# HyoJong-Moon/Distributed-Inference-System-based-Storm

Hardware: AMD Instinct MI355X
Metric: images/sec (whole node) + p50 latency, CIFAR-10 ResNet-20 at 1/2/4/8 GPUs (higher is better)
Workload: dtype bf16

## Files before the change

### csrc/bindings/host_bindings.cpp

```cpp
#include <pybind11/functional.h>
#include <pybind11/numpy.h>
#include <pybind11/pybind11.h>
#include <pybind11/stl.h>

#include <time.h>

#include <atomic>
#include <chrono>
#include <mutex>
#include <thread>

#include "../codec/json_codec.h"
#include "gale/llc_pair.h"
#include "../codec/text_pack.h"
#include "../kafka/broker.h"
#include "../kafka/client.h"
#include "../kafka/compress.h"
#include "../kafka/fetch_framing.h"
#include "../runtime/batch_plan.h"
#include "../runtime/ingest_plan.h"
#include "../runtime/pack_tap.h"
#include "../runtime/resize_plan.h"
#include "plan_dict.h"
#include "../kafka/protocol.h"
// ... 161 lines not shown
    const int64_t t0 = now_ns();
    const int64_t m = (int64_t)set_->batches.size();
    size_t pi = 0;
    int64_t sent = 0;
    while (!stop_) {
      const double due = (double)(now_ns() - t0) * 1e-9 * rate;
      while (!stop_) {
        const size_t k = (size_t)(((next_ % m) + m) % m);
        const int32_t nrec = set_->records[k];
        if ((double)(sent + nrec) > due) break;
        const int part = parts_[pi++ % parts_.size()];
        const int64_t base = b_->append_shared(topic_, part, set_->batches[k]);
        const int64_t t = now_ns();
        {
          std::lock_guard<std::mutex> lk(mu_);
          lp_.push_back(part);
          lbase_.push_back(base);
          ln_.push_back(nrec);
          lt_.push_back(t);
        }
        sent += nrec;
        appended_ += nrec;
        ++next_;
      }
      const int32_t nrec = set_->records[(size_t)(((next_ % m) + m) % m)];
      const double wait_s = ((double)(sent + nrec) - (double)(now_ns() - t0) * 1e-9 * rate) / rate;
      std::this_thread::sleep_for(std::chrono::nanoseconds(
          std::max<int64_t>(20000, (int64_t)(wait_s * 1e9))));
    }
  }
  std::shared_ptr<Broker> b_;
  std::string topic_;
  std::vector<int> parts_;
  std::shared_ptr<BatchSet> set_;
  std::thread t_;
  std::atomic<bool> stop_{true};
  std::atomic<int64_t> next_{0}, appended_{0};
  std::mutex mu_;
  std::vector<int32_t> lp_, ln_;
  std::vector<int64_t> lbase_, lt_;
};

std::shared_ptr<BatchSet> synthetic_batches(const float* x, int64_t n, int H, int W, int C,
                                            int ipr, int rpb, int threads,
                                            const std::string& key_prefix) {
  if (ipr <= 0 || rpb <= 0 || n <= 0) throw std::invalid_argument("synthetic_batches: bad sizes");
  auto bs = std::make_shared<BatchSet>();
  bs->images_per_record = ipr;
  const int64_t nrec = (n + ipr - 1) / ipr;
  const int64_t nb = (nrec + rpb - 1) / rpb;
  bs->batches.resize((size_t)nb);
  bs->records.resize((size_t)nb);
  const size_t img = (size_t)H * W * C;
  std::atomic<int64_t> next{0};
  auto work = [&] {
    std::vector<std::string> vals, keys;
    std::vector<RecordIn> ins;
    for (int64_t b; (b = next++) < nb;) {
      const int64_t r0 = b * rpb, r1 = std::min<int64_t>(nrec, r0 + rpb);
      vals.assign((size_t)(r1 - r0), std::string());
      keys.assign((size_t)(r1 - r0), std::string());
      ins.assign((size_t)(r1 - r0), RecordIn());
      for (int64_t r = r0; r < r1; ++r) {
        const int64_t i0 = r * ipr, cnt = std::min<int64_t>(ipr, n - i0);
        codec::encode_instances(x + (size_t)i0 * img, (int)cnt, H, W, C, vals[(size_t)(r - r0)]);
        RecordIn& ri = ins[(size_t)(r - r0)];
        ri.value = vals[(size_t)(r - r0)];
        if (!key_prefix.empty()) {
          keys[(size_t)(r - r0)] = key_prefix + std::to_string(r);
          ri.key = keys[(size_t)(r - r0)];
          ri.key_null = false;
        }
      }
      Writer w;
      encode_batch(w, ins.data(), ins.size(), 0, 0);
      bs->records[(size_t)b] = (int32_t)(r1 - r0);
      bs->batches[(size_t)b] = std::make_shared<const std::string>(std::move(w.buf));
    }
  };
  std::vector<std::thread> ts;
  for (int t = 1; t < std::max(1, threads); ++t) ts.emplace_back(work);
  work();
  for (auto& t : ts) t.join();
  for (auto& b : bs->batches) bs->bytes += b->size();
  return bs;
}

std::vector<std::string> strs(const py::handle& o) { return o.cast<std::vector<std::string>>(); }

py::bytes py_encode(const std::string& name, py::dict d) {
  Writer w;
  if (name == "request_header") {
    RequestHeader h;
    h.api_key = d["api_key"].cast<int16_t>();
    h.api_version = d["api_version"].cast<int16_t>();
    h.correlation_id = d["correlation_id"].cast<int32_t>();
    h.client_id = d["client_id"].cast<std::string>();
    encode_request_header(w, h);
  } else if (name == "metadata_request") {
    MetadataRequest m;
    if (d["topics"].is_none()) m.all_topics = true;
    else m.topics = strs(d["topics"]);
    m.allow_auto_topic_creation = d["allow_auto_topic_creation"].cast<bool>();
    encode_metadata_request(w, m);
  } else if (name == "fetch_request") {
    FetchRequest m;
    m.max_wait_ms = d["max_wait_ms"].cast<int32_t>();
    m.min_bytes = d["min_bytes"].cast<int32_t>();
    m.max_bytes = d["max_bytes"].cast<int32_t>();
    FetchTopic t;
    t.name = d["topic"].cast<std::string>();
    for (auto p : d["partitions"].cast<py::list>()) {
      auto tp = p.cast<py::tuple>();
      t.partitions.push_back({tp[0].cast<int32_t>(), tp[1].cast<int64_t>(), tp[2].cast<int32_t>()});
    }
    m.topics.push_back(t);
    encode_fetch_request(w, m);
  } else if (name == "produce_request") {
    ProduceRequest m;
    m.acks = d["acks"].cast<int16_t>();
    m.timeout_ms = d["timeout_ms"].cast<int32_t>();
    ProduceTopic t;
    t.name = d["topic"].cast<std::string>();
    ProducePartition pp;
    pp.index = d["partition"].cast<int32_t>();
    pp.records = std::string(view(d["records"].cast<py::bytes>()));
    t.partitions.push_back(pp);
    m.topics.push_back(t);
    encode_produce_request(w, m);
  } else if (name == "list_offsets_request") {
    ListOffsetsRequest m;
    m.topics.push_back({d["topic"].cast<std::string>(),
                        {{d["partition"].cast<int32_t>(), d["timestamp"].cast<int64_t>()}}});
    encode_list_offsets_request(w, m);
  } else if (name == "offset_commit_request") {
    OffsetCommitRequest m;
    m.group_id = d["group_id"].cast<std::string>();
    CommitTopic t;
    t.name = d["topic"].cast<std::string>();
    CommitPartition cp;
    cp.index = d["partition"].cast<int32_t>();
    cp.offset = d["offset"].cast<int64_t>();
    t.partitions.push_back(cp);
    m.topics.push_back(t);
    encode_offset_commit_request(w, m);
  } else {
    throw std::invalid_argument("unknown message " + name);
  }
  return py::bytes(w.buf);
}

py::dict py_decode(const std::string& name, py::bytes b) {
  const std::string_view s = view(b);
  Reader r(s);
  py::dict d;
  if (name == "metadata_response") {
    const MetadataResponse m = decode_metadata_response(r);
    py::list brokers;
    for (auto& n : m.brokers) brokers.append(py::make_tuple(n.node_id, n.host, n.port));
    d["brokers"] = brokers;
    d["cluster_id"] = m.cluster_id;
    d["controller_id"] = m.controller_id;
    py::dict topics;
    for (auto& t : m.topics) {
      py::list parts;
      for (auto& p : t.partitions) parts.append(py::make_tuple(p.index, p.leader, p.error));
      topics[py::str(t.name)] = py::make_tuple(t.error, parts);
    }
    d["topics"] = topics;
  } else if (name == "produce_response") {
    const ProduceResponse m = decode_produce_response(r);
    py::list parts;
    for (auto& t : m.topics)
      for (auto& p : t.partitions)
        parts.append(py::make_tuple(t.name, p.index, p.error, p.base_offset));
    d["partitions"] = parts;
    d["throttle_ms"] = m.throttle_ms;
  } else if (name == "fetch_response") {
    const FetchResponse m = decode_fetch_response(r);
    py::list parts;
    for (auto& t : m.topics)
      for (auto& p : t.partitions) {
        std::vector<RecordRef> recs;
        if (p.records_len > 0)
          decode_records(reinterpret_cast<const uint8_t*>(s.data()), p.records_off,
                         (size_t)p.records_len, 0, true, recs);
        parts.append(py::make_tuple(t.name, p.index, p.error, p.high_watermark,
                                    records_to_py(reinterpret_cast<const uint8_t*>(s.data()), recs)));
      }
    d["partitions"] = parts;
  } else if (name == "api_versions_response") {
    const ApiVersionsResponse m = decode_api_versions_response(r);
    d["error"] = m.error;
    py::dict apis;
    for (auto& a : m.apis) apis[py::int_(a.key)] = py::make_tuple(a.min_version, a.max_version);
    d["apis"] = apis;
  } else {
    throw std::invalid_argument("unknown message " + name);
  }
  return d;
}

std::shared_ptr<py::object> hold(py::object o) {
  return std::shared_ptr<py::object>(new py::object(std::move(o)), [](py::object* p) {
    py::gil_scoped_acquire g;
    delete p;
  });
}

}

void bind_host(py::module_& m) {
  m.def("status_name", &codec::status_name);
  m.def("scan_instances", [](py::bytes b, int H, int W, int C) {
    const std::string_view s = view(b);
    const codec::Scan sc =
        codec::scan_instances(reinterpret_cast<const uint8_t*>(s.data()), s.size(), H, W, C);
    return py::make_tuple(sc.status, sc.arr_off, sc.arr_len, sc.images);
  });
  m.def("parse_instances_host", [](py::bytes b, int H, int W, int C, int max_images) {
    const std::string_view s = view(b);
    const codec::Scan sc =
        codec::scan_instances(reinterpret_cast<const uint8_t*>(s.data()), s.size(), H, W, C);
    const int n = sc.status == codec::OK ? sc.images : 0;
    py::array_t<float> out({(py::ssize_t)n, (py::ssize_t)H, (py::ssize_t)W, (py::ssize_t)C});
    int images = 0;
    int st = sc.status;
    if (st == codec::OK)
      st = codec::parse_instances_host(reinterpret_cast<const uint8_t*>(s.data()), s.size(), H, W,
                                       C, out.mutable_data(), max_images, &images);
    return py::make_tuple(st, out);
  }, py::arg("data"), py::arg("H"), py::arg("W"), py::arg("C"), py::arg("max_images") = -1);
  m.def("scan_instances_b64", [](py::bytes b, int H, int W, int C) {
    const std::string_view s = view(b);
    const codec::Scan sc =
        codec::scan_instances_b64(reinterpret_cast<const uint8_t*>(s.data()), s.size(), H, W, C);
    return py::make_tuple(sc.status, sc.arr_off, sc.arr_len, sc.images);
  });
  m.def("parse_instances_b64_host", [](py::bytes b, int H, int W, int C, int max_images) {
    const std::string_view s = view(b);
    const uint8_t* p = reinterpret_cast<const uint8_t*>(s.data());
    const codec::Scan sc = codec::scan_instances_b64(p, s.size(), H, W, C);
    const int n = sc.status == codec::OK ? sc.images : 0;
    py::array_t<float> out({(py::ssize_t)n, (py::ssize_t)H, (py::ssize_t)W, (py::ssize_t)C});
    int images = 0;
    int st = sc.status;
    if (st == codec::OK)
      st = codec::parse_instances_b64_host(p, s.size(), H, W, C, out.mutable_data(), max_images,
                                           &images);
    return py::make_tuple(st, out);
  }, py::arg("data"), py::arg("H"), py::arg("W"), py::arg("C"), py::arg("max_images") = -1);
  m.def("b64_image_offsets", [](py::bytes arr, int H, int W, int C) -> py::object {
    const std::string_view s = view(arr);
    std::vector<uint32_t> offs;
    if (!codec::b64_image_offsets(reinterpret_cast<const uint8_t*>(s.data()), s.size(), H, W, C,
                                  offs))
      return py::none();
    return py::cast(offs);
  });
  m.def("plan_b64_ingest",
        [](std::vector<std::pair<int64_t, int64_t>> batches,
           std::vector<std::tuple<int, int, int64_t, int64_t, int64_t>> recs,
           std::vector<uint32_t> offs, int H, int W, int C, size_t arena_bytes,
           size_t fetch_size, bool check_crcs) {
          std::vector<B64PlanRecord> rs(recs.size());
          for (size_t i = 0; i < recs.size(); ++i) {
            rs[i].status = std::get<0>(recs[i]);
            rs[i].images = std::get<1>(recs[i]);
            rs[i].value_off = std::get<2>(recs[i]);
            rs[i].value_len = std::get<3>(recs[i]);
            rs[i].arr_off = std::get<4>(recs[i]);
          }
          B64IngestPlan p;
          plan_b64_ingest(batches, kafka::kBatchAttrOffset, check_crcs, rs, offs, H, W, C,
                          arena_bytes, fetch_size, p);
          py::list windows, imgs;
          for (const CrcChunk& c : p.chunks) windows.append(py::make_tuple(c.end, c.len));
          for (const B64Image& d : p.imgs) imgs.append(py::make_tuple(d.off, d.slot, d.rec));
          py::dict out;
          out["windows"] = windows;
          out["batch_windows"] = py::cast(p.batch_chunks);
          out["images"] = imgs;
          out["slot0"] = py::cast(p.slot0);
          out["img0"] = py::cast(p.img0);
          out["chunks_per_image"] = p.chunks_per_image;
          out["lo"] = p.lo;
          out["hi"] = p.hi;
          out["o_chunks"] = p.o_chunks;
          out["o_imgs"] = p.o_imgs;
          out["plan_bytes"] = p.plan_bytes;
          out["o_crc"] = p.o_crc;
          out["o_bad"] = p.o_bad;
          out["result_bytes"] = p.result_bytes;
          return out;
        },
        py::arg("batches"), py::arg("recs"), py::arg("offs"), py::arg("H"), py::arg("W"),
        py::arg("C"), py::arg("arena_bytes"), py::arg("fetch_size"),
        py::arg("check_crcs") = true,
        "The host plan of a b64 fetch's device ingest (csrc/runtime/ingest_plan.h)");
  m.def("plan_json_ingest",
        [](std::vector<std::pair<int64_t, int64_t>> batches,
           std::vector<std::tuple<int, int64_t, int64_t, int64_t, int64_t>> recs, int H, int W,
           int C, size_t arena_bytes, size_t fetch_size, size_t dev_cap, int64_t tap_result,
           bool plan_separate, bool check_crcs) {
          std::vector<JsonPlanRecord> rs(recs.size());
          for (size_t i = 0; i < recs.size(); ++i) {
            rs[i].status = std::get<0>(recs[i]);
            rs[i].value_off = std::get<1>(recs[i]);
            rs[i].value_len = std::get<2>(recs[i]);
            rs[i].arr_off = std::get<3>(recs[i]);
            rs[i].arr_len = std::get<4>(recs[i]);
          }
          JsonIngestPlan p;
          plan_json_ingest(batches, kafka::kBatchAttrOffset, check_crcs, rs, H, W, C, arena_bytes,
                           fetch_size, dev_cap, tap_result, plan_separate, p);
          std::string plan(p.o_gsum, '\0');
          if (!p.empty()) fill_json_ingest(p, rs, reinterpret_cast<uint8_t*>(&plan[0]));
          py::list windows;
          for (const CrcChunk& c : p.chunks) windows.append(py::make_tuple(c.end, c.len));
          py::dict out;
          out["windows"] = windows;
          out["batch_windows"] = py::cast(p.batch_chunks);
          out["rec_of"] = py::cast(p.rec_of);
          out["pjs"] = py::cast(p.pjs);
          out["nc"] = p.nc();
          out["nr"] = p.nr();
          out["np"] = p.np();
          out["ntiles"] = p.ntiles;
          out["ngroups"] = p.ngroups;
          out["ptiles"] = p.ptiles;
          out["ng"] = p.ng;
          out["packed"] = p.packed;
          out["lo"] = p.lo;
          out["span"] = p.span;
          out["link"] = p.link;
          out["c_lo"] = p.c_lo;
          out["c_len"] = p.c_len;
          out["tab_off"] = p.tab_off;
          out["used"] = p.used;
          out["cnt_base"] = p.cnt_base;
          out["o_chunks"] = p.o_chunks;
          out["o_groups"] = p.o_groups;
          out["o_recs"] = p.o_recs;
          out["o_precs"] = p.o_precs;
          out["o_ptr"] = p.o_ptr;
          out["o_gsum"] = p.o_gsum;
          out["prefix"] = p.o_gsum;
          out["o_crc"] = p.o_crc;
          out["o_gbad"] = p.o_gbad;
          out["o_pbad"] = p.o_pbad;
          out["io_bytes"] = p.io_bytes;
          out["plan_off"] = p.plan_off;
          out["plan_in_chunk"] = p.plan_in_chunk;
          out["plan"] = py::bytes(plan);
          return out;
        },
        py::arg("batches"), py::arg("recs"), py::arg("H"), py::arg("W"), py::arg("C"),
        py::arg("arena_bytes"), py::arg("fetch_size"), py::arg("dev_cap"),
        py::arg("tap_result") = (int64_t)-1, py::arg("plan_separate") = false,
        py::arg("check_crcs") = true,
        "The host plan of a JSON fetch's device ingest, laid out and filled "
        "(csrc/runtime/ingest_plan.h)");
  m.def("plan_batch",
        [](std::vector<py::dict> recs, int max_batch, int tiles_cap, int64_t per,
           const std::string& form, bool ptr_input, bool b64, uint64_t d_bytes,
           uint64_t input_base) {
          std::vector<BatchPlanRecord> rs(recs.size());
          std::vector<uint32_t> offs;
          for (size_t i = 0; i < recs.size(); ++i) {
            const py::dict& d = recs[i];
            BatchPlanRecord& r = rs[i];
            auto get = [&d](const char* k, auto& v) {
              if (d.contains(k)) v = d[k].cast<std::decay_t<decltype(v)>>();
            };
            get("buf", r.buf);
            get("arr_off", r.arr_off);
            get("arr_len", r.arr_len);
            get("images", r.images);
            get("pinned", r.pinned);
            get("resident", r.resident);
            get("preparsed", r.preparsed);
            get("dev_text", r.dev_text);
            get("dev_counts", r.dev_counts);
            get("dev_image", r.dev_image);
            if (d.contains("b64_offs")) {
              const auto o = d["b64_offs"].cast<std::vector<uint32_t>>();
              r.b64_first = (int32_t)offs.size();
              r.b64_n = (int32_t)o.size();
              offs.insert(offs.end(), o.begin(), o.end());
            }
          }
          const StepForm f = form == "op-by-op"   ? StepForm::OpByOp
                             : form == "captured" ? StepForm::Captured
                             : form == "kernels"  ? StepForm::Kernels
                                                  : throw std::invalid_argument("plan_batch: form");
          BatchPlan p;
          plan_batch(rs, max_batch, per, f, ptr_input, b64, p);
          const MetaLayout L(max_batch, std::max(tiles_cap, p.ntiles));
          const MetaRange used = L.used(p);
          std::string meta(L.total, '\xee');
          fill_batch(p, rs, offs, L, d_bytes, input_base, reinterpret_cast<uint8_t*>(&meta[0]));
          py::list spans, staged;
          for (const BatchPlan::Span& x : p.spans)
            spans.append(py::make_tuple(x.buf, x.lo, x.len, x.dev));
          for (const BatchPlan::Staged& g : p.staged)
            staged.append(py::make_tuple(g.rec, g.host, g.len));
          py::dict out;
          out["spans"] = spans;
          out["staged"] = staged;
          out["parse_idx"] = py::cast(p.parse_idx);
          out["staged_bytes"] = p.staged_bytes;
          out["staged_dev"] = p.staged_dev;
          out["dev_total"] = p.dev_total;
          out["nrec"] = p.nrec;
          out["ntiles"] = p.ntiles;
          out["img"] = p.img;
          out["b64n"] = p.b64n;
          out["npre"] = p.npre;
          out["resident"] = p.resident;
          out["count_pass"] = p.count_pass;
          py::dict lay;
          lay["hdr"] = L.hdr;
          lay["recs"] = L.recs;
          lay["xs"] = L.xs;
          lay["tiles"] = L.tiles;
          lay["b64_table"] = L.b64_table;
          lay["b64_status"] = L.b64_status;
          lay["total"] = L.total;
          out["layout"] = lay;
          out["used"] = py::make_tuple(used.off, used.bytes);
          out["meta"] = py::bytes(meta);
          return out;
        },
        py::arg("recs"), py::arg("max_batch"), py::arg("tiles_cap"), py::arg("per"),
        py::arg("form"), py::arg("ptr_input") = false, py::arg("b64") = false,
        py::arg("d_bytes") = (uint64_t)0, py::arg("input_base") = (uint64_t)0,
        "The host plan of a GPU replica's batch, laid out and filled "
        "(csrc/runtime/batch_plan.h)");
  m.def("validate_plan",
        [](py::list ops, std::vector<long long> buf_bytes, int max_batch, int slots, int chunk_ops,
           int chunk_images) {
          const PlanSpec spec = plan_spec_from_py(ops, std::move(buf_bytes), max_batch, slots, {},
                                                  chunk_ops, chunk_images);
          validate_plan(spec);
          return plan_ops_to_py(spec);
        },
        py::arg("ops"), py::arg("buf_bytes"), py::arg("max_batch") = 256, py::arg("slots") = 2,
        py::arg("chunk_ops") = 0, py::arg("chunk_images") = 0,
        "What Executor(...) checks before its first HIP call (gale/forward_plan.h), without a "
        "GPU: ValueError for a plan it would refuse, else the ops with every key written out");
  m.attr("BATCH_ATTR_OFFSET") = (int)kafka::kBatchAttrOffset;
  m.def("split_instances_b64", [](py::bytes arr, int H, int W, int C) -> py::object {
    const std::string_view s = view(arr);
    std::vector<std::pair<uint32_t, uint32_t>> spans;
    if (!codec::split_instances_b64(reinterpret_cast<const uint8_t*>(s.data()), s.size(), H, W,
                                    C, spans))
      return py::none();
    return py::cast(spans);
  });
  m.def("scan_instances_b64_bytes", [](py::bytes b, int64_t nbytes) {
    const std::string_view s = view(b);
    const codec::Scan sc = codec::scan_instances_b64_bytes(
        reinterpret_cast<const uint8_t*>(s.data()), s.size(), nbytes);
    return py::make_tuple(sc.status, sc.arr_off, sc.arr_len, sc.images);
  });
  m.def("b64_image_offsets_bytes", [](py::bytes arr, int64_t nbytes) -> py::object {
    const std::string_view s = view(arr);
    std::vector<uint32_t> offs;
    if (!codec::b64_image_offsets_bytes(reinterpret_cast<const uint8_t*>(s.data()), s.size(),
                                        nbytes, offs))
      return py::none();
    return py::cast(offs);
  });
  m.def("split_instances_b64_bytes", [](py::bytes arr, int64_t nbytes) -> py::object {
    const std::string_view s = view(arr);
    std::vector<std::pair<uint32_t, uint32_t>> spans;
    if (!codec::split_instances_b64_bytes(reinterpret_cast<const uint8_t*>(s.data()), s.size(),
                                          nbytes, spans))
      return py::none();
    return py::cast(spans);
  });
  m.def("yuv_coeffs", [](const std::string& matrix, const std::string& range) {
    YuvCoeffs k;
    const int mi = matrix == "bt601" ? 0 : matrix == "bt709" ? 1 : -1;
    const int ri = range == "limited" ? 0 : range == "full" ? 1 : -1;
    if (!yuv_coeffs(mi, ri, &k)) throw std::invalid_argument("yuv_coeffs: matrix / range");
    return py::make_tuple(k.cy, k.crv, k.cgu, k.cgv, k.cbu, k.yo);
  });
  m.def("yuv420_to_rgb_host",
        [](py::bytes frame, int HS, int WS, const std::string& format,
           std::vector<int32_t> coeffs, std::optional<std::vector<float>> a,
           std::optional<std::vector<float>> b) {
          const std::string_view s = view(frame);
          if (coeffs.size() != 6 || (a && a->size() < 3) || (b && b->size() < 3) ||
              bool(a) != bool(b))
            throw std::invalid_argument("yuv420_to_rgb_host: coeffs (6), a / b (>= 3 each)");
          const int fmt = format == "i420" ? YUV_I420 : format == "nv12" ? YUV_NV12 : YUV_NONE;
          if (fmt == YUV_NONE || HS <= 0 || WS <= 0 || (HS & 1) || (WS & 1) ||
              (int64_t)s.size() != yuv420_bytes(HS, WS))
            throw std::invalid_argument("yuv420_to_rgb_host: format / size / byte count");
          YuvCoeffs k;
          k.cy = coeffs[0], k.crv = coeffs[1], k.cgu = coeffs[2], k.cgv = coeffs[3];
          k.cbu = coeffs[4], k.yo = coeffs[5];
          py::array_t<uint8_t> rgb({(py::ssize_t)HS, (py::ssize_t)WS, (py::ssize_t)3});
          py::array_t<float> f32({(py::ssize_t)HS, (py::ssize_t)WS, (py::ssize_t)3});
          codec::yuv420_to_rgb_host(reinterpret_cast<const uint8_t*>(s.data()), HS, WS, fmt, k,
                                    rgb.mutable_data(), f32.mutable_data(),
                                    a ? a->data() : nullptr, b ? b->data() : nullptr);
          return py::make_tuple(rgb, f32);
        },
        py::arg("frame"), py::arg("HS"), py::arg("WS"), py::arg("format"), py::arg("coeffs"),
        py::arg("a") = py::none(), py::arg("b") = py::none());
  m.def("parse_instances_yuv_host",
        [](py::bytes b, int HS, int WS, const std::string& format, std::vector<int32_t> coeffs,
           int max_images) {
          const std::string_view s = view(b);
          const uint8_t* p = reinterpret_cast<const uint8_t*>(s.data());
          if (coeffs.size() != 6) throw std::invalid_argument("parse_instances_yuv_host: coeffs");
          const int fmt = format == "i420" ? YUV_I420 : format == "nv12" ? YUV_NV12 : YUV_NONE;
          YuvCoeffs k;
          k.cy = coeffs[0], k.crv = coeffs[1], k.cgu = coeffs[2], k.cgv = coeffs[3];
          k.cbu = coeffs[4], k.yo = coeffs[5];
          int n = 0;
          int st = codec::parse_instances_yuv_host(p, s.size(), HS, WS, fmt, k, nullptr,
                                                   max_images, &n);
          if (st != codec::OK) n = 0;
          py::array_t<float> out({(py::ssize_t)n, (py::ssize_t)std::max(HS, 0),
                                  (py::ssize_t)std::max(WS, 0), (py::ssize_t)3});
          if (st == codec::OK)
            st = codec::parse_instances_yuv_host(p, s.size(), HS, WS, fmt, k, out.mutable_data(),
                                                 max_images, &n);
          return py::make_tuple(st, out);
        },
        py::arg("data"), py::arg("HS"), py::arg("WS"), py::arg("format"), py::arg("coeffs"),
        py::arg("max_images") = -1);
  m.def("packed_bpp", [](const std::string& format) {
    return packed_bpp(packed_format_of(format.c_str()));
  });
  m.def("packed_to_rgb_host",
        [](py::bytes image, int HS, int WS, const std::string& format,
           std::optional<std::vector<float>> a, std::optional<std::vector<float>> b) {
          const std::string_view s = view(image);
          if ((a && a->size() < 3) || (b && b->size() < 3) || bool(a) != bool(b))
            throw std::invalid_argument("packed_to_rgb_host: a / b (>= 3 each)");
          const int fmt = packed_format_of(format.c_str());
          if (fmt == PACKED_NONE || HS <= 0 || WS <= 0 ||
              (int64_t)s.size() != packed_bytes(HS, WS, fmt))
            throw std::invalid_argument("packed_to_rgb_host: format / size / byte count");
          py::array_t<uint8_t> rgb({(py::ssize_t)HS, (py::ssize_t)WS, (py::ssize_t)3});
          py::array_t<float> f32({(py::ssize_t)HS, (py::ssize_t)WS, (py::ssize_t)3});
          codec::packed_to_rgb_host(reinterpret_cast<const uint8_t*>(s.data()), HS, WS, fmt,
                                    rgb.mutable_data(), f32.mutable_data(),
                                    a ? a->data() : nullptr, b ? b->data() : nullptr);
          return py::make_tuple(rgb, f32);
        },
        py::arg("image"), py::arg("HS"), py::arg("WS"), py::arg("format"),
        py::arg("a") = py::none(), py::arg("b") = py::none());
  m.def("parse_instances_packed_host",
        [](py::bytes b, int HS, int WS, const std::string& format, int max_images) {
          const std::string_view s = view(b);
          const uint8_t* p = reinterpret_cast<const uint8_t*>(s.data());
          const int fmt = packed_format_of(format.c_str());
          int n = 0;
          int st = codec::parse_instances_packed_host(p, s.size(), HS, WS, fmt, nullptr,
                                                      max_images, &n);
          if (st != codec::OK) n = 0;
          py::array_t<float> out({(py::ssize_t)n, (py::ssize_t)std::max(HS, 0),
                                  (py::ssize_t)std::max(WS, 0), (py::ssize_t)3});
          if (st == codec::OK)
            st = codec::parse_instances_packed_host(p, s.size(), HS, WS, fmt, out.mutable_data(),
                                                    max_images, &n);
          return py::make_tuple(st, out);
        },
        py::arg("data"), py::arg("HS"), py::arg("WS"), py::arg("format"),
        py::arg("max_images") = -1);
  m.def("apply_input_prep",
        [](py::array_t<float, py::array::c_style | py::array::forcecast> x, int H, int W, int C,
           bool nchw, std::vector<float> a, std::vector<float> b) {
          const size_t per = (size_t)H * W * C;
          if (a.size() != 4 || b.size() != 4 || per == 0 || (size_t)x.size() % per != 0)
            throw std::invalid_argument("apply_input_prep: four coefficients, whole images");
          const py::ssize_t n = x.size() / (py::ssize_t)per;
          py::array_t<float> out({n, (py::ssize_t)H, (py::ssize_t)W, (py::ssize_t)C});
          memcpy(out.mutable_data(), x.data(), (size_t)x.size() * sizeof(float));
          codec::apply_input_prep(out.mutable_data(), (int)n, H, W, C, nchw, a.data(), b.data());
          return out;
        },
        py::arg("x"), py::arg("H"), py::arg("W"), py::arg("C"), py::arg("nchw"), py::arg("a"),
        py::arg("b"));
  auto ia = [](const void* p, size_t n) {
    return py::array_t<int32_t>((py::ssize_t)n, static_cast<const int32_t*>(p));
  };
  auto fa = [](const void* p, size_t n) {
    return py::array_t<float>((py::ssize_t)n, static_cast<const float*>(p));
  };
  m.def("build_resize_tables",
        [ia, fa](int HS, int WS, int HR, int WR, int H, int W) {
          codec::ResizeTables t;
          codec::build_resize_tables(HS, WS, HR, WR, H, W, t);
          return py::make_tuple(ia(t.y0.data(), H), ia(t.y1.data(), H), fa(t.wy.data(), H),
                                ia(t.x0.data(), W), ia(t.x1.data(), W), fa(t.wx.data(), W));
        },
        py::arg("HS"), py::arg("WS"), py::arg("HR"), py::arg("WR"), py::arg("H"), py::arg("W"));
  m.def("build_resize_aa_tables",
        [ia, fa](int HS, int WS, int HR, int WR, int H, int W, bool device) -> py::object {
          const InputResize r = InputResize::build(HS, WS, HR, WR, H, W, true);
          const codec::ResizeAaTables& t = r.aa_tables();
          if (!device)
            return py::make_tuple(ia(t.ys.data(), H), ia(t.yn.data(), H),
                                  fa(t.wy.data(), t.wy.size()), ia(t.xs.data(), W),
                                  ia(t.xn.data(), W), fa(t.wx.data(), t.wx.size()));
          const ResizeDeviceImage im = pack(r);
          auto at = [&](int i) { return im.bytes.data() + im.off[i]; };
          return py::make_tuple(ia(at(0), H), ia(at(1), H), fa(at(2), (size_t)H * im.ty),
                                ia(at(3), W), ia(at(4), W), fa(at(5), (size_t)W * im.tx), im.ty,
                                im.tx, im.band, im.band_rows);
        },
        py::arg("HS"), py::arg("WS"), py::arg("HR"), py::arg("WR"), py::arg("H"), py::arg("W"),
        py::arg("device") = false);
  m.def("resize_device_image",
        [](int HS, int WS, int HR, int WR, int H, int W, bool antialias) {
          const ResizeDeviceImage im = pack(InputResize::build(HS, WS, HR, WR, H, W, antialias));
          return py::make_tuple(
              py::array_t<uint8_t>((py::ssize_t)im.bytes.size(), im.bytes.data()),
              py::make_tuple(im.off[0], im.off[1], im.off[2], im.off[3], im.off[4], im.off[5]),
              py::make_tuple(im.ty, im.tx, im.band, im.band_rows));
        },
        py::arg("HS"), py::arg("WS"), py::arg("HR"), py::arg("WR"), py::arg("H"), py::arg("W"),
        py::arg("antialias"));
  for (const bool aa : {false, true}) {
    const char* name = aa ? "resize_crop_aa_host" : "resize_crop_host";
    m.def(name,
          [aa, name](py::array_t<float, py::array::c_style | py::array::forcecast> x, int HR,
                     int WR, int H, int W) {
            if (x.ndim() != 4)
              throw std::invalid_argument(std::string(name) + ": x must be [N, HS, WS, C]");
            const InputResize r =
                InputResize::build((int)x.shape(1), (int)x.shape(2), HR, WR, H, W, aa);
            const int C = (int)x.shape(3);
            py::array_t<float> out({x.shape(0), (py::ssize_t)H, (py::ssize_t)W, (py::ssize_t)C});
            r.apply_host(x.data(), (int)x.shape(0), C, out.mutable_data());
            return out;
          },
          py::arg("x"), py::arg("HR"), py::arg("WR"), py::arg("H"), py::arg("W"));
  }
  m.def("text_pack_fast", &codec::text_pack_fast);
  m.def("llc_pin_self_next_domain", &llc::pin_self_next_domain);
  m.def("llc_register_local_port", &llc::register_local_port);
  m.def("llc_pin_self_for_peer", &llc::pin_self_for_peer);
  m.def("set_pack_stream_stores", &codec::set_pack_stream_stores,
        "non-temporal stores for the packed stream (default on; A/B switch)");
  m.def("text_pack", [](py::bytes b, bool force_scalar) {
    const std::string_view s = view(b);
    std::string out(codec::pack_bound(s.size()), '\0');
    py::array_t<uint32_t> tab((py::ssize_t)(2 * codec::pack_groups(s.size())));
    const size_t n = codec::text_pack(reinterpret_cast<const uint8_t*>(s.data()), s.size(),
                                      reinterpret_cast<uint8_t*>(out.data()), tab.mutable_data(),
                                      force_scalar);
    out.resize(n);
    return py::make_tuple(py::bytes(out), tab);
  }, py::arg("data"), py::arg("force_scalar") = false);
  m.def("text_pack_chunked", [](py::bytes b, std::vector<size_t> cuts) {
    const std::string_view s = view(b);
// ... 683 lines not shown
```

### csrc/bindings/module.cpp

```cpp
#include <pybind11/numpy.h>
#include <pybind11/pybind11.h>
#include <pybind11/stl.h>

#include <optional>
#include <stdexcept>
#include <vector>

#include "../comm/rccl.h"
#include "gale/executor.h"
#include "gale/kernels.h"
#include "plan_dict.h"

namespace py = pybind11;

namespace gale {
void bind_host(py::module_& m);
}

namespace {

using gale::ConvDesc;
using gale::desc_from_dict;

inline hipStream_t S(uintptr_t s) { return reinterpret_cast<hipStream_t>(s); }
inline void* P(uintptr_t p) { return reinterpret_cast<void*>(p); }

void chk(hipError_t e, const char* what) { gale::check_hip(e, what); }

std::optional<gale::InputPrep> prep_from(const char* name,
                                         const std::optional<std::vector<float>>& a,
                                         const std::optional<std::vector<float>>& b, bool nchw) {
  if ((a && a->size() != 4) || (b && b->size() != 4))
    throw std::invalid_argument(std::string(name) + ": a / b take four coefficients");
  if (!a && !b && !nchw) return std::nullopt;
  gale::InputPrep prep;
  for (int i = 0; i < 4; ++i) {
    if (a) prep.a[i] = (*a)[i];
    if (b) prep.b[i] = (*b)[i];
  }
  prep.nchw = nchw ? 1 : 0;
  return prep;
}

}

namespace gale {
void install_crash_handler();
}

namespace {
struct MappedBuffer {
  uint8_t* p = nullptr;
  size_t n = 0;
  explicit MappedBuffer(size_t bytes) : n(bytes) {
    gale::check_hip(hipHostMalloc(reinterpret_cast<void**>(&p), bytes ? bytes : 1,
                                  hipHostMallocMapped),
                    "hipHostMalloc(mapped)");
    void* dp = nullptr;
    gale::check_hip(hipHostGetDevicePointer(&dp, p, 0), "hipHostGetDevicePointer");
    if (dp != p) throw std::runtime_error("mapped buffer: device address differs from host");
  }
  ~MappedBuffer() {
    if (p) hipHostFree(p);
  }
};
}

PYBIND11_MODULE(_C, m) {
  py::class_<MappedBuffer, std::shared_ptr<MappedBuffer>>(
      m, "MappedBuffer", "host-mapped pinned buffer (same address on the host and the GPU)")
      .def(py::init<size_t>())
      .def_property_readonly("ptr", [](const MappedBuffer& b) { return (uintptr_t)b.p; })
      .def_property_readonly("size", [](const MappedBuffer& b) { return b.n; })
      .def("numpy", [](std::shared_ptr<MappedBuffer> b) {
        return py::array_t<uint8_t>({(py::ssize_t)b->n}, {1}, b->p,
                                    py::capsule(new std::shared_ptr<MappedBuffer>(b), [](void* c) {
                                      delete static_cast<std::shared_ptr<MappedBuffer>*>(c);
                                    }));
      });
  m.doc() = "gale native library: gfx950 kernels, plan executor, host runtime";
  gale::install_crash_handler();

  m.def("conv2d",
        [](py::dict desc, int batch, uintptr_t x, uintptr_t w, uintptr_t bias, uintptr_t wscale,
           uintptr_t res, uintptr_t y, uintptr_t stream) {
          ConvDesc d = desc_from_dict(desc);
          chk(gale::conv2d(d, batch, P(x), P(w), static_cast<const float*>(P(bias)),
                           static_cast<const float*>(P(wscale)), P(res), P(y), S(stream)),
              "conv2d");
        },
        py::arg("desc"), py::arg("batch"), py::arg("x"), py::arg("w"), py::arg("bias"),
        py::arg("wscale"), py::arg("res"), py::arg("y"), py::arg("stream"));
  m.def("bottleneck56",
        [](int batch, uintptr_t x, uintptr_t w1, uintptr_t b1, uintptr_t w2, uintptr_t b2,
           uintptr_t w3, uintptr_t b3, uintptr_t wd, uintptr_t bd, uintptr_t y, int cin,
           int down, uintptr_t stream) {
          gale::BottleneckParams bp;
          bp.w1 = P(w1); bp.w2 = P(w2); bp.w3 = P(w3); bp.wd = P(wd);
          bp.b1 = static_cast<const float*>(P(b1));
          bp.b2 = static_cast<const float*>(P(b2));
          bp.b3 = static_cast<const float*>(P(b3));
          bp.bd = static_cast<const float*>(P(bd));
          bp.cin = cin;
          bp.down = down;
          chk(gale::bottleneck56(bp, batch, P(x), P(y), S(stream)), "bottleneck56");
        },
        py::arg("batch"), py::arg("x"), py::arg("w1"), py::arg("b1"), py::arg("w2"),
        py::arg("b2"), py::arg("w3"), py::arg("b3"), py::arg("wd"), py::arg("bd"), py::arg("y"),
        py::arg("cin"), py::arg("down"), py::arg("stream"));
  m.def("bottleneck56_supported", &gale::bottleneck56_supported, py::arg("H"), py::arg("W"),
        py::arg("cin"), py::arg("cmid"), py::arg("cout"), py::arg("down"));
  m.def("stem_pool",
        [](int batch, uintptr_t x, uintptr_t w, uintptr_t bias, uintptr_t y, uintptr_t stream) {
          chk(gale::stem_pool(batch, P(x), P(w), static_cast<const float*>(P(bias)), P(y),
                              S(stream)),
              "stem_pool");
        },
        py::arg("batch"), py::arg("x"), py::arg("w"), py::arg("bias"), py::arg("y"),
        py::arg("stream"));
  m.def("stem_pack",
        [](int batch, int H, int W, int C, int Wp, int lp, uintptr_t x, uintptr_t y,
           uintptr_t stream) {
          chk(gale::stem_pack(batch, H, W, C, Wp, lp, static_cast<const float*>(P(x)), P(y),
                              S(stream)),
              "stem_pack");
        });
  m.def("maxpool2d",
        [](int batch, int H, int W, int C, int k, int s, int p, int Ho, int Wo, uintptr_t x,
           uintptr_t y, uintptr_t stream, int fp8) {
          chk(gale::maxpool2d(batch, H, W, C, k, s, p, Ho, Wo, P(x), P(y), fp8, S(stream)),
              "maxpool2d");
        },
        py::arg("batch"), py::arg("H"), py::arg("W"), py::arg("C"), py::arg("k"), py::arg("s"),
        py::arg("p"), py::arg("Ho"), py::arg("Wo"), py::arg("x"), py::arg("y"), py::arg("stream"),
        py::arg("fp8") = 0);
  m.def("avgpool_global",
        [](int batch, int HW, int C, uintptr_t x, uintptr_t y, uintptr_t stream, int fp8) {
          chk(gale::avgpool_global(batch, HW, C, P(x), P(y), fp8, S(stream)), "avgpool_global");
        },
        py::arg("batch"), py::arg("HW"), py::arg("C"), py::arg("x"), py::arg("y"),
        py::arg("stream"), py::arg("fp8") = 0);
  m.def("head_pool_dense_softmax",
        [](int batch, int HW, int C, int N, uintptr_t x, uintptr_t w, uintptr_t b, uintptr_t out,
           uintptr_t stream, int fp8, float in_scale) {
          chk(gale::head_pool_dense_softmax(batch, HW, C, N, P(x), fp8, in_scale,
                                            static_cast<const float*>(P(w)),
                                            static_cast<const float*>(P(b)),
                                            static_cast<float*>(P(out)), S(stream)),
              "head_pool_dense_softmax");
        },
        py::arg("batch"), py::arg("HW"), py::arg("C"), py::arg("N"), py::arg("x"), py::arg("w"),
        py::arg("b"), py::arg("out"), py::arg("stream"), py::arg("fp8") = 0,
        py::arg("in_scale") = 1.0f);
  m.def("softmax_rows", [](int batch, int N, int ld, uintptr_t x, uintptr_t out, uintptr_t stream) {
    chk(gale::softmax_rows(batch, N, ld, static_cast<const float*>(P(x)),
                           static_cast<float*>(P(out)), S(stream)),
        "softmax_rows");
  });
  m.def("cast_f32_bf16",
        [](int64_t n, float scale, float shift, uintptr_t x, uintptr_t y, uintptr_t stream) {
          chk(gale::cast_f32_bf16(n, scale, shift, static_cast<const float*>(P(x)), P(y),
                                  S(stream)),
              "cast_f32_bf16");
        });
  m.def("bn_act",
        [](int batch, int HW, int Wo, int C, uintptr_t x, uintptr_t scale, uintptr_t shift,
           uintptr_t res, int res_H, int res_W, int res_C, int rs, int relu, uintptr_t y,
           uintptr_t stream) {
          chk(gale::bn_act(batch, HW, Wo, C, P(x), static_cast<const float*>(P(scale)),
                           static_cast<const float*>(P(shift)), P(res), res_H, res_W, res_C, rs,
                           relu, P(y), S(stream)),
              "bn_act");
        });
  m.def("json_parse_instances",
        [](int nrec, int ntiles, uintptr_t recs, uintptr_t tile_rec, uintptr_t bytes, int H,
           int W, int C, uintptr_t tile_counts, uintptr_t out, uintptr_t stream,
           bool count_pass, std::optional<std::vector<float>> a,
           std::optional<std::vector<float>> b, bool nchw, uintptr_t d_ntiles, uintptr_t status,
           uintptr_t tile_bad) {
          const auto prep = prep_from("json_parse_instances", a, b, nchw);
          chk(gale::json_parse_instances(nrec, ntiles, static_cast<gale::JsonRecord*>(P(recs)),
                                         static_cast<const int*>(P(tile_rec)),
                                         static_cast<const uint8_t*>(P(bytes)), H, W, C,
                                         static_cast<int*>(P(tile_counts)),
                                         static_cast<float*>(P(out)), S(stream), count_pass,
                                         static_cast<const int*>(P(d_ntiles)),
                                         static_cast<int*>(P(status)),
                                         static_cast<int*>(P(tile_bad)),
                                         prep ? &*prep : nullptr),
              "json_parse_instances");
        },
        py::arg("nrec"), py::arg("ntiles"), py::arg("recs"), py::arg("tile_rec"),
        py::arg("bytes"), py::arg("H"), py::arg("W"), py::arg("C"), py::arg("tile_counts"),
        py::arg("out"), py::arg("stream"), py::arg("count_pass") = true,
        py::arg("a") = py::none(), py::arg("b") = py::none(), py::arg("nchw") = false,
        py::arg("d_ntiles") = 0, py::arg("status") = 0, py::arg("tile_bad") = 0);
  m.def("json_tile_count", &gale::json_tile_count);
  m.def("b64_decode_instances",
        [](int images, uintptr_t imgs, uintptr_t bytes, int H, int W, int C, uintptr_t out,
           uintptr_t status, uintptr_t stream, uintptr_t d_images,
           std::optional<std::vector<float>> a, std::optional<std::vector<float>> b, bool nchw) {
          const auto prep = prep_from("b64_decode_instances", a, b, nchw);
          chk(gale::b64_decode_instances(images, static_cast<const gale::B64Image*>(P(imgs)),
                                         static_cast<const uint8_t*>(P(bytes)), H, W, C,
                                         static_cast<float*>(P(out)),
                                         static_cast<int*>(P(status)), S(stream),
                                         static_cast<const int*>(P(d_images)),
                                         prep ? &*prep : nullptr),
              "b64_decode_instances");
        },
        py::arg("images"), py::arg("imgs"), py::arg("bytes"), py::arg("H"), py::arg("W"),
        py::arg("C"), py::arg("out"), py::arg("status"), py::arg("stream"),
        py::arg("d_images") = 0, py::arg("a") = py::none(), py::arg("b") = py::none(),
        py::arg("nchw") = false);
  m.def("b64_yuv_instances",
        [](int images, uintptr_t imgs, uintptr_t bytes, int HS, int WS, int C, uintptr_t out,
           uintptr_t status, uintptr_t stream, uintptr_t d_images, const std::string& format,
           std::vector<int32_t> coeffs, std::optional<std::vector<float>> a,
           std::optional<std::vector<float>> b, bool nchw, int pairs) {
          const auto prep = prep_from("b64_yuv_instances", a, b, nchw);
          if (coeffs.size() != 6)
            throw std::invalid_argument("b64_yuv_instances: coeffs takes (cy, crv, cgu, cgv, "
                                        "cbu, yo)");
          gale::YuvCoeffs k;
          k.cy = coeffs[0], k.crv = coeffs[1], k.cgu = coeffs[2], k.cgv = coeffs[3];
          k.cbu = coeffs[4], k.yo = coeffs[5];
          const int fmt = format == "i420"   ? (int)gale::YUV_I420
                          : format == "nv12" ? (int)gale::YUV_NV12
                                             : (int)gale::YUV_NONE;
          return (int)gale::b64_yuv_instances(
              images, static_cast<const gale::B64Image*>(P(imgs)),
              static_cast<const uint8_t*>(P(bytes)), HS, WS, C, static_cast<float*>(P(out)),
              static_cast<int*>(P(status)), S(stream), static_cast<const int*>(P(d_images)),
              prep ? &*prep : nullptr, fmt, k, pairs);
        },
        py::arg("images"), py::arg("imgs"), py::arg("bytes"), py::arg("HS"), py::arg("WS"),
        py::arg("C"), py::arg("out"), py::arg("status"), py::arg("stream"),
        py::arg("d_images") = 0, py::arg("format") = "i420",
        py::arg("coeffs") = std::vector<int32_t>{1220945, 1673555, -410793, -852458, 2115221, 16},
        py::arg("a") = py::none(), py::arg("b") = py::none(), py::arg("nchw") = false,
        py::arg("pairs") = 0);
  m.def("b64_packed_instances",
        [](int images, uintptr_t imgs, uintptr_t bytes, int HS, int WS, int C, uintptr_t out,
           uintptr_t status, uintptr_t stream, uintptr_t d_images, const std::string& format,
           std::optional<std::vector<float>> a, std::optional<std::vector<float>> b, bool nchw) {
          const auto prep = prep_from("b64_packed_instances", a, b, nchw);
          return (int)gale::b64_packed_instances(
              images, static_cast<const gale::B64Image*>(P(imgs)),
              static_cast<const uint8_t*>(P(bytes)), HS, WS, C, static_cast<float*>(P(out)),
              static_cast<int*>(P(status)), S(stream), static_cast<const int*>(P(d_images)),
              prep ? &*prep : nullptr, gale::packed_format_of(format.c_str()));
        },
        py::arg("images"), py::arg("imgs"), py::arg("bytes"), py::arg("HS"), py::arg("WS"),
        py::arg("C"), py::arg("out"), py::arg("status"), py::arg("stream"),
        py::arg("d_images") = 0, py::arg("format") = "bgr24", py::arg("a") = py::none(),
        py::arg("b") = py::none(), py::arg("nchw") = false);
  m.def("b64_yuv_pairs", &gale::b64_yuv_pairs);
  m.def("b64_yuv_lds_bytes", &gale::b64_yuv_lds_bytes);
  m.attr("YUV_LDS_BUDGET") = (int)gale::kYuvLdsBudget;
  m.attr("HIP_ERROR_INVALID_VALUE") = (int)hipErrorInvalidValue;
  m.attr("B64_IMAGE_BYTES") = (int)sizeof(gale::B64Image);
  py::module_ comm = m.def_submodule("comm", "in-process RCCL communicator (ncclCommInitAll)");
  py::class_<gale::CommGroup, std::shared_ptr<gale::CommGroup>>(comm, "CommGroup")
      .def(py::init([](std::vector<int> devices) {
             py::gil_scoped_release nogil;
             return std::make_shared<gale::CommGroup>(devices);
           }),
           py::arg("devices"))
      .def_property_readonly("size", &gale::CommGroup::size)
      .def_property_readonly("devices", &gale::CommGroup::devices)
      .def("broadcast",
           [](gale::CommGroup& g, uintptr_t send_root, std::vector<uintptr_t> recv, size_t bytes,
              int root) {
             std::vector<void*> r;
             for (uintptr_t p : recv) r.push_back(reinterpret_cast<void*>(p));
             py::gil_scoped_release nogil;
             g.broadcast(reinterpret_cast<const void*>(send_root), r, bytes, root);
           },
           py::arg("send_root"), py::arg("recv"), py::arg("bytes"), py::arg("root") = 0)
      .def("all_reduce_sum_f64",
           [](gale::CommGroup& g, std::vector<uintptr_t> bufs, size_t count) {
             std::vector<double*> b;
             for (uintptr_t p : bufs) b.push_back(reinterpret_cast<double*>(p));
             py::gil_scoped_release nogil;
             g.all_reduce_sum_f64(b, count);
           },
           py::arg("bufs"), py::arg("count"));
  m.def("crc32c_chunks",
        [](uintptr_t bytes, uintptr_t chunks, int n, uintptr_t tables, uintptr_t out,
           uintptr_t stream) {
          gale::check_hip(gale::crc32c_chunks(reinterpret_cast<const uint8_t*>(bytes),
                                              reinterpret_cast<const gale::CrcChunk*>(chunks), n,
                                              reinterpret_cast<const uint32_t*>(tables),
                                              reinterpret_cast<uint32_t*>(out),
                                              reinterpret_cast<hipStream_t>(stream)),
                          "crc32c_chunks");
        });
  m.def("ingest_crc_count",
        [](uintptr_t bytes, uintptr_t chunks, int nchunks, uintptr_t tables, uintptr_t crc_out,
           int nrec, int ngroups, uintptr_t recs, uintptr_t groups, uintptr_t counts,
           uintptr_t gsum, uintptr_t stream, uintptr_t gbad, uintptr_t packed, uintptr_t tab,
           uintptr_t text_out) {
          gale::check_hip(
              gale::ingest_crc_count(reinterpret_cast<const uint8_t*>(bytes),
                                     reinterpret_cast<const gale::CrcChunk*>(chunks), nchunks,
                                     reinterpret_cast<const uint32_t*>(tables),
                                     reinterpret_cast<uint32_t*>(crc_out), nrec, ngroups,
                                     reinterpret_cast<gale::JsonRecord*>(recs),
                                     reinterpret_cast<const int2*>(groups),
                                     reinterpret_cast<int*>(counts),
                                     reinterpret_cast<int*>(gsum),
                                     reinterpret_cast<int*>(gbad),
                                     reinterpret_cast<hipStream_t>(stream),
                                     reinterpret_cast<const uint8_t*>(packed),
                                     reinterpret_cast<const uint32_t*>(tab),
                                     reinterpret_cast<uint8_t*>(text_out)),
              "ingest_crc_count");
        },
        py::arg("bytes"), py::arg("chunks"), py::arg("nchunks"), py::arg("tables"),
        py::arg("crc_out"), py::arg("nrec"), py::arg("ngroups"), py::arg("recs"),
        py::arg("groups"), py::arg("counts"), py::arg("gsum"), py::arg("stream"),
        py::arg("gbad") = 0, py::arg("packed") = 0, py::arg("tab") = 0, py::arg("text_out") = 0,
        "groups: int32 (record, first tile) pairs, GROUP_TILES tiles each; counts: per record "
        "tile0 + grp0 -> [tile counts][group sums]; gsum: one int per group");
  m.attr("GROUP_TILES") = gale::kGroupTiles;
  m.def("ingest_crc_b64",
        [](uintptr_t bytes, uintptr_t chunks, int nchunks, uintptr_t tables, uintptr_t crc_out,
           int images, uintptr_t imgs, int H, int W, int C, uintptr_t arena, uintptr_t wg_bad,
           uintptr_t stream, std::optional<std::vector<float>> a,
           std::optional<std::vector<float>> b, bool nchw) {
          const auto prep = prep_from("ingest_crc_b64", a, b, nchw);
          chk(gale::ingest_crc_b64(static_cast<const uint8_t*>(P(bytes)),
                                   static_cast<const gale::CrcChunk*>(P(chunks)), nchunks,
                                   static_cast<const uint32_t*>(P(tables)),
                                   static_cast<uint32_t*>(P(crc_out)), images,
                                   static_cast<const gale::B64Image*>(P(imgs)), H, W, C,
                                   static_cast<float*>(P(arena)), static_cast<int*>(P(wg_bad)),
                                   S(stream), prep ? &*prep : nullptr),
              "ingest_crc_b64");
        },
        py::arg("bytes"), py::arg("chunks"), py::arg("nchunks"), py::arg("tables"),
        py::arg("crc_out"), py::arg("images"), py::arg("imgs"), py::arg("H"), py::arg("W"),
        py::arg("C"), py::arg("arena"), py::arg("wg_bad"), py::arg("stream"),
        py::arg("a") = py::none(), py::arg("b") = py::none(), py::arg("nchw") = false);
  m.attr("B64_CHUNK_CHARS") = gale::kB64ChunkChars;
  m.def("text_unpack", [](uintptr_t packed, uintptr_t tab, int64_t n, uintptr_t out,
                          uintptr_t stream) {
    if (out % 16 || packed % 8) throw std::invalid_argument("text_unpack: misaligned buffers");
    gale::check_hip(gale::text_unpack(reinterpret_cast<const uint8_t*>(packed),
                                      reinterpret_cast<const uint32_t*>(tab), n,
                                      reinterpret_cast<uint8_t*>(out),
                                      reinterpret_cast<hipStream_t>(stream)),
                    "text_unpack");
  });
  m.def("format_floats_java", [](int n, uintptr_t x, uintptr_t out16, uintptr_t stream) {
    gale::check_hip(gale::format_floats_java(n, reinterpret_cast<const float*>(x),
                                             reinterpret_cast<void*>(out16),
                                             reinterpret_cast<hipStream_t>(stream)),
                    "format_floats_java");
  });
  m.def("format_floats_java_dev",
        [](int max_n, uintptr_t d_count, int per, uintptr_t x, uintptr_t out16,
           uintptr_t stream) {
          chk(gale::format_floats_java_dev(max_n, static_cast<const int*>(P(d_count)), per,
                                           static_cast<const float*>(P(x)), P(out16), S(stream)),
              "format_floats_java_dev");
        },
        py::arg("max_n"), py::arg("d_count"), py::arg("per"), py::arg("x"), py::arg("out16"),
        py::arg("stream"));
  m.def("format_floats_java_step",
        [](int max_n, uintptr_t d_count, int per, uintptr_t x, uintptr_t out16, uintptr_t d_nrec,
           uintptr_t status, uintptr_t status_out, uintptr_t stream) {
          chk(gale::format_floats_java_step(max_n, static_cast<const int*>(P(d_count)), per,
                                            static_cast<const float*>(P(x)), P(out16),
                                            static_cast<const int*>(P(d_nrec)),
                                            static_cast<int*>(P(status)),
                                            static_cast<int*>(P(status_out)), S(stream)),
              "format_floats_java_step");
        },
        py::arg("max_n"), py::arg("d_count"), py::arg("per"), py::arg("x"), py::arg("out16"),
        py::arg("d_nrec"), py::arg("status"), py::arg("status_out"), py::arg("stream"));
  m.def("topk_java",
        [](int rows, int classes, int k, uintptr_t x, uintptr_t text16, uintptr_t idx,
           uintptr_t stream) {
          chk(gale::topk_java(rows, classes, k, static_cast<const float*>(P(x)), P(text16),
                              static_cast<int32_t*>(P(idx)), S(stream)),
              "topk_java");
        },
        py::arg("rows"), py::arg("classes"), py::arg("k"), py::arg("x"), py::arg("text16"),
        py::arg("idx"), py::arg("stream"));
  m.def("topk_java_dev",
        [](int max_rows, uintptr_t d_rows, int classes, int k, uintptr_t x, uintptr_t text16,
           uintptr_t idx, uintptr_t stream) {
          chk(gale::topk_java_dev(max_rows, static_cast<const int*>(P(d_rows)), classes, k,
                                  static_cast<const float*>(P(x)), P(text16),
                                  static_cast<int32_t*>(P(idx)), S(stream)),
              "topk_java_dev");
        },
        py::arg("max_rows"), py::arg("d_rows"), py::arg("classes"), py::arg("k"), py::arg("x"),
        py::arg("text16"), py::arg("idx"), py::arg("stream"));
  m.def("topk_java_step",
        [](int max_rows, uintptr_t d_rows, int classes, int k, uintptr_t x, uintptr_t text16,
           uintptr_t idx, uintptr_t d_nrec, uintptr_t status, uintptr_t status_out,
           uintptr_t stream) {
          chk(gale::topk_java_step(max_rows, static_cast<const int*>(P(d_rows)), classes, k,
                                   static_cast<const float*>(P(x)), P(text16),
                                   static_cast<int32_t*>(P(idx)),
                                   static_cast<const int*>(P(d_nrec)),
                                   static_cast<int*>(P(status)),
                                   static_cast<int*>(P(status_out)), S(stream)),
              "topk_java_step");
        },
        py::arg("max_rows"), py::arg("d_rows"), py::arg("classes"), py::arg("k"), py::arg("x"),
        py::arg("text16"), py::arg("idx"), py::arg("d_nrec"), py::arg("status"),
        py::arg("status_out"), py::arg("stream"));
  auto resize_plan = [](int HS, int WS, int H, int W, int C, const std::vector<uintptr_t>& t) {
    if (t.size() != 6) throw std::invalid_argument("resize_crop: six table pointers");
    gale::ResizePlan p;
    p.HS = HS, p.WS = WS, p.H = H, p.W = W, p.C = C;
    p.y0 = static_cast<const int32_t*>(P(t[0]));
    p.y1 = static_cast<const int32_t*>(P(t[1]));
    p.wy = static_cast<const float*>(P(t[2]));
    p.x0 = static_cast<const int32_t*>(P(t[3]));
    p.x1 = static_cast<const int32_t*>(P(t[4]));
    p.wx = static_cast<const float*>(P(t[5]));
    return p;
  };
  m.def("resize_crop",
        [resize_plan](int images, int HS, int WS, int H, int W, int C,
                      std::vector<uintptr_t> tables, uintptr_t src, uintptr_t dst,
                      uintptr_t stream) {
          chk(gale::resize_crop(images, resize_plan(HS, WS, H, W, C, tables),
                                static_cast<const float*>(P(src)), static_cast<float*>(P(dst)),
                                S(stream)),
              "resize_crop");
        },
        py::arg("images"), py::arg("HS"), py::arg("WS"), py::arg("H"), py::arg("W"), py::arg("C"),
        py::arg("tables"), py::arg("src"), py::arg("dst"), py::arg("stream"));
  m.def("resize_crop_dev",
        [resize_plan](int max_images, uintptr_t d_images, int HS, int WS, int H, int W, int C,
                      std::vector<uintptr_t> tables, uintptr_t src, uintptr_t dst,
                      uintptr_t stream) {
          chk(gale::resize_crop_dev(max_images, static_cast<const int*>(P(d_images)),
                                    resize_plan(HS, WS, H, W, C, tables),
                                    static_cast<const float*>(P(src)), static_cast<float*>(P(dst)),
                                    S(stream)),
              "resize_crop_dev");
        },
        py::arg("max_images"), py::arg("d_images"), py::arg("HS"), py::arg("WS"), py::arg("H"),
        py::arg("W"), py::arg("C"), py::arg("tables"), py::arg("src"), py::arg("dst"),
        py::arg("stream"));
  auto resize_aa_plan = [](const std::vector<int>& dims, const std::vector<uintptr_t>& t,
                           const std::vector<int>& launch) {
    if (dims.size() != 7 || t.size() != 6 || launch.size() != 4)
      throw std::invalid_argument("resize_crop_aa: seven dims, six table pointers, four figures");
    gale::ResizeAaPlan p;
    p.HS = dims[0], p.WS = dims[1], p.HR = dims[2], p.WR = dims[3], p.H = dims[4], p.W = dims[5];
    p.C = dims[6];
    p.ty = launch[0], p.tx = launch[1], p.band = launch[2], p.band_rows = launch[3];
    p.ys = static_cast<const int32_t*>(P(t[0]));
    p.yn = static_cast<const int32_t*>(P(t[1]));
    p.wy = static_cast<const float*>(P(t[2]));
    p.xs = static_cast<const int32_t*>(P(t[3]));
    p.xn = static_cast<const int32_t*>(P(t[4]));
    p.wx = static_cast<const float*>(P(t[5]));
    return p;
  };
  m.def("resize_crop_aa",
        [resize_aa_plan](int images, std::vector<int> dims, std::vector<uintptr_t> tables,
                         std::vector<int> launch, uintptr_t src, uintptr_t dst, uintptr_t stream) {
          chk(gale::resize_crop_aa(images, resize_aa_plan(dims, tables, launch),
                                   static_cast<const float*>(P(src)), static_cast<float*>(P(dst)),
                                   S(stream)),
              "resize_crop_aa");
        },
        py::arg("images"), py::arg("dims"), py::arg("tables"), py::arg("launch"), py::arg("src"),
        py::arg("dst"), py::arg("stream"));
  m.def("resize_crop_aa_dev",
        [resize_aa_plan](int max_images, uintptr_t d_images, std::vector<int> dims,
                         std::vector<uintptr_t> tables, std::vector<int> launch, uintptr_t src,
                         uintptr_t dst, uintptr_t stream) {
          chk(gale::resize_crop_aa_dev(max_images, static_cast<const int*>(P(d_images)),
                                       resize_aa_plan(dims, tables, launch),
                                       static_cast<const float*>(P(src)),
                                       static_cast<float*>(P(dst)), S(stream)),
              "resize_crop_aa_dev");
        },
        py::arg("max_images"), py::arg("d_images"), py::arg("dims"), py::arg("tables"),
        py::arg("launch"), py::arg("src"), py::arg("dst"), py::arg("stream"));
  m.attr("FLOAT_TEXT_SLOT") = gale::kFloatTextSlot;
  m.attr("INPUT_TABLE_IMAGES") = gale::kInputTableImages;
  m.attr("INPUT_TABLE_BASES") = gale::kInputTableBases;
  m.def("set_conv_path", &gale::set_conv_path);
  m.def("set_conv_patch", &gale::set_conv_patch);
  m.def("conv_patch_supported", [](py::dict desc, int batch, bool has_res) {
    return gale::conv_patch_supported(desc_from_dict(desc), batch, has_res);
  });
  m.def("conv_mfma_plan", [](py::dict desc, int batch, bool has_res) {
    const gale::ConvMfmaPlan p = gale::conv_mfma_plan(desc_from_dict(desc), batch, has_res);
    static const char* const kModes[] = {"fast", "gather", "1x1"};
    py::dict r;
    r["ok"] = p.ok;
    r["mode"] = kModes[p.mode];
    r["nt"] = p.nt;
    r["pr"] = p.pr;
    r["n_blocks"] = p.n_blocks;
    r["bk"] = p.bk;
    r["nkc"] = p.nkc;
    r["m_tiles"] = p.m_tiles;
    r["grid_m"] = p.grid_m;
    r["lds_bytes"] = p.lds_bytes;
    return r;
  }, py::arg("desc"), py::arg("batch"), py::arg("has_res"));
  m.def("device_pci_bus_id", [](int device) {
    char buf[64] = {0};
    chk(hipDeviceGetPCIBusId(buf, (int)sizeof(buf), device), "hipDeviceGetPCIBusId");
    return std::string(buf);
  });
  m.def("conv_path", &gale::conv_path);
  m.attr("JSON_TILE_BYTES") = gale::kJsonTileBytes;
  m.attr("JSON_RECORD_BYTES") = (int)sizeof(gale::JsonRecord);
  m.def("memcpy_async",
        [](uintptr_t dst, uintptr_t src, size_t n, uintptr_t stream) {
          chk(hipMemcpyAsync(P(dst), P(src), n, hipMemcpyDefault, S(stream)), "memcpy_async");
        });
  m.def("stream_sync", [](uintptr_t stream) {
    py::gil_scoped_release nogil;
    chk(hipStreamSynchronize(S(stream)), "stream_sync");
  });

  py::class_<gale::Executor, std::shared_ptr<gale::Executor>>(m, "Executor")
      .def(py::init([](int device, py::list ops, std::vector<long long> buf_bytes, int max_batch,
                       int slots, std::vector<int> buckets, int chunk_ops, int chunk_images) {
             return std::make_shared<gale::Executor>(
                 device, gale::plan_spec_from_py(ops, std::move(buf_bytes), max_batch, slots,
                                                 std::move(buckets), chunk_ops, chunk_images));
           }),
           py::arg("device"), py::arg("ops"), py::arg("buf_bytes"), py::arg("max_batch"),
           py::arg("slots") = 2, py::arg("buckets") = std::vector<int>{}, py::arg("chunk_ops") = 0,
           py::arg("chunk_images") = 0)
      .def("run",
           [](gale::Executor& e, int slot, int batch, uintptr_t stream, bool use_graph) {
             py::gil_scoped_release nogil;
             e.run(slot, batch, S(stream), use_graph);
           },
           py::arg("slot"), py::arg("batch"), py::arg("stream"), py::arg("use_graph") = true)
      .def("run_on",
           [](gale::Executor& e, int batch, uintptr_t in, uintptr_t out, uintptr_t stream) {
             py::gil_scoped_release nogil;
             e.run_on(batch, P(in), P(out), S(stream));
           })
      .def("capture_all",
           [](gale::Executor& e, uintptr_t stream) {
             py::gil_scoped_release nogil;
             e.capture_all(S(stream));
           })
      .def("launch_device_batch",
           [](gale::Executor& e, int slot, uintptr_t d_batch, uintptr_t stream, uintptr_t text,
              uintptr_t status, uintptr_t status_out, uintptr_t nrec, uintptr_t xs) {
             if (status_out && (!status || !nrec))
               throw py::value_error("launch_device_batch: status_out needs status and nrec");
             gale::StepOut so;
             so.text = P(text);
             so.status = static_cast<int*>(P(status));
             so.status_out = static_cast<int*>(P(status_out));
             so.nrec = static_cast<const int*>(P(nrec));
             py::gil_scoped_release nogil;
             e.launch_device_batch(slot, static_cast<const int*>(P(d_batch)), S(stream),
                                   text || status_out ? &so : nullptr,
                                   static_cast<const float* const*>(P(xs)));
           },
           py::arg("slot"), py::arg("d_batch"), py::arg("stream"), py::arg("text") = 0,
           py::arg("status") = 0, py::arg("status_out") = 0, py::arg("nrec") = 0,
           py::arg("xs") = 0)
      .def("launch_table",
           [](gale::Executor& e, int slot, int batch, std::vector<uintptr_t> bases,
              std::vector<uint32_t> codes, uintptr_t stream, uintptr_t text) {
             if (bases.size() > (size_t)gale::kInputTableBases ||
                 codes.size() > (size_t)gale::kInputTableImages)
               throw py::value_error("launch_table: too many bases / codes for an InputTable");
             gale::InputTable tab{};
             for (size_t i = 0; i < bases.size(); ++i)
               tab.base[i] = static_cast<const float*>(P(bases[i]));
             for (size_t i = 0; i < codes.size(); ++i) tab.code[i] = codes[i];
             gale::StepOut so;
             so.text = P(text);
             py::gil_scoped_release nogil;
             e.launch_table(slot, batch, tab, S(stream), text ? &so : nullptr);
           },
           py::arg("slot"), py::arg("batch"), py::arg("bases"), py::arg("codes"),
           py::arg("stream"), py::arg("text") = 0)
      .def("input_ptr", [](gale::Executor& e, int slot) { return (uintptr_t)e.input(slot); })
      .def("output_ptr", [](gale::Executor& e, int slot) { return (uintptr_t)e.output(slot); })
      .def("bucket_for", &gale::Executor::bucket_for)
      .def_property_readonly("buckets", &gale::Executor::buckets)
      .def_property_readonly("max_batch", &gale::Executor::max_batch)
      .def_property_readonly("slots", &gale::Executor::slots)
      .def_property_readonly("device", &gale::Executor::device)
      .def_property_readonly("graphs_captured", &gale::Executor::graphs_captured)
      .def_property_readonly("graph_pays", &gale::Executor::graph_pays)
      .def_property_readonly("step_out_ok", &gale::Executor::step_out_ok);

  gale::bind_host(m);
}
```

### csrc/include/gale/kernels.h

```cpp
#pragma once
#include <hip/hip_runtime.h>
#include <stdint.h>

#include "../../codec/pixfmt.h"
#include "../../codec/yuv.h"

namespace gale {

struct ConvDesc {
  int H, W, Cin;
  int Ho, Wo, Cout;
  int KH, KW, stride, pad;
  int K;
  int Kpad;
  int Npad;
  int relu;
  int has_res, res_H, res_W, res_C, res_stride;
  int in_f32;
  int out_f32;
  int fp8;
  float in_scale;
  float out_scale;
  float res_scale;
  int stem;
  int f32;
};

hipError_t conv2d(const ConvDesc& d, int batch, const void* x, const void* w, const float* bias,
                  const float* wscale, const void* res, void* y, hipStream_t stream);
hipError_t conv2d_f32(const ConvDesc& d, int batch, const void* x, const void* w,
                      const float* bias, const void* res, void* y, hipStream_t stream);

enum ConvMfmaMode : int { CONV_MFMA_FAST = 0, CONV_MFMA_GATHER = 1, CONV_MFMA_1X1 = 2 };
struct ConvMfmaPlan {
  bool ok = false;
  int mode = CONV_MFMA_FAST;
  int nt = 0;
  int pr = 0;
  int n_blocks = 0;
  int bk = 0;
  int nkc = 0;
  int m_tiles = 0;
  int grid_m = 0;
  size_t lds_bytes = 0;
};
ConvMfmaPlan conv_mfma_plan(const ConvDesc& d, int batch, bool has_res);

enum ElemType : int { ET_BF16 = 0, ET_FP8 = 1, ET_F32 = 2 };

bool conv_gemm_supported(const ConvDesc& d, int batch, bool has_res);
void set_conv_path(int mode);
int conv_path();
bool conv_gemm_proj_supported(const ConvDesc& d, int batch, int H2, int W2, int Cin2,
                              int stride2, int Kpad2);
hipError_t conv2d_gemm_proj(const ConvDesc& d, int batch, const void* x, const void* w,
                            const float* bias, const void* x2, int H2, int W2, int Cin2,
                            int stride2, int Kpad2, const void* w2, const float* bias2, void* y,
                            hipStream_t stream);
hipError_t conv2d_gemm(const ConvDesc& d, int batch, const void* x, const void* w,
                       const float* bias, const void* res, void* y, hipStream_t stream);

bool conv_patch_supported(const ConvDesc& d, int batch, bool has_res);
void set_conv_patch(int mode);
hipError_t conv2d_patch(const ConvDesc& d, int batch, const void* x, const void* w,
                        const float* bias, const void* res, void* y, hipStream_t stream);

struct BottleneckParams {
  const void* w1 = nullptr;
  const void* w2 = nullptr;
  const void* w3 = nullptr;
  const void* wd = nullptr;
  const float* b1 = nullptr;
  const float* b2 = nullptr;
  const float* b3 = nullptr;
  const float* bd = nullptr;
  int cin = 256;
  int down = 0;
};
bool bottleneck56_supported(int H, int W, int cin, int cmid, int cout, int down);
hipError_t bottleneck56(const BottleneckParams& p, int batch, const void* x, void* y,
                        hipStream_t stream);

bool stem_pool_supported(const ConvDesc& d, int H, int W, int C, int k, int s, int p, int Ho,
                         int Wo);
hipError_t stem_pool(int batch, const void* x, const void* w, const float* bias, void* y,
                     hipStream_t stream);

hipError_t stem_pack(int batch, int H, int W, int C, int Wp, int lp, const float* x, void* y,
                     hipStream_t stream);

hipError_t maxpool2d(int batch, int H, int W, int C, int k, int s, int p, int Ho, int Wo,
                     const void* x, void* y, int et, hipStream_t stream);

hipError_t avgpool_global(int batch, int HW, int C, const void* x, void* y, int et,
                          hipStream_t stream);

hipError_t head_pool_dense_softmax(int batch, int HW, int C, int N, const void* x, int et,
                                   float in_scale, const float* w, const float* bias, float* out,
                                   hipStream_t stream);

constexpr int kInputTableImages = 512, kInputTableBases = 16;
struct InputTable {
  const float* base[kInputTableBases];
  uint32_t code[kInputTableImages];
};

struct StepOut {
  void* text = nullptr;
  int* status = nullptr;
  int* status_out = nullptr;
  const int* nrec = nullptr;
};

struct ResNet20Params {
  const void* w[19];
  const float* b[19];
  const float* fc_w;
  const float* fc_b;
  int fp8;
  const float* ws[19];
  float s_in[19], s_out[19], s_res[19];
  const int* batch_dev;
  StepOut so;
  const float* const* xs;
};
hipError_t resnet20_fused_forward(const ResNet20Params& p, int batch, const float* x, float* out,
                                  hipStream_t stream, const InputTable* tab = nullptr);

struct LeNet5Params {
  const void* w1;
  const float* b1;
  const void* w2;
  const float* b2;
  const void* w3;
  const float* b3;
  const void* w4;
  const float* b4;
  const float* w5;
  const float* b5;
  const int* batch_dev;
  StepOut so;
  const float* const* xs;
};
hipError_t lenet5_fused_forward(const LeNet5Params& p, int batch, const float* x, float* out,
                                hipStream_t stream, const InputTable* tab = nullptr);

hipError_t softmax_rows(int batch, int N, int ld, const float* x, float* out, hipStream_t stream);

hipError_t bn_act(int batch, int HW, int Wo, int C, const void* x, const float* scale,
                  const float* shift, const void* res, int res_H, int res_W, int res_C, int rs,
                  int relu, void* y, hipStream_t stream, int et = 0);

hipError_t cast_f32_bf16(int64_t n, float scale, float shift, const float* x, void* y,
                         hipStream_t stream);


constexpr int kJsonTileBytes = 2048;
constexpr int kGroupTiles = 4;
struct JsonRecord {
  int64_t off;
  int32_t len;
  int32_t slot;
  int32_t images;
  int32_t status;
  int32_t tile0;
  int32_t has_cnt;
  int64_t cnt_off;
  int64_t grp0;
};
static_assert(sizeof(JsonRecord) == 48, "JsonRecord layout (host <-> device tables)");
inline int json_tile_count(int64_t off, int32_t len) {
  if (len <= 0) return 0;
  const int64_t abeg = off & ~(int64_t)15;
  return (int)((off + len - abeg + kJsonTileBytes - 1) / kJsonTileBytes);
}
struct InputPrep {
  int nchw = 0;
  float a[4] = {1.f, 1.f, 1.f, 1.f};
  float b[4] = {0.f, 0.f, 0.f, 0.f};
  bool identity() const {
    for (int i = 0; i < 4; ++i)
      if (a[i] != 1.f || b[i] != 0.f) return false;
    return !nchw;
  }
};
hipError_t json_parse_instances(int nrec, int ntiles, JsonRecord* recs, const int* tile_rec,
                                const uint8_t* bytes, int H, int W, int C, int* tile_counts,
                                float* out, hipStream_t stream, bool count_pass = true,
                                const int* d_ntiles = nullptr, int* status = nullptr,
                                int* tile_bad = nullptr, const InputPrep* prep = nullptr);

constexpr int kB64ChunkChars = 4096;
struct B64Image {
  int64_t off;
  int32_t slot;
  int32_t rec;
};
static_assert(sizeof(B64Image) == 16, "B64Image layout (host <-> device tables)");
hipError_t b64_decode_instances(int images, const B64Image* imgs, const uint8_t* bytes, int H,
                                int W, int C, float* out, int* status, hipStream_t stream,
                                const int* d_images = nullptr, const InputPrep* prep = nullptr);

constexpr size_t kYuvLdsBudget = 64 * 1024;
int b64_yuv_pairs(int HS, int WS);
size_t b64_yuv_lds_bytes(int WS, int pairs);
hipError_t b64_yuv_instances(int images, const B64Image* imgs, const uint8_t* bytes, int HS,
                             int WS, int C, float* out, int* status, hipStream_t stream,
                             const int* d_images, const InputPrep* prep, int format,
                             const YuvCoeffs& coeffs, int pairs = 0);

hipError_t b64_packed_instances(int images, const B64Image* imgs, const uint8_t* bytes, int HS,
                                int WS, int C, float* out, int* status, hipStream_t stream,
                                const int* d_images, const InputPrep* prep, int format);

struct ResizePlan {
  int HS = 0, WS = 0, H = 0, W = 0, C = 0;
  const int32_t* y0 = nullptr;
  const int32_t* y1 = nullptr;
  const float* wy = nullptr;
  const int32_t* x0 = nullptr;
  const int32_t* x1 = nullptr;
  const float* wx = nullptr;
};
hipError_t resize_crop(int images, const ResizePlan& plan, const float* src, float* dst,
                       hipStream_t stream);
hipError_t resize_crop_dev(int max_images, const int* d_images, const ResizePlan& plan,
                           const float* src, float* dst, hipStream_t stream);

struct ResizeAaPlan {
  int HS = 0, WS = 0, HR = 0, WR = 0, H = 0, W = 0, C = 0;
  int ty = 0, tx = 0;
  int band = 0, band_rows = 0;
  const int32_t* ys = nullptr;
  const int32_t* yn = nullptr;
  const float* wy = nullptr;
  const int32_t* xs = nullptr;
  const int32_t* xn = nullptr;
  const float* wx = nullptr;
};
hipError_t resize_crop_aa(int images, const ResizeAaPlan& plan, const float* src, float* dst,
                          hipStream_t stream);
hipError_t resize_crop_aa_dev(int max_images, const int* d_images, const ResizeAaPlan& plan,
                              const float* src, float* dst, hipStream_t stream);

constexpr int kCrcChunkBytes = 4096;
struct CrcChunk {
  int64_t end;
  int32_t len;
  int32_t pad_;
};
hipError_t crc32c_chunks(const uint8_t* bytes, const CrcChunk* chunks, int n,
                         const uint32_t* tables, uint32_t* out, hipStream_t stream);

hipError_t ingest_crc_count(const uint8_t* bytes, const CrcChunk* chunks, int nchunks,
                            const uint32_t* tables, uint32_t* crc_out, int nrec, int ngroups,
                            JsonRecord* recs, const int2* groups, int* counts, int* gsum,
                            int* gbad, hipStream_t stream, const uint8_t* packed = nullptr,
                            const uint32_t* tab = nullptr, uint8_t* text_out = nullptr);

hipError_t ingest_crc_b64(const uint8_t* bytes, const CrcChunk* chunks, int nchunks,
                          const uint32_t* tables, uint32_t* crc_out, int images,
                          const B64Image* imgs, int H, int W, int C, float* arena, int* wg_bad,
                          hipStream_t stream, const InputPrep* prep = nullptr);

hipError_t text_unpack(const uint8_t* packed, const uint32_t* tab, int64_t n, uint8_t* out,
                       hipStream_t stream);

constexpr int kFloatTextSlot = 16;
hipError_t format_floats_java(int n, const float* x, void* out16, hipStream_t stream);
hipError_t format_floats_java_dev(int max_n, const int* d_count, int per, const float* x,
                                  void* out16, hipStream_t stream);
hipError_t format_floats_java_step(int max_n, const int* d_count, int per, const float* x,
                                   void* out16, const int* d_nrec, int* status, int* status_out,
                                   hipStream_t stream);

hipError_t topk_java(int rows, int classes, int k, const float* x, void* text16, int32_t* idx,
                     hipStream_t stream);
hipError_t topk_java_dev(int max_rows, const int* d_rows, int classes, int k, const float* x,
                         void* text16, int32_t* idx, hipStream_t stream);
hipError_t topk_java_step(int max_rows, const int* d_rows, int classes, int k, const float* x,
                          void* text16, int32_t* idx, const int* d_nrec, int* status,
                          int* status_out, hipStream_t stream);

}
```

### csrc/kernels/json_parse.hip

```cpp
#include "common.cuh"
#include "crc32c.cuh"
#include "gale/kernels.h"
#include "exact_decimal.cuh"
#include "text_expand.cuh"

namespace gale {
namespace {

constexpr int kTile = kJsonTileBytes;
constexpr int kLaneBytes = kTile / 64;
constexpr int kChunks = kLaneBytes / 16;
static_assert(kChunks >= 1 && kChunks * 16 * 64 == kTile, "tile = 64 lanes x 16-byte chunks");
constexpr int kHalo = 64;
constexpr int kWaves = 4;
constexpr int kText = kTile + 2 * kHalo + 16;
constexpr int kMaxTok = kTile / 2;

__device__ __forceinline__ bool is_ws(unsigned c) {
  return c == ' ' || c == '\n' || c == '\r' || c == '\t';
}
__device__ __forceinline__ bool is_delim(unsigned c) {
  return c == '[' || c == ']' || c == ',' || is_ws(c);
}

__device__ __forceinline__ double pow10_exact(int k) {
  const double a = (k & 1) ? 1e1 : 1.0, b = (k & 2) ? 1e2 : 1.0, c = (k & 4) ? 1e4 : 1.0,
               d = (k & 8) ? 1e8 : 1.0, e = (k & 16) ? 1e16 : 1.0;
  return ((a * b) * (c * d)) * e;
}

constexpr uint32_t kHi03 = 0x08060001u, kHi47 = 0x00102010u;
constexpr uint32_t kLo03 = 0x0808080Au, kLo47 = 0x08081808u, kLo8B = 0x24010908u,
                   kLoCF = 0x00042502u;
constexpr uint32_t kDelimG = 0x23232323u, kNumG = 0x1C1C1C1Cu, kDigitG = 0x08080808u;

__device__ __forceinline__ uint32_t classify4(uint32_t x) {
  const uint32_t hi = __builtin_amdgcn_perm(kHi47, kHi03, (x >> 4) & 0x07070707u);
  const uint32_t l = x & 0x0F0F0F0Fu;
  const uint32_t s = l & 0x07070707u;
  const uint32_t p0 = __builtin_amdgcn_perm(kLo47, kLo03, s);
  const uint32_t p1 = __builtin_amdgcn_perm(kLoCF, kLo8B, s);
  const uint32_t m = ((l >> 3) & 0x01010101u) * 0xFFu;
  const uint32_t lo = (m & p1) | (~m & p0);
  const uint32_t ascii = ~(((x >> 7) & 0x01010101u) * 0xFFu);
  return hi & lo & ascii;
}

__device__ __forceinline__ uint32_t nz4(uint32_t cls, uint32_t g) {
  const uint32_t t = ((cls & g) + 0x7F7F7F7Fu) & 0x80808080u;
  return ((t >> 7) * 0x01020408u) >> 24;
}

struct Masks16 {
  uint32_t delim, num, digit;
};

__device__ __forceinline__ Masks16 classify16(uint32_t w0, uint32_t w1, uint32_t w2,
                                              uint32_t w3) {
  const uint32_t c0 = classify4(w0), c1 = classify4(w1), c2 = classify4(w2), c3 = classify4(w3);
  Masks16 m;
  m.delim = nz4(c0, kDelimG) | nz4(c1, kDelimG) << 4 | nz4(c2, kDelimG) << 8 |
            nz4(c3, kDelimG) << 12;
  m.num = nz4(c0, kNumG) | nz4(c1, kNumG) << 4 | nz4(c2, kNumG) << 8 | nz4(c3, kNumG) << 12;
  m.digit = nz4(c0, kDigitG) | nz4(c1, kDigitG) << 4 | nz4(c2, kDigitG) << 8 |
            nz4(c3, kDigitG) << 12;
  return m;
}

__device__ __forceinline__ uint32_t bits_range(int a, int b) {
  return b > a ? ((1u << b) - 1u) & ~((1u << a) - 1u) : 0u;
}

__device__ __forceinline__ uint32_t valid16(int p, int beg, int end) {
  return bits_range(min(max(beg - p, 0), 16), min(max(end - p, 0), 16));
}

__device__ __forceinline__ uint32_t chunk_masks(const Masks16& m, int p, int beg, int end) {
  const uint32_t vm = valid16(p, beg, end);
  return ((m.delim | ~vm) & 0xFFFFu) | (m.digit & vm) << 16;
}

__device__ __forceinline__ void token_starts(const uint4 (&v)[kChunks], int o, int beg, int end,
                                             bool prev_delim, uint32_t (&st)[kChunks],
                                             uint32_t (&cm)[kChunks], bool* bad) {
  uint32_t carry = prev_delim ? 1u : 0u;
  bool b = false;
#pragma unroll
  for (int i = 0; i < kChunks; ++i) {
    const Masks16 m = classify16(v[i].x, v[i].y, v[i].z, v[i].w);
    cm[i] = chunk_masks(m, o + 16 * i, beg, end);
    const uint32_t dx = cm[i] & 0xFFFFu;
    const uint32_t tokb = ~dx & 0xFFFFu;
    b |= (tokb & ~m.num) != 0;
    st[i] = tokb & ((dx << 1) | carry) & 0xFFFFu;
    carry = dx >> 15;
  }
  *bad = b;
}

__device__ __forceinline__ int wave_sum_i(int v) {
#pragma unroll
  for (int o = 32; o > 0; o >>= 1) v += __shfl_xor(v, o, 64);
  return v;
}

__device__ __forceinline__ void wave_lds_sync() { asm volatile("s_waitcnt lgkmcnt(0)" ::: "memory"); }

struct Text {
  const uint8_t* g;
  const uint8_t* l;
  int lbase, lo, hi;
  __device__ __forceinline__ unsigned at(int q) const {
    return (q >= lo && q < hi) ? (unsigned)l[q - lbase] : (unsigned)g[q];
  }
};


__device__ __forceinline__ void limbs_mul(uint32_t* N, int* nl, uint32_t m) {
  uint64_t carry = 0;
  for (int i = 0; i < *nl; ++i) {
    const uint64_t v = (uint64_t)N[i] * m + carry;
    N[i] = (uint32_t)(v % 1000000000ull);
    carry = v / 1000000000ull;
  }
  while (carry) {
    N[(*nl)++] = (uint32_t)(carry % 1000000000ull);
    carry /= 1000000000ull;
  }
}

__device__ __noinline__ int cmp_token_dyadic(const Text& t, int i0, int end, uint64_t K, int E) {
  uint32_t N[16];
  int nl = 0, s = 0;
  for (uint64_t k = K; k || nl == 0; k /= 1000000000ull) N[nl++] = (uint32_t)(k % 1000000000ull);
  if (E >= 0) {
    for (int k = E; k > 0; k -= 29) limbs_mul(N, &nl, 1u << (k < 29 ? k : 29));
  } else {
    s = -E;
    for (int k = s; k > 0; k -= 13) {
      uint32_t p = 1;
      for (int j = 0; j < (k < 13 ? k : 13); ++j) p *= 5u;
      limbs_mul(N, &nl, p);
    }
  }
  int top = 1;
  for (uint32_t v = N[nl - 1]; v >= 10; v /= 10) ++top;
  const int nd = 9 * (nl - 1) + top;
  int k = i0;
  if (t.at(k) == '-') ++k;
  int int_sig = 0, lead_zeros = 0, first = -1;
  unsigned c = k < end ? t.at(k) : 0u;
  for (; c >= '0' && c <= '9'; c = ++k < end ? t.at(k) : 0u)
    if (first >= 0 || c != '0') {
      if (first < 0) first = k;
      ++int_sig;
    }
  if (c == '.')
    for (c = ++k < end ? t.at(k) : 0u; c >= '0' && c <= '9'; c = ++k < end ? t.at(k) : 0u)
      if (first < 0) {
        if (c == '0') ++lead_zeros;
        else first = k;
      }
  int ex = 0;
  if (c == 'e' || c == 'E') {
    c = ++k < end ? t.at(k) : 0u;
    const bool eneg = c == '-';
    if (c == '+' || c == '-') c = ++k < end ? t.at(k) : 0u;
    for (; c >= '0' && c <= '9'; c = ++k < end ? t.at(k) : 0u)
      if (ex < 100000) ex = ex * 10 + (int)(c - '0');
    if (eneg) ex = -ex;
  }
  if (first < 0) return -1;
  const int Lx = (int_sig > 0 ? int_sig : -lead_zeros) + ex, Lm = nd - s;
  if (Lx != Lm) return Lx > Lm ? 1 : -1;
  int j = nd - 1;
  for (k = first; k < end; ++k) {
    c = t.at(k);
    if (c == '.') continue;
    if (c < '0' || c > '9') break;
    int dm = 0;
    if (j >= 0) {
      uint32_t v = N[j / 9];
      for (int r = j % 9; r > 0; --r) v /= 10;
      dm = (int)(v % 10);
    }
    const int dx = (int)(c - '0');
    if (dx != dm) return dx > dm ? 1 : -1;
    --j;
  }
  for (; j >= 0; --j) {
    uint32_t v = N[j / 9];
    for (int r = j % 9; r > 0; --r) v /= 10;
    if (v % 10) return -1;
  }
  return 0;
}

__device__ __forceinline__ int cmp_x_dyadic(uint64_t w, int q, bool sticky, uint64_t K, int E,
                                            const Text* tok, int i0, int end) {
  const int c = cmp_decimal_dyadic(w, q, K, E);
  if (!sticky) return c;
  if (c >= 0) return 1;
  if (cmp_decimal_dyadic(w + 1, q, K, E) <= 0) return -1;
  return cmp_token_dyadic(*tok, i0, end, K, E);
}

__device__ __forceinline__ void f32_split(float f, uint64_t* M, int* e) {
  const uint32_t b = __float_as_uint(f);
  const uint32_t ex = (b >> 23) & 0xff, fr = b & 0x7fffff;
  if (ex == 0xff) { *M = 1u << 24; *e = 104; }
  else if (ex == 0) { *M = fr; *e = -149; }
  else { *M = fr | 0x800000u; *e = (int)ex - 150; }
}

__device__ __forceinline__ float f32_join(uint64_t M, int e) {
  if (M >= (1u << 24)) { M >>= 1; ++e; }
  if (e > 104) return __uint_as_float(0x7f800000u);
  if (M < (1u << 23)) return __uint_as_float((uint32_t)M);
  return __uint_as_float(((uint32_t)(e + 150) << 23) | ((uint32_t)M & 0x7fffff));
}

__device__ float exact_f32(uint64_t w, int q, bool sticky, double d, const Text* tok, int i0,
                          int end) {
  float f = (float)d;
  uint64_t M;
  int e;
  f32_split(f, &M, &e);
  for (int it = 0; it < 4; ++it) {
    if (M < (1u << 24)) {
      const int c = cmp_x_dyadic(w, q, sticky, 2 * M + 1, e - 1, tok, i0, end);
      if (c > 0 || (c == 0 && (M & 1))) {
        ++M;
        if (M == (1u << 24) && e < 104) { M = 1u << 23; ++e; }
        continue;
      }
    }
    if (M > 0) {
      uint64_t Mp = M - 1;
      int ep = e;
      if (M == (1u << 23) && e > -149) { Mp = (1u << 24) - 1; ep = e - 1; }
      if (M == (1u << 24)) { Mp = (1u << 24) - 1; }
      const int c = cmp_x_dyadic(w, q, sticky, 2 * Mp + 1, ep - 1, tok, i0, end);
      if (c < 0 || (c == 0 && (M & 1))) {
        M = Mp;
        e = ep;
        continue;
      }
    }
    break;
  }
  return f32_join(M, e);
}

__device__ __forceinline__ float scale10(uint64_t w, int q, bool neg, bool sticky,
                                         const Text* tok = nullptr, int i0 = 0, int end = 0) {
  float r;
  if (w == 0 || q < -66) {
    r = 0.f;
  } else if (q > 39) {
    r = __uint_as_float(0x7f800000u);
  } else {
    const bool exact_in = w < (1ull << 53) && q >= -22 && q <= 22 && !sticky;
    double d = (double)w;
    if (q >= 0) {
      d = q <= 22 ? d * pow10_exact(q) : d * pow10_exact(22) * pow10_exact(q - 22);
    } else {
      int k = -q;
      while (k > 22) {
        d /= pow10_exact(22);
        k -= 22;
      }
      d /= pow10_exact(k);
    }
    r = (float)d;
    bool ambiguous = !(r < 3.4028234e38f);
    const uint64_t db = (uint64_t)__double_as_longlong(d);
    const int dexp = (int)((db >> 52) & 0x7ff);
    if (!ambiguous && exact_in && dexp >= 1023 - 126) {
      ambiguous = (db & 0x1fffffffull) == 0x10000000ull;
    } else if (!ambiguous) {
      const uint32_t rb = __float_as_uint(r);
      const double lo = 0.5 * ((double)r + (double)__uint_as_float(rb - (rb ? 1u : 0u)));
      const double hi = 0.5 * ((double)r + (double)__uint_as_float(rb + 1u));
      if (exact_in) {
        ambiguous = d == lo || d == hi;
      } else {
        const double tol = fabs(d) * 0x1p-50;
        ambiguous = fabs(d - lo) <= tol || fabs(d - hi) <= tol;
      }
    }
    if (ambiguous) r = exact_f32(w, q, sticky, d, tok, i0, end);
  }
  return neg ? -r : r;
}

__device__ float parse_number(const Text& t, int i0, int end, bool* ok, int* len) {
  int i = i0;
  bool neg = false;
  unsigned c = i < end ? t.at(i) : 0u;
  if (c == '-') { neg = true; ++i; c = i < end ? t.at(i) : 0u; }
  uint64_t mant = 0;
  int digits = 0, exp10 = 0;
  bool good = true, sticky = false;
  if (i >= end) {
    good = false;
  } else if (c == '0') {
    ++i;
    c = i < end ? t.at(i) : 0u;
    if (c >= '0' && c <= '9') good = false;
  } else if (c >= '1' && c <= '9') {
    while (c >= '0' && c <= '9') {
      if (digits < 19) { mant = mant * 10 + (c - '0'); ++digits; }
      else { ++exp10; sticky |= c != '0'; }
      ++i;
      c = i < end ? t.at(i) : 0u;
    }
  } else {
    good = false;
  }
  if (good && c == '.') {
    ++i;
    c = i < end ? t.at(i) : 0u;
    int fd = 0;
    while (c >= '0' && c <= '9') {
      if (digits < 19) {
        if (mant != 0 || c != '0') ++digits;
        mant = mant * 10 + (c - '0');
        --exp10;
      } else {
        sticky |= c != '0';
      }
      ++fd;
      ++i;
      c = i < end ? t.at(i) : 0u;
    }
    if (fd == 0) good = false;
  }
  if (good && (c == 'e' || c == 'E')) {
    ++i;
    c = i < end ? t.at(i) : 0u;
    bool eneg = false;
    if (c == '+' || c == '-') {
      eneg = c == '-';
      ++i;
      c = i < end ? t.at(i) : 0u;
    }
    int e = 0, ed = 0;
    while (c >= '0' && c <= '9') {
      if (e < 100000) e = e * 10 + (c - '0');
      ++ed;
      ++i;
      c = i < end ? t.at(i) : 0u;
    }
    if (ed == 0) good = false;
    exp10 += eneg ? -e : e;
  }
  while (i < end && !is_delim(c)) {
    good = false;
    ++i;
    c = i < end ? t.at(i) : 0u;
  }
  *ok = good;
  *len = i - i0;
  return good ? scale10(mant, exp10, neg, sticky, &t, i0, i) : 0.f;
}

__device__ __forceinline__ uint32_t udiv_rcp(uint32_t n, uint32_t d, double rd) {
  uint32_t q = (uint32_t)((double)n * rd);
  if (n - q * d >= d) ++q;
  return q;
}

struct Dims {
  uint32_t C, W, H;
  double rC, rW, rH;
};

__device__ __forceinline__ int wraps(uint32_t idx, const Dims& d) {
  const uint32_t px = udiv_rcp(idx, d.C, d.rC);
  if (idx - px * d.C) return 0;
  const uint32_t row = udiv_rcp(px, d.W, d.rW);
  if (px - row * d.W) return 1;
  return (row - udiv_rcp(row, d.H, d.rH) * d.H) ? 2 : 3;
}

__device__ bool gap_ok(const Text& t, int beg, int pos, uint32_t idx, int k) {
  int opens = 0, closes = 0, commas = 0;
  int q = pos - 1;
  for (; q >= beg; --q) {
    const unsigned c = t.at(q);
    if (is_ws(c)) continue;
    if (c == '[') {
      if (commas) return false;
      ++opens;
    } else if (c == ',') {
      if (commas) return false;
      ++commas;
    } else if (c == ']') {
      if (!commas) return false;
      ++closes;
    } else {
      break;
    }
  }
  if (idx == 0) return q < beg && opens == 4 && commas == 0 && closes == 0;
  return q >= beg && commas == 1 && opens == k && closes == k;
}

__device__ bool tail_ok(const Text& t, int pos, int end) {
  int closes = 0;
  for (int q = pos; q < end; ++q) {
    const unsigned c = t.at(q);
    if (is_ws(c)) continue;
    if (c != ']') return false;
    ++closes;
  }
  return closes == 4;
}

__device__ __forceinline__ uint32_t byte_at(uint32_t w0, uint32_t w1, uint32_t w2, uint32_t w3,
                                            int k) {
  const uint32_t lo = (k & 4) ? w1 : w0;
  const uint32_t hi = (k & 4) ? w3 : w2;
  return (((k & 8) ? hi : lo) >> ((k & 3) * 8)) & 0xFFu;
}

__device__ __forceinline__ bool parse_window(const uint8_t* text, int x, uint32_t m0, uint32_t m1,
                                             int off, float* out) {
  const uint32_t* tw = reinterpret_cast<const uint32_t*>(text) + (x >> 2);
  const uint32_t sh = (uint32_t)(x & 3);
  const uint32_t d0 = tw[0], d1 = tw[1], d2 = tw[2], d3 = tw[3], d4 = tw[4];
  const uint32_t w0 = __builtin_amdgcn_alignbyte(d1, d0, sh);
  const uint32_t w1 = __builtin_amdgcn_alignbyte(d2, d1, sh);
  const uint32_t w2 = __builtin_amdgcn_alignbyte(d3, d2, sh);
  const uint32_t w3 = __builtin_amdgcn_alignbyte(d4, d3, sh);
  const uint32_t delim = (((m1 << 16) | (m0 & 0xFFFFu)) >> off) & 0xFFFFu;
  const uint32_t D = (((m1 & 0xFFFF0000u) | (m0 >> 16)) >> off) & 0xFFFFu;
  const uint32_t tok = ~delim & 0xFFFFu;
  const int L = __builtin_ctz(~tok);
  if (L >= 16) return false;
  const int s = byte_at(w0, w1, w2, w3, 0) == '-' ? 1 : 0;
  const int ie = s + __builtin_ctz(~(D >> s));
  bool ok = ie > s && !(byte_at(w0, w1, w2, w3, s) == '0' && ie > s + 1);
  int fb = ie, fe = ie;
  if (byte_at(w0, w1, w2, w3, ie) == '.' && ie < L) {
    fb = ie + 1;
    fe = fb + __builtin_ctz(~(D >> fb));
    ok &= fe > fb;
  }
  int eb = fe, ee = fe;
  bool eneg = false;
  const uint32_t ce = byte_at(w0, w1, w2, w3, fe);
  if (fe < L && (ce == 'e' || ce == 'E')) {
    int p = fe + 1;
    const uint32_t c2 = byte_at(w0, w1, w2, w3, p);
    if (p < L && (c2 == '+' || c2 == '-')) {
      eneg = c2 == '-';
      ++p;
    }
    eb = p;
    ee = p + __builtin_ctz(~(D >> p));
    ok &= ee > eb;
  }
  if (!ok || ee != L) return false;
  const uint32_t mm = bits_range(s, ie) | bits_range(fb, fe);
  uint64_t a = 0;
  const uint32_t wd[4] = {w0, w1, w2, w3};
#pragma unroll
  for (int j = 0; j < 15; ++j) {
    const uint32_t d = ((wd[j >> 2] >> ((j & 3) * 8)) & 0xFFu) - '0';
    a = ((mm >> j) & 1u) ? a * 10u + d : a;
  }
  uint32_t e = 0;
  for (int p = eb; p < ee; ++p)
    if (e < 100000u) e = e * 10u + (byte_at(w0, w1, w2, w3, p) - '0');
  const int exp10 = (eneg ? -(int)e : (int)e) - (fe - fb);
  *out = scale10(a, exp10, s != 0, false);
  return true;
}

__device__ __forceinline__ bool gap_window(const uint8_t* text, int x, int k) {
  const uint32_t* tw = reinterpret_cast<const uint32_t*>(text) + ((x - 8) >> 2);
  const uint32_t sh = (uint32_t)(x & 3);
  const uint32_t d0 = tw[0], d1 = tw[1], d2 = tw[2];
  const uint64_t g = (uint64_t)__builtin_amdgcn_alignbyte(d2, d1, sh) << 32 |
                     __builtin_amdgcn_alignbyte(d1, d0, sh);
  const int plen = 2 * k + 1;
  const uint64_t pat = k == 0 ? 0x2Cull : k == 1 ? 0x5B2C5Dull
                     : k == 2 ? 0x5B5B2C5D5Dull : 0x5B5B5B2C5D5D5Dull;
  if ((g >> (8 * (8 - plen))) != pat) return false;
  const uint32_t prev = (uint32_t)(g >> (8 * (7 - plen))) & 0xFFu;
  return prev - '0' < 10u;
}

__device__ __forceinline__ int tile_tokens(const JsonRecord& r, int tl, const uint8_t* bytes,
                                           bool* bad) {
  const int lane = threadIdx.x & 63;
  const int64_t abeg = r.off & ~(int64_t)15;
  const uint8_t* rb = bytes + abeg;
  const int beg = (int)(r.off - abeg), end = beg + r.len;
  const int o = tl * kTile + kLaneBytes * lane;
  uint4 v[kChunks];
#pragma unroll
  for (int i = 0; i < kChunks; ++i)
    v[i] = (o + 16 * i < end) ? *reinterpret_cast<const uint4*>(rb + o + 16 * i)
                              : make_uint4(0, 0, 0, 0);
  unsigned prevb = __shfl_up(v[kChunks - 1].w >> 24, 1, 64);
  if (lane == 0 && o - 1 >= beg) prevb = rb[o - 1];
  const bool pd = (o - 1 < beg) || is_delim(prevb);
  uint32_t st[kChunks], cm[kChunks];
  token_starts(v, o, beg, end, pd, st, cm, bad);
  int lc = 0;
#pragma unroll
  for (int i = 0; i < kChunks; ++i) lc += __builtin_popcount(st[i]);
  return wave_sum_i(lc);
}

__device__ __forceinline__ int tile_tokens_packed(const JsonRecord& r, int tl, uint8_t* bytes,
                                                  const PackedText& pt, bool* bad) {
  const int lane = threadIdx.x & 63;
  const int64_t abeg = r.off & ~(int64_t)15;
  uint8_t* rb = bytes + abeg;
  const int beg = (int)(r.off - abeg), end = beg + r.len;
  const int o = tl * kTile + kLaneBytes * lane;
  uint4 v[kChunks];
#pragma unroll
  for (int i = 0; i < kChunks; ++i) {
    if (o + 16 * i < end) {
      v[i] = expand16(pt, abeg + o + 16 * i);
      *reinterpret_cast<uint4*>(rb + o + 16 * i) = v[i];
    } else {
      v[i] = make_uint4(0, 0, 0, 0);
    }
  }
  unsigned prevb = __shfl_up(v[kChunks - 1].w >> 24, 1, 64);
  if (lane == 0 && o - 1 >= beg) prevb = expand16(pt, abeg + o - 16).w >> 24;
  const bool pd = (o - 1 < beg) || is_delim(prevb);
  uint32_t st[kChunks], cm[kChunks];
  token_starts(v, o, beg, end, pd, st, cm, bad);
  int lc = 0;
#pragma unroll
  for (int i = 0; i < kChunks; ++i) lc += __builtin_popcount(st[i]);
  return wave_sum_i(lc);
}

__device__ __forceinline__ int record_tiles(const JsonRecord& r) {
  const int64_t abeg = r.off & ~(int64_t)15;
  return (int)((r.off + r.len - abeg + kTile - 1) / kTile);
}

__device__ __forceinline__ void count_tile(JsonRecord* recs, const int* tile_rec, int t,
                                           const uint8_t* bytes, int* counts, int* status) {
  const int ri = tile_rec[t];
  const JsonRecord r = recs[ri];
  if (r.has_cnt) return;
  bool bad;
  const int cnt = tile_tokens(r, t - r.tile0, bytes, &bad);
  if ((threadIdx.x & 63) == 0) counts[t] = cnt;
  if (bad) atomicMax(status ? &status[ri] : &recs[ri].status, 2);
}

template <bool PACKED>
__device__ __forceinline__ void count_group(JsonRecord* recs, const int2* groups, int g,
                                            uint8_t* bytes, const PackedText& pt, int* counts,
                                            int* gsum, int* gbad, int* lds8) {
  const int wave = threadIdx.x >> 6;
  const int2 gr = groups[g];
  const JsonRecord r = recs[gr.x];
  const int nt = record_tiles(r);
  const int tl = gr.y + wave;
  int cnt = 0;
  bool bad = false;
  if (tl < nt) {
    cnt = PACKED ? tile_tokens_packed(r, tl, bytes, pt, &bad)
                 : tile_tokens(r, tl, bytes, &bad);
    if ((threadIdx.x & 63) == 0) counts[r.tile0 + (int)r.grp0 + tl] = cnt;
    if (bad && !gbad) atomicMax(&recs[gr.x].status, 2);
    bad = __ballot(bad) != 0;
  }
  if ((threadIdx.x & 63) == 0) {
    lds8[wave] = cnt;
    lds8[kGroupTiles + wave] = bad ? 1 : 0;
  }
  __syncthreads();
  if (threadIdx.x == 0) {
    int acc = 0, nbad = 0;
#pragma unroll
    for (int w = 0; w < kGroupTiles; ++w) {
      acc += lds8[w];
      nbad += lds8[kGroupTiles + w];
    }
    counts[r.tile0 + (int)r.grp0 + nt + gr.y / kGroupTiles] = acc;
    gsum[g] = acc;
    if (gbad) gbad[g] = nbad ? 2 : 0;
  }
}

__global__ __launch_bounds__(256) void json_count_kernel(JsonRecord* recs, const int* tile_rec,
                                                         int ntiles, const uint8_t* bytes,
                                                         int* counts, const int* d_ntiles,
                                                         int* status) {
  const int t = blockIdx.x * kWaves + (threadIdx.x >> 6);
  if (d_ntiles) ntiles = min(ntiles, *d_ntiles);
  if (t >= ntiles) return;
  count_tile(recs, tile_rec, t, bytes, counts, status);
}

__device__ __forceinline__ void crc_windows_packed(const PackedText& pt, const CrcChunk* chunks,
                                                   int n, const uint32_t* T, uint32_t* out,
                                                   int block, int nblocks) {
  const int lane = threadIdx.x & 63, wave = threadIdx.x >> 6;
  for (int c = block * crc::kCrcWaves + wave; c < n; c += nblocks * crc::kCrcWaves) {
    const CrcChunk ch = chunks[c];
    const int64_t cs = ch.end - ch.len;
    const int64_t wa = ch.end - (int64_t)64 * (64 - lane);
    const int64_t hi = wa + 64;
    uint32_t crc = 0;
    if (hi > cs) {
      const int64_t b16 = wa & ~(int64_t)15;
      uint32_t w[20];
#pragma unroll
      for (int j = 0; j < 5; ++j) {
        const int64_t p = b16 + 16 * j;
        const uint4 v = (p < hi && p + 16 > cs) ? expand16(pt, p) : make_uint4(0, 0, 0, 0);
        w[4 * j] = v.x;
        w[4 * j + 1] = v.y;
        w[4 * j + 2] = v.z;
        w[4 * j + 3] = v.w;
      }
      const uint32_t sh = (uint32_t)(wa & 3);
      uint32_t x[16];
      switch ((int)((wa & 15) >> 2)) {
#define GALE_ALIGN_WORDS(D)                                                       \
  _Pragma("unroll") for (int t = 0; t < 16; ++t) x[t] =                           \
      __builtin_amdgcn_alignbyte(w[t + (D) + 1], w[t + (D)], sh);
        case 0: GALE_ALIGN_WORDS(0) break;
        case 1: GALE_ALIGN_WORDS(1) break;
        case 2: GALE_ALIGN_WORDS(2) break;
        default: GALE_ALIGN_WORDS(3) break;
#undef GALE_ALIGN_WORDS
      }
#pragma unroll
      for (int t = 0; t < 16; ++t) {
        const int64_t at = wa + 4 * t;
        uint32_t v = x[t];
        if (at + 4 <= cs) v = 0;
        else if (at < cs) v &= 0xffffffffu << (8 * (uint32_t)(cs - at));
        crc = crc::crc_word(T, crc, v);
      }
    }
    crc = crc::gf2_mulmod(crc, T[1024 + lane]);
#pragma unroll
    for (int o = 32; o > 0; o >>= 1) crc ^= __shfl_xor(crc, o, 64);
    if (lane == 0) out[c] = crc;
  }
}

static_assert(kGroupTiles == kWaves, "one tile group per counting workgroup");
template <bool PACKED>
__global__ __launch_bounds__(256) void ingest_crc_count_kernel(
    uint8_t* bytes, PackedText pt, const CrcChunk* chunks, int nchunks, const uint32_t* tables,
    uint32_t* crc_out, int crc_blocks, JsonRecord* recs, const int2* groups, int ngroups,
    int* counts, int* gsum, int* gbad) {
  __shared__ uint32_t T[crc::kTableWords];
  if ((int)blockIdx.x < crc_blocks) {
    crc::crc_stage_tables(tables, T);
    if (PACKED)
      crc_windows_packed(pt, chunks, nchunks, T, crc_out, blockIdx.x, crc_blocks);
    else
      crc::crc_windows(bytes, chunks, nchunks, T, crc_out, blockIdx.x, crc_blocks);
    return;
  }
  const int g = (int)blockIdx.x - crc_blocks;
  if (g >= ngroups) return;
  count_group<PACKED>(recs, groups, g, bytes, pt, counts, gsum, gbad, reinterpret_cast<int*>(T));
}

template <bool PREP>
__device__ __forceinline__ void json_parse_tile(JsonRecord* recs, const int* tile_rec, int ntiles,
                                                const uint8_t* bytes, int H, int W, int C,
                                                const int* counts, float* out,
                                                const int* d_ntiles, int* status, int* tile_bad,
                                                const InputPrep& prep) {
  __shared__ __attribute__((aligned(16))) uint8_t lds_text[kWaves][kText];
  __shared__ uint16_t lds_tok[kWaves][kMaxTok];
  __shared__ uint32_t lds_cm[kWaves][kTile / 16 + 1];
  const int lane = threadIdx.x & 63, wave = threadIdx.x >> 6;
  const int t = blockIdx.x * kWaves + wave;
  if (d_ntiles) ntiles = min(ntiles, *d_ntiles);
  if (t >= ntiles) return;
  uint8_t* text = lds_text[wave];
  uint16_t* tok = lds_tok[wave];
  uint32_t* cmk = lds_cm[wave];
  const int ri = tile_rec[t];
  const JsonRecord r = recs[ri];
  const int64_t abeg = r.off & ~(int64_t)15;
  const uint8_t* rb = bytes + abeg;
  const int beg = (int)(r.off - abeg), end = beg + r.len;
  const int aend = (end + 15) & ~15;
  const int per_image = H * W * C;
  int expected = r.images * per_image;
  if (r.images < 0) {
    const int* rc = reinterpret_cast<const int*>(bytes + r.cnt_off);
    const int nt = record_tiles(r);
    const int ng = (nt + kGroupTiles - 1) / kGroupTiles;
    int s = 0;
    for (int k = lane; k < ng; k += 64) s += rc[nt + k];
    const int tot = wave_sum_i(s);
    expected = (tot % per_image == 0 && tot / per_image <= r.len / (2 * per_image)) ? tot : 0;
  }
  const int tl = t - r.tile0;
  const int t0 = tl * kTile;
  const bool last_tile = t0 + kTile >= end;

  Text tx;
  tx.g = rb;
  tx.l = text;
  tx.lbase = t0 - kHalo;
  tx.lo = max(t0 - kHalo, 0);
  tx.hi = min(t0 + kTile + kHalo, aend);
  for (int q = tx.lo + 16 * lane; q < tx.hi; q += 16 * 64)
    *reinterpret_cast<uint4*>(text + (q - tx.lbase)) = *reinterpret_cast<const uint4*>(rb + q);

  int part = 0;
  if (r.has_cnt) {
    const int* rc = reinterpret_cast<const int*>(bytes + r.cnt_off);
    const int* gs = rc + record_tiles(r);
    const int gi = tl / kGroupTiles;
    for (int k = lane; k < gi; k += 64) part += gs[k];
    if (lane < tl - gi * kGroupTiles) part += rc[gi * kGroupTiles + lane];
  } else {
    for (int k = r.tile0 + lane; k < t; k += 64) part += counts[k];
  }
  const int base = wave_sum_i(part);
  wave_lds_sync();

  const int o = t0 + kLaneBytes * lane;
  uint4 v[kChunks];
#pragma unroll
  for (int i = 0; i < kChunks; ++i)
    v[i] = (o + 16 * i < end) ? *reinterpret_cast<const uint4*>(text + (o + 16 * i - tx.lbase))
                              : make_uint4(0, 0, 0, 0);
  const bool pd = (o - 1 < beg) || is_delim(text[o - 1 - tx.lbase]);
  uint32_t st[kChunks], cm[kChunks];
  bool bad_ignored;
  token_starts(v, o, beg, end, pd, st, cm, &bad_ignored);
#pragma unroll
  for (int i = 0; i < kChunks; ++i) cmk[kChunks * lane + i] = cm[i];
  if (lane == 63) {
    const int p = t0 + kTile;
    const uint4 h = p < end ? *reinterpret_cast<const uint4*>(text + (p - tx.lbase))
                            : make_uint4(0, 0, 0, 0);
    cmk[kTile / 16] = chunk_masks(classify16(h.x, h.y, h.z, h.w), p, beg, end);
  }
  int cnt = 0;
#pragma unroll
  for (int i = 0; i < kChunks; ++i) cnt += __builtin_popcount(st[i]);
  int inc = cnt;
#pragma unroll
  for (int d = 1; d < 64; d <<= 1) {
    const int u = __shfl_up(inc, d, 64);
    if (lane >= d) inc += u;
  }
  const int ntok = __shfl(inc, 63, 64);
  int li = inc - cnt;
#pragma unroll
  for (int i = 0; i < kChunks; ++i) {
    uint32_t s = st[i];
    while (s) {
      const int j = __builtin_ctz(s);
      s &= s - 1;
      tok[li++] = (uint16_t)(o + 16 * i + j - tx.lbase);
    }
  }
  wave_lds_sync();

  const bool nchw = PREP && prep.nchw;
  const int d0 = nchw ? W : C, d1 = nchw ? H : W, d2 = nchw ? C : H;
  Dims dims;
  dims.C = (uint32_t)d0; dims.W = (uint32_t)d1; dims.H = (uint32_t)d2;
  dims.rC = 1.0 / d0; dims.rW = 1.0 / d1; dims.rH = 1.0 / d2;
  float* dst = out + (int64_t)r.slot * per_image;
  int bad = 0;
  for (int j = lane; j < ntok; j += 64) {
    const int x = tok[j];
    const int pos = x + tx.lbase;
    const int idx = base + j;
    float val;
    int len = 0;
    bool ok;
    const int ci = (pos - t0) >> 4;
    if (parse_window(text, x, cmk[ci], cmk[ci + 1], pos & 15, &val)) {
      ok = true;
      len = -1;
    } else {
      ok = false;
      val = parse_number(tx, pos, end, &ok, &len);
    }
    int kn = 0;
    if (PREP) {
      const uint32_t px = udiv_rcp((uint32_t)idx, dims.C, dims.rC);
      const uint32_t i0 = (uint32_t)idx - px * dims.C;
      uint32_t sidx = (uint32_t)idx, ch = i0;
      if (prep.nchw) {
        const uint32_t row = udiv_rcp(px, dims.W, dims.rW);
        const uint32_t i1 = px - row * dims.W;
        const uint32_t img = udiv_rcp(row, dims.H, dims.rH);
        ch = row - img * dims.H;
        kn = i0 ? 0 : i1 ? 1 : ch ? 2 : 3;
        sidx = img * (uint32_t)per_image + (i1 * (uint32_t)W + i0) * (uint32_t)C + ch;
      }
      if (idx < expected) {
        const float a = ch == 0 ? prep.a[0] : ch == 1 ? prep.a[1] : ch == 2 ? prep.a[2] : prep.a[3];
        const float b = ch == 0 ? prep.b[0] : ch == 1 ? prep.b[1] : ch == 2 ? prep.b[2] : prep.b[3];
        dst[sidx] = __builtin_fmaf(val, a, b);
      }
    }
    if (!ok) {
      bad = max(bad, 2);
    } else {
      const int k = idx <= 0 ? 0 : (PREP && prep.nchw) ? kn : wraps((uint32_t)idx, dims);
      const bool fast_gap = idx > 0 && pos - 8 >= tx.lo && pos - (2 * k + 2) >= beg &&
                            gap_window(text, x, k);
      if (!fast_gap && !gap_ok(tx, beg, pos, (uint32_t)idx, k)) {
        bad = 3;
      } else if (idx == expected - 1) {
        if (len < 0) parse_number(tx, pos, end, &ok, &len);
        if (!tail_ok(tx, pos + len, end)) bad = 3;
      }
    }
    if (!PREP && idx < expected) dst[idx] = val;
  }
  if (last_tile && lane == 0 && base + ntok != expected) bad = max(bad, 1);
  if (tile_bad) {
#pragma unroll
    for (int d = 32; d > 0; d >>= 1) bad = max(bad, __shfl_xor(bad, d, 64));
    if (lane == 0) tile_bad[t] = bad;
  } else if (bad) {
    atomicMax(status ? &status[ri] : &recs[ri].status, bad);
  }
}

__global__ __launch_bounds__(256) void json_parse_kernel(JsonRecord* recs, const int* tile_rec,
                                                         int ntiles, const uint8_t* bytes, int H,
                                                         int W, int C, const int* counts,
                                                         float* out, const int* d_ntiles,
                                                         int* status, int* tile_bad) {
  json_parse_tile<false>(recs, tile_rec, ntiles, bytes, H, W, C, counts, out, d_ntiles, status,
                         tile_bad, InputPrep());
}

__global__ __launch_bounds__(256) __attribute__((amdgpu_waves_per_eu(4, 4)))
void json_parse_prep_kernel(JsonRecord* recs, const int* tile_rec, int ntiles,
                            const uint8_t* bytes, int H, int W, int C, const int* counts,
                            float* out, const int* d_ntiles, int* status, int* tile_bad,
                            InputPrep prep) {
  json_parse_tile<true>(recs, tile_rec, ntiles, bytes, H, W, C, counts, out, d_ntiles, status,
                        tile_bad, prep);
}

}



hipError_t ingest_crc_count(const uint8_t* bytes, const CrcChunk* chunks, int nchunks,
                            const uint32_t* tables, uint32_t* crc_out, int nrec, int ngroups,
                            JsonRecord* recs, const int2* groups, int* counts, int* gsum,
                            int* gbad, hipStream_t stream, const uint8_t* packed,
                            const uint32_t* tab, uint8_t* text_out) {
  if (nrec <= 0) ngroups = 0;
  int crc_blocks = (nchunks + crc::kCrcWaves - 1) / crc::kCrcWaves;
  if (crc_blocks > 1024) crc_blocks = 1024;
  if (crc_blocks + ngroups == 0) return hipSuccess;
  if (packed) {
    if (!tab || !text_out || (reinterpret_cast<uintptr_t>(packed) & 7) ||
        (reinterpret_cast<uintptr_t>(text_out) & 15))
      return hipErrorInvalidValue;
    hipLaunchKernelGGL(ingest_crc_count_kernel<true>, dim3(crc_blocks + ngroups), dim3(256), 0,
                       stream, text_out, PackedText{packed, tab}, chunks, nchunks, tables,
                       crc_out, crc_blocks, recs, groups, ngroups, counts, gsum, gbad);
  } else {
    hipLaunchKernelGGL(ingest_crc_count_kernel<false>, dim3(crc_blocks + ngroups), dim3(256), 0,
                       stream, const_cast<uint8_t*>(bytes), PackedText{nullptr, nullptr}, chunks,
                       nchunks, tables, crc_out, crc_blocks, recs, groups, ngroups, counts, gsum,
                       gbad);
  }
  return hipGetLastError();
}

hipError_t json_parse_instances(int nrec, int ntiles, JsonRecord* recs, const int* tile_rec,
                                const uint8_t* bytes, int H, int W, int C, int* tile_counts,
                                float* out, hipStream_t stream, bool count_pass,
                                const int* d_ntiles, int* status, int* tile_bad,
                                const InputPrep* prep) {
  if (nrec <= 0 || ntiles <= 0) return hipSuccess;
  if (H <= 0 || W <= 0 || C <= 0) return hipErrorInvalidValue;
  const bool with_prep = prep && !prep->identity();
  if (with_prep) {
    if ((int64_t)H * W * C >= (1 << 20)) return hipErrorInvalidValue;
    if (C > 4)
      for (int i = 1; i < 4; ++i)
        if (prep->a[i] != prep->a[0] || prep->b[i] != prep->b[0]) return hipErrorInvalidValue;
  }
  if (tile_bad && count_pass) return hipErrorInvalidValue;
  const int blocks = (ntiles + kWaves - 1) / kWaves;
  if (count_pass)
    hipLaunchKernelGGL(json_count_kernel, dim3(blocks), dim3(64 * kWaves), 0, stream, recs,
                       tile_rec, ntiles, bytes, tile_counts, d_ntiles, status);
  if (with_prep)
    hipLaunchKernelGGL(json_parse_prep_kernel, dim3(blocks), dim3(64 * kWaves), 0, stream, recs,
                       tile_rec, ntiles, bytes, H, W, C, tile_counts, out, d_ntiles, status,
                       tile_bad, *prep);
  else
    hipLaunchKernelGGL(json_parse_kernel, dim3(blocks), dim3(64 * kWaves), 0, stream, recs,
                       tile_rec, ntiles, bytes, H, W, C, tile_counts, out, d_ntiles, status,
                       tile_bad);
  return hipGetLastError();
}

}
```

### csrc/runtime/gpu_ingest.cpp

```cpp
#include "gpu_ingest.h"
#include "metrics.h"

#include <stdlib.h>
#include <string.h>

#include <chrono>
#include <stdexcept>
#include <thread>

#include "../codec/json_codec.h"
#include "gale/executor.h"
#include "replica.h"

namespace gale {

GpuIngest::GpuIngest(int device, int lanes, int poll_us)
    : device_(device), poll_us_(poll_us), shift_chunk_(kCrcChunkBytes) {
  check_hip(hipSetDevice(device_), "ingest: hipSetDevice");
  std::vector<uint32_t> t(kafka::kCrcDeviceTableWords);
  kafka::crc32c_device_tables(t.data());
  check_hip(hipMalloc(reinterpret_cast<void**>(&d_tables_), t.size() * 4), "ingest: tables");
  check_hip(hipMemcpy(d_tables_, t.data(), t.size() * 4, hipMemcpyHostToDevice),
            "ingest: tables H2D");
  for (int i = 0; i < std::max(1, lanes); ++i) {
    auto L = std::make_unique<Lane>();
    check_hip(hipStreamCreateWithFlags(&L->stream, hipStreamNonBlocking), "ingest: stream");
    check_hip(hipEventCreateWithFlags(&L->done, hipEventDisableTiming), "ingest: event");
    lanes_.push_back(std::move(L));
  }
  if (const char* e = getenv("GALE_INGEST_DEV_TIMING")) dev_every_ = std::max(0, atoi(e));
  if (const char* e = getenv("GALE_INGEST_PLAN_SEPARATE")) plan_separate_ = atoi(e) != 0;
  if (dev_every_ > 0)
    for (auto& L : lanes_)
      for (hipEvent_t& ev : L->tev) check_hip(hipEventCreate(&ev), "ingest: timing event");
}

GpuIngest::~GpuIngest() {
  hipSetDevice(device_);
  for (auto& L : lanes_) {
    if (L->stream) hipStreamSynchronize(L->stream);
    if (L->h_io) hipHostFree(L->h_io);
    if (L->d_io) hipFree(L->d_io);
    if (L->d_counts) hipFree(L->d_counts);
    if (L->done) hipEventDestroy(L->done);
    for (hipEvent_t ev : L->tev)
      if (ev) hipEventDestroy(ev);
    if (L->stream) hipStreamDestroy(L->stream);
  }
  if (d_tables_) hipFree(d_tables_);
}

void GpuIngest::grow(Lane& L, size_t io_bytes, size_t tiles) {
  check_hip(hipSetDevice(device_), "ingest: hipSetDevice");
  auto up = [](size_t want, size_t have) {
    return (std::max(want, have * 2) + 4095) & ~(size_t)4095;
  };
  if (io_bytes > L.io_cap) {
    if (L.h_io) hipHostFree(L.h_io);
    if (L.d_io) hipFree(L.d_io);
    L.io_cap = up(io_bytes, L.io_cap);
    check_hip(hipMalloc(reinterpret_cast<void**>(&L.d_io), L.io_cap), "ingest: d_io");
    check_hip(hipHostMalloc(reinterpret_cast<void**>(&L.h_io), L.io_cap, hipHostMallocMapped),
              "ingest: h_io");
    void* dp = nullptr;
    check_hip(hipHostGetDevicePointer(&dp, L.h_io, 0), "ingest: h_io device pointer");
    if (dp != L.h_io) throw std::runtime_error("ingest: mapped plan buffer has another address");
  }
  if (tiles * sizeof(int) > L.counts_cap) {
    if (L.d_counts) hipFree(L.d_counts);
    L.counts_cap = up(tiles * sizeof(int), L.counts_cap);
    check_hip(hipMalloc(reinterpret_cast<void**>(&L.d_counts), L.counts_cap), "ingest: counts");
  }
}

void GpuIngest::wait(Lane& L) {
  if (poll_us_ <= 0) {
    check_hip(hipEventSynchronize(L.done), "ingest: hipEventSynchronize");
    return;
  }
  for (;;) {
    const hipError_t e = hipEventQuery(L.done);
    if (e == hipSuccess) return;
    if (e != hipErrorNotReady) check_hip(e, "ingest: hipEventQuery");
    std::this_thread::sleep_for(std::chrono::microseconds(poll_us_));
  }
}

void GpuIngest::mark(Lane& L, const Stamps& ts, int k) {
  if (ts.timed) check_hip(hipEventRecord(L.tev[k], L.stream), "ingest: timing event");
}

void GpuIngest::begin(Lane& L, Stamps& ts, const kafka::Fetched& f, uint8_t* dev,
                      const Transfer& t) {
  hipStream_t st = L.stream;
  ts.plan = mono_ns();
  ts.timed = dev_every_ > 0 && L.nrun++ % dev_every_ == 0;
  mark(L, ts, 0);
  if (t.tab_bytes) memcpy(t.hpl, t.tab, t.tab_bytes);
  const bool has_plan = t.plan_bytes > 0;
  if (t.in_chunk && has_plan) {
    check_hip(hipMemcpyAsync(dev + t.lo, f.buf.get() + t.lo, t.plan_off + t.plan_bytes - t.lo,
                             hipMemcpyHostToDevice, st),
              "ingest: H2D text + plan");
  } else {
    check_hip(hipMemcpyAsync(dev + t.lo, f.buf.get() + t.lo, t.len, hipMemcpyHostToDevice, st),
              "ingest: H2D text");
    if (has_plan)
      check_hip(hipMemcpyAsync(L.d_io, L.h_io, t.plan_bytes, hipMemcpyHostToDevice, st),
                "ingest: H2D plan");
  }
  plan_in_chunk_ += t.in_chunk && has_plan;
  mark(L, ts, 1);
  text_bytes_ += (int64_t)t.text_bytes;
  link_bytes_ += (int64_t)t.link_bytes;
}

int64_t GpuIngest::end(Lane& L, const Stamps& ts, bool parsed) {
  mark(L, ts, 3);
  check_hip(hipEventRecord(L.done, L.stream), "ingest: event");
  const int64_t t_wait = mono_ns();
  wait(L);
  const int64_t t_post = mono_ns();
  ++runs_;
  prep_ns_ += t_wait - ts.start;
  plan_ns_ += ts.plan - ts.start;
  wait_ns_ += t_post - t_wait;
  if (ts.timed) {
    float ms[3] = {0.f, 0.f, 0.f};
    for (int k = 0; k < (parsed ? 3 : 2); ++k)
      check_hip(hipEventElapsedTime(&ms[k], L.tev[k], L.tev[k + 1]), "ingest: event time");
    ++dev_runs_;
    dev_copy_ns_ += (int64_t)(ms[0] * 1e6);
    dev_count_ns_ += (int64_t)(ms[1] * 1e6);
    dev_parse_ns_ += (int64_t)(ms[2] * 1e6);
    dev_wait_ns_ += t_post - t_wait;
  }
  return t_post;
}

void GpuIngest::join_batch_crcs(const kafka::Fetched& f,
                                const std::vector<std::pair<size_t, size_t>>& batch_chunks,
                                const uint32_t* crc, IngestIO& io) {
  for (size_t b = 0; b < batch_chunks.size(); ++b) {
    const kafka::BatchSpan& bs = f.batches[b];
    uint32_t raw = 0;
    for (size_t k = 0; k < batch_chunks[b].second; ++k) {
      const uint32_t c = crc[batch_chunks[b].first + k];
      raw = k == 0 ? c : shift_chunk_(raw) ^ c;
    }
    const uint64_t len = bs.len - (size_t)kafka::kBatchAttrOffset;
    const uint32_t got = raw ^ kafka::crc32c_shift(0xffffffffu, len) ^ 0xffffffffu;
    kafka::Reader cr(f.buf.get() + bs.off + kafka::kBatchCrcOffset, 4);
    io.batch_ok[b] = got == cr.u32();
  }
}

void GpuIngest::run_b64(int lane, const kafka::Fetched& f, uint8_t* dev, size_t dev_cap,
                        bool check_crcs, int H, int W, int C, IngestIO& io, float* arena,
                        size_t arena_bytes) {
  Lane& L = *lanes_[(size_t)lane % lanes_.size()];
  std::lock_guard<std::mutex> lk(L.mu);
  Stamps ts;
  ts.start = mono_ns();
  const size_t nrec_all = f.records.size();
  io.cnt_off.assign(nrec_all, -1);
  io.batch_ok.assign(f.batches.size(), 1);
  io.img.assign(nrec_all, nullptr);
  std::vector<std::pair<int64_t, int64_t>> batches;
  for (const kafka::BatchSpan& b : f.batches) batches.emplace_back((int64_t)b.off, (int64_t)b.len);
  std::vector<B64PlanRecord> recs(nrec_all);
  for (size_t i = 0; i < nrec_all; ++i) {
    const kafka::RecordRef& rr = f.records[i];
    B64PlanRecord& r = recs[i];
    r.status = io.status[i];
    r.images = io.images[i];
    r.value_off = rr.value_off;
    r.value_len = rr.value_len;
    r.arr_off = io.arr_off[i];
  }
  B64IngestPlan plan;
  plan_b64_ingest(batches, kafka::kBatchAttrOffset, check_crcs, recs, io.b64_offs, H, W, C,
                  arena ? arena_bytes : 0, f.size, plan);
  const size_t nc = plan.chunks.size(), ni = plan.imgs.size();
  if (nc == 0 && plan.ok_records == 0) return;
  grow(L, plan.plan_bytes + plan.result_bytes + 16, 1);
  Transfer t;
  t.lo = plan.c_lo;
  t.len = t.text_bytes = t.link_bytes = plan.c_len;
  t.plan_off = plan.plan_off;
  t.plan_bytes = plan.plan_bytes;
  t.in_chunk = !plan_separate_ && t.plan_off + plan.plan_bytes <= dev_cap;
  t.hpl = t.in_chunk ? f.buf.get() + t.plan_off : L.h_io;
  const uint8_t* dpl = t.in_chunk ? dev + t.plan_off : L.d_io;
  if (nc) memcpy(t.hpl + plan.o_chunks, plan.chunks.data(), nc * sizeof(CrcChunk));
  if (ni) memcpy(t.hpl + plan.o_imgs, plan.imgs.data(), ni * sizeof(B64Image));
  uint8_t* res = L.h_io + plan.plan_bytes;
  int* wg_bad = reinterpret_cast<int*>(res + plan.o_bad);
  begin(L, ts, f, dev, t);
  check_hip(ingest_crc_b64(dev, reinterpret_cast<const CrcChunk*>(dpl + plan.o_chunks), (int)nc,
                           d_tables_, reinterpret_cast<uint32_t*>(res + plan.o_crc), (int)ni,
                           reinterpret_cast<const B64Image*>(dpl + plan.o_imgs), H, W, C, arena,
                           wg_bad, L.stream, &input_prep_),
            "ingest: crc32c + b64 decode");
  mark(L, ts, 2);
  const int64_t t_post = end(L, ts, false);
  join_batch_crcs(f, plan.batch_chunks, reinterpret_cast<const uint32_t*>(res + plan.o_crc), io);
  const int64_t per = (int64_t)H * W * C;
  const int cpi = plan.chunks_per_image;
  for (size_t i = 0; i < nrec_all; ++i) {
    if (plan.img0[i] < 0) continue;
    const int* w = wg_bad + (size_t)plan.img0[i] * cpi;
    int v = 0;
    for (int64_t g = 0; g < (int64_t)io.images[i] * cpi; ++g) v = std::max(v, w[g]);
    if (v == 2) io.status[i] = codec::BAD_NUMBER;
    else io.img[i] = arena + (int64_t)plan.slot0[i] * per;
  }
  post_ns_ += mono_ns() - t_post;
}

void GpuIngest::run(int lane, const kafka::Fetched& f, uint8_t* dev, size_t dev_cap,
                    bool check_crcs, int H, int W, int C, IngestIO& io, float* arena,
                    size_t arena_bytes) {
  Lane& L = *lanes_[(size_t)lane % lanes_.size()];
  std::lock_guard<std::mutex> lk(L.mu);
  Stamps ts;
  ts.start = mono_ns();
  const size_t nrec_all = f.records.size();
  io.images.assign(nrec_all, 0);
  io.cnt_off.assign(nrec_all, -1);
  io.batch_ok.assign(f.batches.size(), 1);
  io.img.assign(nrec_all, nullptr);
  L.batches.clear();
  for (const kafka::BatchSpan& b : f.batches)
    L.batches.emplace_back((int64_t)b.off, (int64_t)b.len);
  L.recs.resize(nrec_all);
  for (size_t i = 0; i < nrec_all; ++i) {
    const kafka::RecordRef& rr = f.records[i];
    JsonPlanRecord& r = L.recs[i];
    r.status = io.status[i];
    r.value_off = rr.value_off;
    r.value_len = rr.value_len;
    r.arr_off = io.arr_off[i];
    r.arr_len = io.arr_len[i];
  }
  const JsonIngestPlan& p = L.plan;
  plan_json_ingest(L.batches, kafka::kBatchAttrOffset, check_crcs, L.recs, H, W, C,
                   arena ? arena_bytes : 0, f.size, dev_cap, f.tap_result, plan_separate_, L.plan);
  if (p.empty()) return;
  const size_t nc = p.nc(), nr = p.nr(), np = p.np();
  grow(L, p.io_bytes + 16, (size_t)p.ntiles + (size_t)p.ngroups + 1);
  uint8_t* hpl = p.plan_in_chunk ? f.buf.get() + p.plan_off : L.h_io;
  uint8_t* dpl = p.plan_in_chunk ? dev + p.plan_off : L.d_io;
  fill_json_ingest(p, L.recs, hpl);
  const JsonRecord* hr = reinterpret_cast<const JsonRecord*>(hpl + p.o_recs);
  const JsonRecord* hp = reinterpret_cast<const JsonRecord*>(hpl + p.o_precs);
  Transfer t;
  t.lo = p.c_lo;
  t.len = p.c_len;
  t.plan_off = p.plan_off;
  t.plan_bytes = p.o_gsum;
  t.in_chunk = p.plan_in_chunk;
  t.hpl = hpl;
  if (p.packed) {
    t.tab = f.buf.get() + p.tab_off;
    t.tab_bytes = p.ng * 2 * sizeof(uint32_t);
  }
  t.text_bytes = p.span;
  t.link_bytes = p.link;
  begin(L, ts, f, dev, t);
  uint32_t* d_crc = reinterpret_cast<uint32_t*>(L.h_io + p.o_crc);
  int* d_gsum = reinterpret_cast<int*>(L.h_io + p.o_gsum);
  int* d_gbad = reinterpret_cast<int*>(L.h_io + p.o_gbad);
  int* d_pbad = reinterpret_cast<int*>(L.h_io + p.o_pbad);
  int* d_cnt = p.cnt_base >= 0 ? reinterpret_cast<int*>(dev + p.cnt_base) : L.d_counts;
  check_hip(ingest_crc_count(dev, reinterpret_cast<const CrcChunk*>(dpl + p.o_chunks), (int)nc,
                             d_tables_, d_crc, (int)nr, p.ngroups,
                             reinterpret_cast<JsonRecord*>(dpl + p.o_recs),
                             reinterpret_cast<const int2*>(dpl + p.o_groups), d_cnt, d_gsum,
                             d_gbad, L.stream, p.packed ? dev + p.c_lo : nullptr,
                             p.packed ? reinterpret_cast<const uint32_t*>(dpl) : nullptr,
                             p.packed ? dev : nullptr),
            "ingest: crc32c + count");
  mark(L, ts, 2);
  if (np > 0)
    check_hip(json_parse_instances((int)np, p.ptiles,
                                   reinterpret_cast<JsonRecord*>(dpl + p.o_precs),
                                   reinterpret_cast<const int*>(dpl + p.o_ptr), dev, H, W, C,
                                   L.d_counts, arena, L.stream, false, nullptr,
                                   nullptr, d_pbad, &input_prep_),
              "ingest: parse");
  const int64_t t_post = end(L, ts, true);
  join_batch_crcs(f, p.batch_chunks, d_crc, io);
  size_t k = 0;
  for (size_t j = 0; j < nr; ++j) {
    const size_t i = (size_t)p.rec_of[j];
    const bool parsed = k < np && (size_t)p.pjs[k] == j;
    const JsonRecord* pr = parsed ? &hp[k++] : nullptr;
    const int64_t g1 = j + 1 < nr ? hr[j + 1].grp0 : p.ngroups;
    int64_t tok = 0;
    int bad = 0;
    for (int64_t g = hr[j].grp0; g < g1; ++g) {
      tok += d_gsum[g];
      bad |= d_gbad[g];
    }
    if (bad != 0) {
      io.status[i] = codec::BAD_NUMBER;
    } else if (tok == 0) {
      io.status[i] = codec::EMPTY;
    } else if (tok % p.per != 0) {
      io.status[i] = codec::BAD_SHAPE;
    } else {
      io.images[i] = (int32_t)(tok / p.per);
      if (p.cnt_base >= 0) io.cnt_off[i] = p.cnt_off(hr[j]);
      if (pr) {
        const int nt = json_tile_count(pr->off, pr->len);
        int v = 0;
        for (int t0 = 0; t0 < nt; ++t0) v = std::max(v, d_pbad[pr->tile0 + t0]);
        const int32_t verdict = device_verdict_status(v);
        if (verdict != codec::OK) io.status[i] = verdict;
        else io.img[i] = arena + (int64_t)pr->slot * p.per;
      }
    }
  }
  post_ns_ += mono_ns() - t_post;
}

}
```

### csrc/runtime/gpu_ingest.h

```cpp
#pragma once
#include <hip/hip_runtime.h>

#include <atomic>
#include <memory>
#include <mutex>
#include <utility>
#include <vector>

#include "gale/kernels.h"
#include "ingest.h"
#include "ingest_plan.h"

namespace gale {

class GpuIngest : public Ingest {
 public:
  GpuIngest(int device, int lanes, int poll_us);
  ~GpuIngest() override;
  int device() const override { return device_; }
  void run(int lane, const kafka::Fetched& f, uint8_t* dev, size_t dev_cap, bool check_crcs,
           int H, int W, int C, IngestIO& io, float* arena = nullptr,
           size_t arena_bytes = 0) override;
  void run_b64(int lane, const kafka::Fetched& f, uint8_t* dev, size_t dev_cap, bool check_crcs,
               int H, int W, int C, IngestIO& io, float* arena = nullptr,
               size_t arena_bytes = 0) override;
  void link_bytes(int64_t& text, int64_t& link) const override {
    text = text_bytes_.load();
    link = link_bytes_.load();
  }
  void set_input_prep(const InputPrep& p) { input_prep_ = p; }
  Timing timing() const override {
    Timing t;
    t.runs = runs_.load();
    t.prep_ns = prep_ns_.load();
    t.plan_ns = plan_ns_.load();
    t.wait_ns = wait_ns_.load();
    t.post_ns = post_ns_.load();
    t.dev_runs = dev_runs_.load();
    t.dev_copy_ns = dev_copy_ns_.load();
    t.dev_count_ns = dev_count_ns_.load();
    t.dev_parse_ns = dev_parse_ns_.load();
    t.dev_wait_ns = dev_wait_ns_.load();
    t.plan_in_chunk = plan_in_chunk_.load();
    return t;
  }

 private:
  struct Lane {
    std::mutex mu;
    hipStream_t stream = nullptr;
    hipEvent_t done = nullptr;
    uint8_t* h_io = nullptr;
    uint8_t* d_io = nullptr;
    size_t io_cap = 0;
    int* d_counts = nullptr;
    size_t counts_cap = 0;
    hipEvent_t tev[4] = {nullptr, nullptr, nullptr, nullptr};
    int64_t nrun = 0;
    std::vector<std::pair<int64_t, int64_t>> batches;
    std::vector<JsonPlanRecord> recs;
    JsonIngestPlan plan;
  };
  struct Transfer {
    size_t lo = 0, len = 0;
    size_t plan_off = 0, plan_bytes = 0;
    bool in_chunk = false;
    uint8_t* hpl = nullptr;
    const uint8_t* tab = nullptr;
    size_t tab_bytes = 0;
    size_t text_bytes = 0, link_bytes = 0;
  };
  struct Stamps {
    int64_t start = 0, plan = 0;
    bool timed = false;
  };
  void grow(Lane& L, size_t io_bytes, size_t tiles);
  void wait(Lane& L);
  void begin(Lane& L, Stamps& ts, const kafka::Fetched& f, uint8_t* dev, const Transfer& t);
  void mark(Lane& L, const Stamps& ts, int k);
  int64_t end(Lane& L, const Stamps& ts, bool parsed);
  void join_batch_crcs(const kafka::Fetched& f,
                       const std::vector<std::pair<size_t, size_t>>& batch_chunks,
                       const uint32_t* crc, IngestIO& io);
  int device_, poll_us_;
  InputPrep input_prep_;
  std::atomic<int64_t> text_bytes_{0}, link_bytes_{0};
  std::atomic<int64_t> runs_{0}, prep_ns_{0}, plan_ns_{0}, wait_ns_{0}, post_ns_{0};
  std::atomic<int64_t> dev_runs_{0}, dev_copy_ns_{0}, dev_count_ns_{0}, dev_parse_ns_{0},
      dev_wait_ns_{0};
  int dev_every_ = 0;
  bool plan_separate_ = false;
  std::atomic<int64_t> plan_in_chunk_{0};
  uint32_t* d_tables_ = nullptr;
  std::vector<std::unique_ptr<Lane>> lanes_;
  kafka::CrcShift shift_chunk_;
};

}
```

### csrc/runtime/ingest_plan.cpp

```cpp
#include "ingest_plan.h"

#include <string.h>

#include <algorithm>
#include <stdexcept>

#include "../codec/text_pack.h"

namespace gale {

namespace {

size_t align16(size_t n) { return (n + 15) & ~(size_t)15; }
size_t align256(size_t n) { return (n + 255) & ~(size_t)255; }

void plan_batches(const std::vector<std::pair<int64_t, int64_t>>& batches, int64_t attr_off,
                  bool check_crcs, size_t fetch_size, std::vector<CrcChunk>& chunks,
                  std::vector<std::pair<size_t, size_t>>& batch_chunks, size_t& lo, size_t& hi) {
  for (const auto& b : batches) {
    if (b.first < 0 || b.second < 0 || (uint64_t)b.first + (uint64_t)b.second > fetch_size)
      throw std::invalid_argument("ingest plan: batch outside the fetch");
    lo = std::min(lo, (size_t)b.first);
    hi = std::max(hi, (size_t)(b.first + b.second));
    if (!check_crcs) continue;
    const size_t first = chunks.size();
    const size_t n = append_crc_windows(b.first + attr_off, b.first + b.second, chunks);
    batch_chunks.emplace_back(first, n);
  }
}

int64_t image_elements(int H, int W, int C) {
  if (H <= 0 || W <= 0 || C <= 0) throw std::invalid_argument("ingest plan: bad image shape");
  const int64_t per = (int64_t)H * W * C;
  if (per > (1 << 30)) throw std::invalid_argument("ingest plan: image too large");
  return per;
}

}

size_t append_crc_windows(int64_t rs, int64_t re, std::vector<CrcChunk>& chunks) {
  const int64_t len = re - rs;
  if (len <= 0) return 0;
  const int64_t n = (len + kCrcChunkBytes - 1) / kCrcChunkBytes;
  for (int64_t k = 0; k < n; ++k) {
    CrcChunk c;
    c.end = re - (int64_t)kCrcChunkBytes * (n - 1 - k);
    c.len = k == 0 ? (int32_t)(len - (int64_t)kCrcChunkBytes * (n - 1)) : kCrcChunkBytes;
    c.pad_ = 0;
    chunks.push_back(c);
  }
  return (size_t)n;
}

void plan_json_ingest(const std::vector<std::pair<int64_t, int64_t>>& batches, int64_t attr_off,
                      bool check_crcs, const std::vector<JsonPlanRecord>& recs, int H, int W,
                      int C, size_t arena_bytes, size_t fetch_size, size_t dev_cap,
                      int64_t tap_result, bool plan_separate, JsonIngestPlan& out) {
  {
    JsonIngestPlan fresh;
    fresh.chunks.swap(out.chunks);
    fresh.batch_chunks.swap(out.batch_chunks);
    fresh.rec_of.swap(out.rec_of);
    fresh.pjs.swap(out.pjs);
    fresh.chunks.clear();
    fresh.batch_chunks.clear();
    fresh.rec_of.clear();
    fresh.pjs.clear();
    out = std::move(fresh);
  }
  const int64_t per = out.per = image_elements(H, W, C);
  size_t lo = fetch_size, hi = 0;
  plan_batches(batches, attr_off, check_crcs, fetch_size, out.chunks, out.batch_chunks, lo, hi);
  for (size_t i = 0; i < recs.size(); ++i) {
    const JsonPlanRecord& r = recs[i];
    if (r.status != 0) continue;
    if (r.value_off < 0 || r.value_len < 0 || r.arr_off < 0 || r.arr_len < 0 ||
        r.arr_len > 0x7fffffffll ||
        (uint64_t)r.value_off + (uint64_t)r.value_len > fetch_size)
      throw std::invalid_argument("ingest plan: record outside the fetch");
    if ((uint64_t)r.arr_off + (uint64_t)r.arr_len > (uint64_t)r.value_len)
      throw std::invalid_argument("ingest plan: array outside its record");
    out.rec_of.push_back((int)i);
    const int nt = json_tile_count(r.value_off + r.arr_off, (int32_t)r.arr_len);
    out.ntiles += nt;
    out.ngroups += (nt + kGroupTiles - 1) / kGroupTiles;
    lo = std::min(lo, (size_t)r.value_off);
    hi = std::max(hi, (size_t)(r.value_off + r.value_len));
  }
  if (out.empty()) return;
  const size_t nc = out.nc(), nr = out.nr();
  out.packed = tap_result >= 0;
  if (out.packed) {
    lo = 0;
    hi = fetch_size;
  }
  lo &= ~(size_t)15;
  const size_t span = hi - lo;
  out.lo = lo;
  out.span = span;
  out.ng = out.packed ? codec::pack_groups(span) : 0;
  out.link = out.packed ? (size_t)tap_result : span;
  out.c_lo = out.packed ? codec::pack_offset(span) : lo;
  out.c_len = out.link;
  out.tab_off = out.packed ? codec::tab_offset(span) : 0;
  out.used = out.c_lo + out.c_len;
  if (out.used > dev_cap) throw std::invalid_argument("ingest plan: the copy ends past the mirror");
  const size_t ncnt = (size_t)out.ntiles + (size_t)out.ngroups;
  if (out.ntiles > 0) {
    const size_t cb = align256(ncnt * sizeof(int));
    if (dev_cap > cb + 256 && ((dev_cap - cb) & ~(size_t)255) >= align256(out.used + 64))
      out.cnt_base = (int64_t)((dev_cap - cb) & ~(size_t)255);
  }
  if (arena_bytes > 0 && out.cnt_base >= 0) {
    const int64_t S = 2 * per;
    for (size_t j = 0; j < nr; ++j) {
      const JsonPlanRecord& r = recs[(size_t)out.rec_of[j]];
      const int64_t off = r.value_off + r.arr_off;
      const int64_t slot = (off + S - 1) / S, cap = r.arr_len / S;
      if (cap <= 0 || (slot + cap) * per * (int64_t)sizeof(float) > (int64_t)arena_bytes) continue;
      out.pjs.push_back((int)j);
      out.ptiles += json_tile_count(off, (int32_t)r.arr_len);
    }
  }
  const size_t np = out.np(), ngroups = (size_t)out.ngroups, ptiles = (size_t)out.ptiles;
  out.o_chunks = align16(out.ng * 2 * sizeof(uint32_t));
  out.o_groups = out.o_chunks + align16(nc * sizeof(CrcChunk));
  out.o_recs = out.o_groups + align16(ngroups * sizeof(int2));
  out.o_precs = out.o_recs + nr * sizeof(JsonRecord);
  out.o_ptr = out.o_precs + np * sizeof(JsonRecord);
  out.o_gsum = out.o_ptr + align16(ptiles * sizeof(int));
  out.o_crc = out.o_gsum + align16(ngroups * 4);
  out.o_gbad = out.o_crc + align16(nc * 4);
  out.o_pbad = out.o_gbad + align16(ngroups * 4);
  out.io_bytes = out.o_pbad + align16(ptiles * 4);
  out.plan_off = align256(std::max(fetch_size, out.used));
  const size_t plan_lim = out.cnt_base >= 0 ? (size_t)out.cnt_base : dev_cap;
  const bool on_tab = out.packed && out.plan_off < out.tab_off + out.ng * 2 * sizeof(uint32_t) &&
                      out.tab_off < out.plan_off + out.o_gsum;
  out.plan_in_chunk = !plan_separate && !on_tab && out.plan_off + out.o_gsum <= plan_lim;
}

void fill_json_ingest(const JsonIngestPlan& p, const std::vector<JsonPlanRecord>& recs,
                      uint8_t* dst) {
  const size_t nc = p.nc(), nr = p.nr(), np = p.np();
  if (nc) memcpy(dst + p.o_chunks, p.chunks.data(), nc * sizeof(CrcChunk));
  int2* hg = reinterpret_cast<int2*>(dst + p.o_groups);
  JsonRecord* hr = reinterpret_cast<JsonRecord*>(dst + p.o_recs);
  int tile = 0, grp = 0;
  for (size_t j = 0; j < nr; ++j) {
    const JsonPlanRecord& r = recs[(size_t)p.rec_of[j]];
    JsonRecord& jr = hr[j];
    jr.off = r.value_off + r.arr_off;
    jr.len = (int32_t)r.arr_len;
    jr.slot = 0;
    jr.images = 0;
    jr.status = 0;
    jr.tile0 = tile;
    jr.has_cnt = 0;
    jr.cnt_off = 0;
    jr.grp0 = grp;
    const int nt = json_tile_count(jr.off, jr.len);
    for (int t0 = 0; t0 < nt; t0 += kGroupTiles) {
      hg[grp].x = (int)j;
      hg[grp].y = t0;
      ++grp;
    }
    tile += nt;
  }
  JsonRecord* hp = reinterpret_cast<JsonRecord*>(dst + p.o_precs);
  int* hpt = reinterpret_cast<int*>(dst + p.o_ptr);
  const int64_t S = 2 * p.per;
  int pt = 0;
  for (size_t k = 0; k < np; ++k) {
    const JsonRecord& jr = hr[p.pjs[k]];
    JsonRecord& pr = hp[k];
    pr = jr;
    pr.slot = (int32_t)((jr.off + S - 1) / S);
    pr.images = -1;
    pr.status = 0;
    pr.tile0 = pt;
    pr.has_cnt = 1;
    pr.cnt_off = p.cnt_off(jr);
    pr.grp0 = 0;
    const int nt = json_tile_count(pr.off, pr.len);
    for (int t = 0; t < nt; ++t) hpt[pt + t] = (int)k;
    pt += nt;
  }
}

void plan_b64_ingest(const std::vector<std::pair<int64_t, int64_t>>& batches, int64_t attr_off,
                     bool check_crcs, const std::vector<B64PlanRecord>& recs,
                     const std::vector<uint32_t>& offs, int H, int W, int C, size_t arena_bytes,
                     size_t fetch_size, B64IngestPlan& out) {
  out = B64IngestPlan();
  const int64_t per = image_elements(H, W, C);
  const int64_t L = 4 * ((per + 2) / 3);
  out.chunks_per_image = (int)((L + kB64ChunkChars - 1) / kB64ChunkChars);
  size_t lo = fetch_size, hi = 0;
  plan_batches(batches, attr_off, check_crcs, fetch_size, out.chunks, out.batch_chunks, lo, hi);
  out.slot0.assign(recs.size(), -1);
  out.img0.assign(recs.size(), -1);
  size_t next_off = 0;
  int64_t next_slot = 0;
  bool cut = false;
  for (size_t i = 0; i < recs.size(); ++i) {
    const B64PlanRecord& r = recs[i];
    if (r.status != 0) continue;
    if (r.images <= 0 || r.value_off < 0 || r.value_len < 0 || r.arr_off < 0 ||
        r.arr_off > r.value_len || (uint64_t)r.value_off + (uint64_t)r.value_len > fetch_size)
      throw std::invalid_argument("b64 ingest plan: record outside the fetch");
    if (offs.size() - next_off < (size_t)r.images)
      throw std::invalid_argument("b64 ingest plan: fewer string offsets than images");
    ++out.ok_records;
    lo = std::min(lo, (size_t)r.value_off);
    hi = std::max(hi, (size_t)(r.value_off + r.value_len));
    const uint32_t* ro = offs.data() + next_off;
    next_off += (size_t)r.images;
    for (int32_t k = 0; k < r.images; ++k)
      if (r.arr_off + (int64_t)ro[k] + L > r.value_len)
        throw std::invalid_argument("b64 ingest plan: string outside its record");
    if (!cut && ((uint64_t)(next_slot + r.images) * (uint64_t)per * sizeof(float) > arena_bytes ||
                 next_slot + r.images > 0x7fffffffll))
      cut = true;
    if (cut) continue;
    out.slot0[i] = (int32_t)next_slot;
    out.img0[i] = (int32_t)out.imgs.size();
    for (int32_t k = 0; k < r.images; ++k) {
      B64Image d;
      d.off = r.value_off + r.arr_off + (int64_t)ro[k];
      d.slot = (int32_t)(next_slot + k);
      d.rec = (int32_t)i;
      out.imgs.push_back(d);
    }
    next_slot += r.images;
  }
  if (hi < lo) lo = hi = 0;
  out.lo = lo;
  out.hi = hi;
  out.c_lo = lo & ~(size_t)15;
  out.c_len = hi - out.c_lo;
  out.plan_off = align256(fetch_size);
  const size_t nc = out.chunks.size(), ni = out.imgs.size();
  out.o_chunks = 0;
  out.o_imgs = out.o_chunks + align16(nc * sizeof(CrcChunk));
  out.plan_bytes = out.o_imgs + align16(ni * sizeof(B64Image));
  out.o_crc = 0;
  out.o_bad = out.o_crc + align16(nc * sizeof(uint32_t));
  out.result_bytes = out.o_bad + align16(ni * (size_t)out.chunks_per_image * sizeof(int32_t));
}

}
```

### csrc/runtime/ingest_plan.h

```cpp
#pragma once
#include <stddef.h>
#include <stdint.h>

#include <utility>
#include <vector>

#include "gale/kernels.h"

namespace gale {

size_t append_crc_windows(int64_t rs, int64_t re, std::vector<CrcChunk>& chunks);


struct JsonPlanRecord {
  int32_t status = 0;
  int64_t value_off = 0;
  int64_t value_len = 0;
  int64_t arr_off = 0;
  int64_t arr_len = 0;
};

struct JsonIngestPlan {
  std::vector<CrcChunk> chunks;
  std::vector<std::pair<size_t, size_t>> batch_chunks;
  std::vector<int> rec_of;
  std::vector<int> pjs;
  int ntiles = 0, ngroups = 0;
  int ptiles = 0;
  bool packed = false;
  size_t lo = 0, span = 0, link = 0, ng = 0;
  size_t c_lo = 0, c_len = 0;
  size_t tab_off = 0;
  size_t used = 0;
  int64_t cnt_base = -1;
  size_t o_chunks = 0, o_groups = 0, o_recs = 0, o_precs = 0, o_ptr = 0;
  size_t o_gsum = 0;
  size_t o_crc = 0, o_gbad = 0, o_pbad = 0, io_bytes = 0;
  size_t plan_off = 0;
  bool plan_in_chunk = false;
  int64_t per = 0;

  size_t nc() const { return chunks.size(); }
  size_t nr() const { return rec_of.size(); }
  size_t np() const { return pjs.size(); }
  bool empty() const { return chunks.empty() && rec_of.empty(); }
  int64_t cnt_off(const JsonRecord& r) const {
    return cnt_base + ((int64_t)r.tile0 + r.grp0) * (int64_t)sizeof(int);
  }
};

void plan_json_ingest(const std::vector<std::pair<int64_t, int64_t>>& batches, int64_t attr_off,
                      bool check_crcs, const std::vector<JsonPlanRecord>& recs, int H, int W,
                      int C, size_t arena_bytes, size_t fetch_size, size_t dev_cap,
                      int64_t tap_result, bool plan_separate, JsonIngestPlan& out);

void fill_json_ingest(const JsonIngestPlan& plan, const std::vector<JsonPlanRecord>& recs,
                      uint8_t* dst);


struct B64PlanRecord {
  int32_t status = 0;
  int32_t images = 0;
  int64_t value_off = 0;
  int64_t value_len = 0;
  int64_t arr_off = 0;
};

struct B64IngestPlan {
  std::vector<CrcChunk> chunks;
  std::vector<std::pair<size_t, size_t>> batch_chunks;
  std::vector<B64Image> imgs;
  std::vector<int32_t> slot0;
  std::vector<int32_t> img0;
  int chunks_per_image = 1;
  size_t lo = 0, hi = 0;
  size_t c_lo = 0, c_len = 0;
  size_t plan_off = 0;
  size_t ok_records = 0;
  size_t o_chunks = 0, o_imgs = 0, plan_bytes = 0;
  size_t o_crc = 0, o_bad = 0, result_bytes = 0;
};

void plan_b64_ingest(const std::vector<std::pair<int64_t, int64_t>>& batches, int64_t attr_off,
                     bool check_crcs, const std::vector<B64PlanRecord>& recs,
                     const std::vector<uint32_t>& offs, int H, int W, int C, size_t arena_bytes,
                     size_t fetch_size, B64IngestPlan& out);

}
```

Before: 2.149 million.

## Fuse CRC, token count and parse into one kernel for small JSON records

Adds a fused ingest path. Small JSON records (up to a fixed tile cap, with arena slots that fit) are routed to a single kernel that counts tokens per tile in LDS, computes prefix bases, and parses and writes floats in one launch. This replaces the separate count, group-sum and parse passes and avoids the host round trip between them. The cost is extra LDS per block, a cap on record size, and more complex planning and verdict settling. Whether it runs by default depends on the fuse_waves setting in the runtime, which is only partly visible.

```diff
diff --git a/csrc/bindings/host_bindings.cpp b/csrc/bindings/host_bindings.cpp
--- a/csrc/bindings/host_bindings.cpp
+++ b/csrc/bindings/host_bindings.cpp
@@ -487,7 +487,7 @@
         [](std::vector<std::pair<int64_t, int64_t>> batches,
            std::vector<std::tuple<int, int64_t, int64_t, int64_t, int64_t>> recs, int H, int W,
            int C, size_t arena_bytes, size_t fetch_size, size_t dev_cap, int64_t tap_result,
-           bool plan_separate, bool check_crcs) {
+           bool plan_separate, bool check_crcs, int fuse_waves) {
           std::vector<JsonPlanRecord> rs(recs.size());
           for (size_t i = 0; i < recs.size(); ++i) {
             rs[i].status = std::get<0>(recs[i]);
@@ -498,7 +498,7 @@
           }
           JsonIngestPlan p;
           plan_json_ingest(batches, kafka::kBatchAttrOffset, check_crcs, rs, H, W, C, arena_bytes,
-                           fetch_size, dev_cap, tap_result, plan_separate, p);
+                           fetch_size, dev_cap, tap_result, plan_separate, p, fuse_waves);
           std::string plan(p.o_gsum, '\0');
           if (!p.empty()) fill_json_ingest(p, rs, reinterpret_cast<uint8_t*>(&plan[0]));
           py::list windows;
@@ -537,13 +537,21 @@
           out["io_bytes"] = p.io_bytes;
           out["plan_off"] = p.plan_off;
           out["plan_in_chunk"] = p.plan_in_chunk;
+          out["fused"] = py::cast(p.fused);
+          out["nf"] = p.nf();
+          out["fchunks"] = p.fchunks;
+          out["fuse_waves"] = p.fuse_waves;
+          out["o_frecs"] = p.o_frecs;
+          out["o_fchunks"] = p.o_fchunks;
+          out["o_ftot"] = p.o_ftot;
+          out["o_fbad"] = p.o_fbad;
           out["plan"] = py::bytes(plan);
           return out;
         },
         py::arg("batches"), py::arg("recs"), py::arg("H"), py::arg("W"), py::arg("C"),
         py::arg("arena_bytes"), py::arg("fetch_size"), py::arg("dev_cap"),
         py::arg("tap_result") = (int64_t)-1, py::arg("plan_separate") = false,
-        py::arg("check_crcs") = true,
+        py::arg("check_crcs") = true, py::arg("fuse_waves") = 0,
         "The host plan of a JSON fetch's device ingest, laid out and filled "
         "(csrc/runtime/ingest_plan.h)");
   m.def("plan_batch",
diff --git a/csrc/bindings/module.cpp b/csrc/bindings/module.cpp
--- a/csrc/bindings/module.cpp
+++ b/csrc/bindings/module.cpp
@@ -324,6 +324,34 @@
         "groups: int32 (record, first tile) pairs, GROUP_TILES tiles each; counts: per record "
         "tile0 + grp0 -> [tile counts][group sums]; gsum: one int per group");
   m.attr("GROUP_TILES") = gale::kGroupTiles;
+  m.def("ingest_crc_parse",
+        [](uintptr_t bytes, uintptr_t chunks, int nchunks, uintptr_t tables, uintptr_t crc_out,
+           int nrec, int nfchunks, uintptr_t recs, uintptr_t fchunks, int H, int W, int C,
+           uintptr_t arena, uintptr_t rtot, uintptr_t cbad, uintptr_t stream, uintptr_t packed,
+           uintptr_t tab, std::optional<std::vector<float>> a,
+           std::optional<std::vector<float>> b, bool nchw, int waves) {
+          const auto prep = prep_from("ingest_crc_parse", a, b, nchw);
+          chk(gale::ingest_crc_parse(static_cast<uint8_t*>(P(bytes)),
+                                     static_cast<const gale::CrcChunk*>(P(chunks)), nchunks,
+                                     static_cast<const uint32_t*>(P(tables)),
+                                     static_cast<uint32_t*>(P(crc_out)), nrec, nfchunks,
+                                     static_cast<const gale::JsonRecord*>(P(recs)),
+                                     static_cast<const int2*>(P(fchunks)), H, W, C,
+                                     static_cast<float*>(P(arena)), static_cast<int2*>(P(rtot)),
+                                     static_cast<int*>(P(cbad)), S(stream),
+                                     static_cast<const uint8_t*>(P(packed)),
+                                     static_cast<const uint32_t*>(P(tab)),
+                                     prep ? &*prep : nullptr, waves),
+              "ingest_crc_parse");
+        },
+        py::arg("bytes"), py::arg("chunks"), py::arg("nchunks"), py::arg("tables"),
+        py::arg("crc_out"), py::arg("nrec"), py::arg("nfchunks"), py::arg("recs"),
+        py::arg("fchunks"), py::arg("H"), py::arg("W"), py::arg("C"), py::arg("arena"),
+        py::arg("rtot"), py::arg("cbad"), py::arg("stream"), py::arg("packed") = 0,
+        py::arg("tab") = 0, py::arg("a") = py::none(), py::arg("b") = py::none(),
+        py::arg("nchw") = false, py::arg("waves") = 0);
+  m.attr("FUSED_MAX_TILES") = gale::kFusedMaxTiles;
+  m.attr("FUSED_WAVES") = gale::kFusedWaves;
   m.def("ingest_crc_b64",
         [](uintptr_t bytes, uintptr_t chunks, int nchunks, uintptr_t tables, uintptr_t crc_out,
            int images, uintptr_t imgs, int H, int W, int C, uintptr_t arena, uintptr_t wg_bad,
diff --git a/csrc/include/gale/kernels.h b/csrc/include/gale/kernels.h
--- a/csrc/include/gale/kernels.h
+++ b/csrc/include/gale/kernels.h
@@ -258,6 +258,18 @@
                             int* gbad, hipStream_t stream, const uint8_t* packed = nullptr,
                             const uint32_t* tab = nullptr, uint8_t* text_out = nullptr);
 
+constexpr int kFusedMaxTiles = 32;
+constexpr int kFusedWaves = 8;
+inline int json_fused_chunks(int64_t off, int32_t len, int waves = kFusedWaves) {
+  return (json_tile_count(off, len) + waves - 1) / waves;
+}
+hipError_t ingest_crc_parse(uint8_t* bytes, const CrcChunk* chunks, int nchunks,
+                            const uint32_t* tables, uint32_t* crc_out, int nrec, int nfchunks,
+                            const JsonRecord* recs, const int2* fchunks, int H, int W, int C,
+                            float* out, int2* rtot, int* cbad, hipStream_t stream,
+                            const uint8_t* packed = nullptr, const uint32_t* tab = nullptr,
+                            const InputPrep* prep = nullptr, int waves = 0);
+
 hipError_t ingest_crc_b64(const uint8_t* bytes, const CrcChunk* chunks, int nchunks,
                           const uint32_t* tables, uint32_t* crc_out, int images,
                           const B64Image* imgs, int H, int W, int C, float* arena, int* wg_bad,
diff --git a/csrc/kernels/json_parse.hip b/csrc/kernels/json_parse.hip
--- a/csrc/kernels/json_parse.hip
+++ b/csrc/kernels/json_parse.hip
@@ -115,6 +115,19 @@
   }
 };
 
+struct PackedView {
+  PackedText pt;
+  int64_t abeg;
+  const uint8_t* l;
+  int lbase, lo, hi;
+  __device__ __forceinline__ unsigned at(int q) const {
+    if (q >= lo && q < hi) return (unsigned)l[q - lbase];
+    const uint4 v = expand16(pt, abeg + (q & ~15));
+    const uint32_t w = (q & 8) ? ((q & 4) ? v.w : v.z) : ((q & 4) ? v.y : v.x);
+    return (w >> ((q & 3) * 8)) & 0xFFu;
+  }
+};
+
 
 __device__ __forceinline__ void limbs_mul(uint32_t* N, int* nl, uint32_t m) {
   uint64_t carry = 0;
@@ -129,7 +142,8 @@
   }
 }
 
-__device__ __noinline__ int cmp_token_dyadic(const Text& t, int i0, int end, uint64_t K, int E) {
+template <class TX>
+__device__ __noinline__ int cmp_token_dyadic(const TX& t, int i0, int end, uint64_t K, int E) {
   uint32_t N[16];
   int nl = 0, s = 0;
   for (uint64_t k = K; k || nl == 0; k /= 1000000000ull) N[nl++] = (uint32_t)(k % 1000000000ull);
@@ -196,8 +210,9 @@
   return 0;
 }
 
+template <class TX>
 __device__ __forceinline__ int cmp_x_dyadic(uint64_t w, int q, bool sticky, uint64_t K, int E,
-                                            const Text* tok, int i0, int end) {
+                                            const TX* tok, int i0, int end) {
   const int c = cmp_decimal_dyadic(w, q, K, E);
   if (!sticky) return c;
   if (c >= 0) return 1;
@@ -220,7 +235,8 @@
   return __uint_as_float(((uint32_t)(e + 150) << 23) | ((uint32_t)M & 0x7fffff));
 }
 
-__device__ float exact_f32(uint64_t w, int q, bool sticky, double d, const Text* tok, int i0,
+template <class TX>
+__device__ float exact_f32(uint64_t w, int q, bool sticky, double d, const TX* tok, int i0,
                           int end) {
   float f = (float)d;
   uint64_t M;
@@ -252,8 +268,9 @@
   return f32_join(M, e);
 }
 
+template <class TX = Text>
 __device__ __forceinline__ float scale10(uint64_t w, int q, bool neg, bool sticky,
-                                         const Text* tok = nullptr, int i0 = 0, int end = 0) {
+                                         const TX* tok = nullptr, int i0 = 0, int end = 0) {
   float r;
   if (w == 0 || q < -66) {
     r = 0.f;
@@ -294,7 +311,8 @@
   return neg ? -r : r;
 }
 
-__device__ float parse_number(const Text& t, int i0, int end, bool* ok, int* len) {
+template <class TX>
+__device__ float parse_number(const TX& t, int i0, int end, bool* ok, int* len) {
   int i = i0;
   bool neg = false;
   unsigned c = i < end ? t.at(i) : 0u;
@@ -384,7 +402,8 @@
   return (row - udiv_rcp(row, d.H, d.rH) * d.H) ? 2 : 3;
 }
 
-__device__ bool gap_ok(const Text& t, int beg, int pos, uint32_t idx, int k) {
+template <class TX>
+__device__ bool gap_ok(const TX& t, int beg, int pos, uint32_t idx, int k) {
   int opens = 0, closes = 0, commas = 0;
   int q = pos - 1;
   for (; q >= beg; --q) {
@@ -407,7 +426,8 @@
   return q >= beg && commas == 1 && opens == k && closes == k;
 }
 
-__device__ bool tail_ok(const Text& t, int pos, int end) {
+template <class TX>
+__device__ bool tail_ok(const TX& t, int pos, int end) {
   int closes = 0;
   for (int q = pos; q < end; ++q) {
     const unsigned c = t.at(q);
@@ -493,6 +513,19 @@
   return prev - '0' < 10u;
 }
 
+__device__ __forceinline__ int count_loaded(const uint4 (&v)[kChunks], unsigned prev0, int o,
+                                            int beg, int end, bool* bad) {
+  unsigned prevb = __shfl_up(v[kChunks - 1].w >> 24, 1, 64);
+  if ((threadIdx.x & 63) == 0) prevb = prev0;
+  const bool pd = (o - 1 < beg) || is_delim(prevb);
+  uint32_t st[kChunks], cm[kChunks];
+  token_starts(v, o, beg, end, pd, st, cm, bad);
+  int lc = 0;
+#pragma unroll
+  for (int i = 0; i < kChunks; ++i) lc += __builtin_popcount(st[i]);
+  return wave_sum_i(lc);
+}
+
 __device__ __forceinline__ int tile_tokens(const JsonRecord& r, int tl, const uint8_t* bytes,
                                            bool* bad) {
   const int lane = threadIdx.x & 63;
@@ -505,17 +538,12 @@
   for (int i = 0; i < kChunks; ++i)
     v[i] = (o + 16 * i < end) ? *reinterpret_cast<const uint4*>(rb + o + 16 * i)
                               : make_uint4(0, 0, 0, 0);
-  unsigned prevb = __shfl_up(v[kChunks - 1].w >> 24, 1, 64);
-  if (lane == 0 && o - 1 >= beg) prevb = rb[o - 1];
-  const bool pd = (o - 1 < beg) || is_delim(prevb);
-  uint32_t st[kChunks], cm[kChunks];
-  token_starts(v, o, beg, end, pd, st, cm, bad);
-  int lc = 0;
-#pragma unroll
-  for (int i = 0; i < kChunks; ++i) lc += __builtin_popcount(st[i]);
-  return wave_sum_i(lc);
-}
-
+  unsigned prev0 = 0;
+  if (lane == 0 && o - 1 >= beg) prev0 = rb[o - 1];
+  return count_loaded(v, prev0, o, beg, end, bad);
+}
+
+template <bool STORE = true>
 __device__ __forceinline__ int tile_tokens_packed(const JsonRecord& r, int tl, uint8_t* bytes,
                                                   const PackedText& pt, bool* bad) {
   const int lane = threadIdx.x & 63;
@@ -528,20 +556,14 @@
   for (int i = 0; i < kChunks; ++i) {
     if (o + 16 * i < end) {
       v[i] = expand16(pt, abeg + o + 16 * i);
-      *reinterpret_cast<uint4*>(rb + o + 16 * i) = v[i];
+      if (STORE) *reinterpret_cast<uint4*>(rb + o + 16 * i) = v[i];
     } else {
       v[i] = make_uint4(0, 0, 0, 0);
     }
   }
-  unsigned prevb = __shfl_up(v[kChunks - 1].w >> 24, 1, 64);
-  if (lane == 0 && o - 1 >= beg) prevb = expand16(pt, abeg + o - 16).w >> 24;
-  const bool pd = (o - 1 < beg) || is_delim(prevb);
-  uint32_t st[kChunks], cm[kChunks];
-  token_starts(v, o, beg, end, pd, st, cm, bad);
-  int lc = 0;
-#pragma unroll
-  for (int i = 0; i < kChunks; ++i) lc += __builtin_popcount(st[i]);
-  return wave_sum_i(lc);
+  unsigned prev0 = 0;
+  if (lane == 0 && o - 1 >= beg) prev0 = expand16(pt, abeg + o - 16).w >> 24;
+  return count_loaded(v, prev0, o, beg, end, bad);
 }
 
 __device__ __forceinline__ int record_tiles(const JsonRecord& r) {
@@ -675,6 +697,12 @@
   if (g >= ngroups) return;
   count_group<PACKED>(recs, groups, g, bytes, pt, counts, gsum, gbad, reinterpret_cast<int*>(T));
 }
+
+template <bool PREP, class TX>
+__device__ __forceinline__ int parse_staged_tile(const TX& tx, const uint8_t* text, uint16_t* tok,
+                                                 uint32_t* cmk, int slot, int beg, int end, int t0,
+                                                 int base, int expected, int H, int W, int C,
+                                                 float* out, const InputPrep& prep);
 
 template <bool PREP>
 __device__ __forceinline__ void json_parse_tile(JsonRecord* recs, const int* tile_rec, int ntiles,
@@ -711,7 +739,6 @@
   }
   const int tl = t - r.tile0;
   const int t0 = tl * kTile;
-  const bool last_tile = t0 + kTile >= end;
 
   Text tx;
   tx.g = rb;
@@ -734,7 +761,25 @@
   }
   const int base = wave_sum_i(part);
   wave_lds_sync();
-
+  int bad = parse_staged_tile<PREP>(tx, text, tok, cmk, r.slot, beg, end, t0, base, expected, H,
+                                    W, C, out, prep);
+  if (tile_bad) {
+#pragma unroll
+    for (int d = 32; d > 0; d >>= 1) bad = max(bad, __shfl_xor(bad, d, 64));
+    if (lane == 0) tile_bad[t] = bad;
+  } else if (bad) {
+    atomicMax(status ? &status[ri] : &recs[ri].status, bad);
+  }
+}
+
+template <bool PREP, class TX>
+__device__ __forceinline__ int parse_staged_tile(const TX& tx, const uint8_t* text, uint16_t* tok,
+                                                 uint32_t* cmk, int slot, int beg, int end, int t0,
+                                                 int base, int expected, int H, int W, int C,
+                                                 float* out, const InputPrep& prep) {
+  const int lane = threadIdx.x & 63;
+  const int per_image = H * W * C;
+  const bool last_tile = t0 + kTile >= end;
   const int o = t0 + kLaneBytes * lane;
   uint4 v[kChunks];
 #pragma unroll
@@ -780,7 +825,7 @@
   Dims dims;
   dims.C = (uint32_t)d0; dims.W = (uint32_t)d1; dims.H = (uint32_t)d2;
   dims.rC = 1.0 / d0; dims.rW = 1.0 / d1; dims.rH = 1.0 / d2;
-  float* dst = out + (int64_t)r.slot * per_image;
+  float* dst = out + (int64_t)slot * per_image;
   int bad = 0;
   for (int j = lane; j < ntok; j += 64) {
     const int x = tok[j];
@@ -832,13 +877,122 @@
     if (!PREP && idx < expected) dst[idx] = val;
   }
   if (last_tile && lane == 0 && base + ntok != expected) bad = max(bad, 1);
-  if (tile_bad) {
+  return bad;
+}
+
+template <int NW, bool PACKED, bool PREP>
+__device__ __forceinline__ void ingest_parse_chunk(uint8_t* bytes, const PackedText& pt,
+                                                   const JsonRecord* recs, const int2* fchunks,
+                                                   int g, int H, int W, int C, float* out,
+                                                   int2* rtot, int* cbad, const InputPrep& prep,
+                                                   int* lds) {
+  __shared__ __attribute__((aligned(16))) uint8_t lds_text[NW][kText];
+  __shared__ uint16_t lds_tok[NW][kMaxTok];
+  __shared__ uint32_t lds_cm[NW][kTile / 16 + 1];
+  int* cnts = lds;
+  int* bads = lds + kFusedMaxTiles;
+  int* verd = lds + 2 * kFusedMaxTiles;
+  const int lane = threadIdx.x & 63, wave = threadIdx.x >> 6;
+  const int2 ch = fchunks[g];
+  const JsonRecord r = recs[ch.x];
+  const int nt = record_tiles(r);
+  if (nt > kFusedMaxTiles) {
+    if (threadIdx.x == 0) cbad[g] = 3;
+    return;
+  }
+  for (int tk = wave; tk < nt; tk += NW) {
+    bool tbad;
+    const int cnt = PACKED ? tile_tokens_packed<false>(r, tk, bytes, pt, &tbad)
+                           : tile_tokens(r, tk, bytes, &tbad);
+    const bool wbad = __ballot(tbad) != 0;
+    if (lane == 0) {
+      cnts[tk] = cnt;
+      bads[tk] = wbad ? 1 : 0;
+    }
+  }
+  const int64_t abeg = r.off & ~(int64_t)15;
+  uint8_t* rb = bytes + abeg;
+  const int beg = (int)(r.off - abeg), end = beg + r.len;
+  const int aend = (end + 15) & ~15;
+  const int tl = ch.y + wave;
+  const int t0 = tl * kTile;
+  const int lbase = t0 - kHalo, lo = max(t0 - kHalo, 0);
+  const int hi = tl < nt ? min(t0 + kTile + kHalo, aend) : 0;
+  uint8_t* text = lds_text[wave];
+  for (int q = lo + 16 * lane; q < hi; q += 16 * 64) {
+    const uint4 v = PACKED ? expand16(pt, abeg + q) : *reinterpret_cast<const uint4*>(rb + q);
+    *reinterpret_cast<uint4*>(text + (q - lbase)) = v;
+    if (PACKED && q >= t0 && q < t0 + kTile) *reinterpret_cast<uint4*>(rb + q) = v;
+  }
+  __syncthreads();
+  int bad = 0;
+  if (tl < nt) {
+    const int c = lane < nt ? cnts[lane] : 0;
+    const int tot = wave_sum_i(c);
+    const int base = wave_sum_i(lane < tl ? c : 0);
+    const int per_image = H * W * C;
+    const int expected =
+        (tot % per_image == 0 && tot / per_image <= r.len / (2 * per_image)) ? tot : 0;
+    if (wave == 0 && ch.y == 0) {
+      const bool rbad = __ballot(lane < nt && bads[lane] != 0) != 0;
+      if (lane == 0) rtot[ch.x] = make_int2(tot, rbad ? 2 : 0);
+    }
+    if (PACKED) {
+      PackedView tx;
+      tx.pt = pt;
+      tx.abeg = abeg;
+      tx.l = text;
+      tx.lbase = lbase;
+      tx.lo = lo;
+      tx.hi = hi;
+      bad = parse_staged_tile<PREP>(tx, text, lds_tok[wave], lds_cm[wave], r.slot, beg, end, t0,
+                                    base, expected, H, W, C, out, prep);
+    } else {
+      Text tx;
+      tx.g = rb;
+      tx.l = text;
+      tx.lbase = lbase;
+      tx.lo = lo;
+      tx.hi = hi;
+      bad = parse_staged_tile<PREP>(tx, text, lds_tok[wave], lds_cm[wave], r.slot, beg, end, t0,
+                                    base, expected, H, W, C, out, prep);
+    }
 #pragma unroll
     for (int d = 32; d > 0; d >>= 1) bad = max(bad, __shfl_xor(bad, d, 64));
-    if (lane == 0) tile_bad[t] = bad;
-  } else if (bad) {
-    atomicMax(status ? &status[ri] : &recs[ri].status, bad);
-  }
+  }
+  if (lane == 0) verd[wave] = bad;
+  __syncthreads();
+  if (threadIdx.x == 0) {
+    int v = 0;
+#pragma unroll
+    for (int w = 0; w < NW; ++w) v = max(v, verd[w]);
+    cbad[g] = v;
+  }
+}
+
+template <int NW, bool PACKED, bool PREP>
+__global__ __launch_bounds__(64 * NW) __attribute__((amdgpu_waves_per_eu(4, 4)))
+void ingest_crc_parse_kernel(uint8_t* bytes, PackedText pt, const CrcChunk* chunks, int nchunks,
+                             const uint32_t* tables, uint32_t* crc_out, int crc_blocks,
+                             const JsonRecord* recs, const int2* fchunks, int nfchunks, int H,
+                             int W, int C, float* out, int2* rtot, int* cbad, InputPrep prep) {
+  __shared__ uint32_t T[crc::kTableWords];
+  static_assert(2 * kFusedMaxTiles + NW <= crc::kTableWords && kFusedMaxTiles <= 64 &&
+                    NW >= crc::kCrcWaves,
+                "the count words fit the table area; one lane per tile in the prefix");
+  if ((int)blockIdx.x < crc_blocks) {
+    crc::crc_stage_tables(tables, T);
+    if ((int)(threadIdx.x >> 6) >= crc::kCrcWaves) return;
+    if (PACKED)
+      crc_windows_packed(pt, chunks, nchunks, T, crc_out, blockIdx.x, crc_blocks);
+    else
+      crc::crc_windows(bytes, chunks, nchunks, T, crc_out, blockIdx.x, crc_blocks);
+    return;
+  }
+  const int g = (int)blockIdx.x - crc_blocks;
+  if (g >= nfchunks) return;
+  ingest_parse_chunk<NW, PACKED, PREP>(bytes, pt, recs, fchunks, g, H, W, C, out, rtot, cbad,
+                                       prep, reinterpret_cast<int*>(T));
 }
 
 __global__ __launch_bounds__(256) void json_parse_kernel(JsonRecord* recs, const int* tile_rec,
@@ -888,6 +1042,63 @@
   return hipGetLastError();
 }
 
+namespace {
+
+template <int NW>
+void launch_crc_parse(bool packed, bool with_prep, int blocks, hipStream_t stream, uint8_t* bytes,
+                      PackedText pt, const CrcChunk* chunks, int nchunks, const uint32_t* tables,
+                      uint32_t* crc_out, int crc_blocks, const JsonRecord* recs,
+                      const int2* fchunks, int nfchunks, int H, int W, int C, float* out,
+                      int2* rtot, int* cbad, const InputPrep& prep) {
+#define GALE_CRC_PARSE(PACKED, PREP)                                                           \
+  hipLaunchKernelGGL((ingest_crc_parse_kernel<NW, PACKED, PREP>), dim3(blocks), dim3(64 * NW), \
+                     0, stream, bytes, pt, chunks, nchunks, tables, crc_out, crc_blocks, recs, \
+                     fchunks, nfchunks, H, W, C, out, rtot, cbad, prep)
+  if (packed && with_prep) GALE_CRC_PARSE(true, true);
+  else if (packed) GALE_CRC_PARSE(true, false);
+  else if (with_prep) GALE_CRC_PARSE(false, true);
+  else GALE_CRC_PARSE(false, false);
+#undef GALE_CRC_PARSE
+}
+
+}
+
+hipError_t ingest_crc_parse(uint8_t* bytes, const CrcChunk* chunks, int nchunks,
+                            const uint32_t* tables, uint32_t* crc_out, int nrec, int nfchunks,
+                            const JsonRecord* recs, const int2* fchunks, int H, int W, int C,
+                            float* out, int2* rtot, int* cbad, hipStream_t stream,
+                            const uint8_t* packed, const uint32_t* tab, const InputPrep* prep,
+                            int waves) {
+  if (nrec <= 0) nfchunks = 0;
+  int crc_blocks = (nchunks + crc::kCrcWaves - 1) / crc::kCrcWaves;
+  if (crc_blocks > 1024) crc_blocks = 1024;
+  if (crc_blocks + nfchunks == 0) return hipSuccess;
+  if (waves == 0) waves = kFusedWaves;
+  if (waves != 8 && waves != 16) return hipErrorInvalidValue;
+  if (nfchunks > 0 && (H <= 0 || W <= 0 || C <= 0)) return hipErrorInvalidValue;
+  const bool with_prep = prep && !prep->identity();
+  if (with_prep) {
+    if ((int64_t)H * W * C >= (1 << 20)) return hipErrorInvalidValue;
+    if (C > 4)
+      for (int i = 1; i < 4; ++i)
+        if (prep->a[i] != prep->a[0] || prep->b[i] != prep->b[0]) return hipErrorInvalidValue;
+  }
+  if (packed && (!tab || (reinterpret_cast<uintptr_t>(packed) & 7) ||
+                 (reinterpret_cast<uintptr_t>(bytes) & 15)))
+    return hipErrorInvalidValue;
+  const PackedText pt{packed, packed ? tab : nullptr};
+  const InputPrep pv = with_prep ? *prep : InputPrep();
+  if (waves == 8)
+    launch_crc_parse<8>(packed != nullptr, with_prep, crc_blocks + nfchunks, stream, bytes, pt,
+                        chunks, nchunks, tables, crc_out, crc_blocks, recs, fchunks, nfchunks, H,
+                        W, C, out, rtot, cbad, pv);
+  else
+    launch_crc_parse<16>(packed != nullptr, with_prep, crc_blocks + nfchunks, stream, bytes, pt,
+                         chunks, nchunks, tables, crc_out, crc_blocks, recs, fchunks, nfchunks, H,
+                         W, C, out, rtot, cbad, pv);
+  return hipGetLastError();
+}
+
 hipError_t json_parse_instances(int nrec, int ntiles, JsonRecord* recs, const int* tile_rec,
                                 const uint8_t* bytes, int H, int W, int C, int* tile_counts,
                                 float* out, hipStream_t stream, bool count_pass,
diff --git a/csrc/runtime/gpu_ingest.cpp b/csrc/runtime/gpu_ingest.cpp
--- a/csrc/runtime/gpu_ingest.cpp
+++ b/csrc/runtime/gpu_ingest.cpp
@@ -30,6 +30,7 @@
   }
   if (const char* e = getenv("GALE_INGEST_DEV_TIMING")) dev_every_ = std::max(0, atoi(e));
   if (const char* e = getenv("GALE_INGEST_PLAN_SEPARATE")) plan_separate_ = atoi(e) != 0;
+  if (const char* e = getenv("GALE_INGEST_FUSED")) fused_ = atoi(e) != 0;
   if (dev_every_ > 0)
     for (auto& L : lanes_)
       for (hipEvent_t& ev : L->tev) check_hip(hipEventCreate(&ev), "ingest: timing event");
@@ -245,9 +246,10 @@
   }
   const JsonIngestPlan& p = L.plan;
   plan_json_ingest(L.batches, kafka::kBatchAttrOffset, check_crcs, L.recs, H, W, C,
-                   arena ? arena_bytes : 0, f.size, dev_cap, f.tap_result, plan_separate_, L.plan);
+                   arena ? arena_bytes : 0, f.size, dev_cap, f.tap_result, plan_separate_, L.plan,
+                   fused_ ? kFusedWaves : 0);
   if (p.empty()) return;
-  const size_t nc = p.nc(), nr = p.nr(), np = p.np();
+  const size_t nc = p.nc(), nr = p.nr(), np = p.np(), nf = p.nf();
   grow(L, p.io_bytes + 16, (size_t)p.ntiles + (size_t)p.ngroups + 1);
   uint8_t* hpl = p.plan_in_chunk ? f.buf.get() + p.plan_off : L.h_io;
   uint8_t* dpl = p.plan_in_chunk ? dev + p.plan_off : L.d_io;
@@ -273,15 +275,28 @@
   int* d_gbad = reinterpret_cast<int*>(L.h_io + p.o_gbad);
   int* d_pbad = reinterpret_cast<int*>(L.h_io + p.o_pbad);
   int* d_cnt = p.cnt_base >= 0 ? reinterpret_cast<int*>(dev + p.cnt_base) : L.d_counts;
-  check_hip(ingest_crc_count(dev, reinterpret_cast<const CrcChunk*>(dpl + p.o_chunks), (int)nc,
+  int2* d_ftot = reinterpret_cast<int2*>(L.h_io + p.o_ftot);
+  int* d_fbad = reinterpret_cast<int*>(L.h_io + p.o_fbad);
+  const uint8_t* d_packed = p.packed ? dev + p.c_lo : nullptr;
+  const uint32_t* d_tab = p.packed ? reinterpret_cast<const uint32_t*>(dpl) : nullptr;
+  if (nf > 0) {
+    if (nr == 0) mark(L, ts, 2);
+    check_hip(ingest_crc_parse(dev, reinterpret_cast<const CrcChunk*>(dpl + p.o_chunks), (int)nc,
+                               d_tables_, d_crc, (int)nf, p.fchunks,
+                               reinterpret_cast<const JsonRecord*>(dpl + p.o_frecs),
+                               reinterpret_cast<const int2*>(dpl + p.o_fchunks), H, W, C, arena,
+                               d_ftot, d_fbad, L.stream, d_packed, d_tab, &input_prep_,
+                               p.fuse_waves),
+              "ingest: crc32c + count + parse");
+  }
+  const size_t nc2 = nf > 0 ? 0 : nc;
+  check_hip(ingest_crc_count(dev, reinterpret_cast<const CrcChunk*>(dpl + p.o_chunks), (int)nc2,
                              d_tables_, d_crc, (int)nr, p.ngroups,
                              reinterpret_cast<JsonRecord*>(dpl + p.o_recs),
                              reinterpret_cast<const int2*>(dpl + p.o_groups), d_cnt, d_gsum,
-                             d_gbad, L.stream, p.packed ? dev + p.c_lo : nullptr,
-                             p.packed ? reinterpret_cast<const uint32_t*>(dpl) : nullptr,
-                             p.packed ? dev : nullptr),
+                             d_gbad, L.stream, d_packed, d_tab, p.packed ? dev : nullptr),
             "ingest: crc32c + count");
-  mark(L, ts, 2);
+  if (!(nf > 0 && nr == 0)) mark(L, ts, 2);
   if (np > 0)
     check_hip(json_parse_instances((int)np, p.ptiles,
                                    reinterpret_cast<JsonRecord*>(dpl + p.o_precs),
@@ -291,6 +306,30 @@
               "ingest: parse");
   const int64_t t_post = end(L, ts, true);
   join_batch_crcs(f, p.batch_chunks, d_crc, io);
+  auto settle = [&](size_t i, int64_t tok, int bad, int v, int32_t slot) {
+    if (bad != 0) {
+      io.status[i] = codec::BAD_NUMBER;
+    } else if (tok == 0) {
+      io.status[i] = codec::EMPTY;
+    } else if (tok % p.per != 0) {
+      io.status[i] = codec::BAD_SHAPE;
+    } else {
+      io.images[i] = (int32_t)(tok / p.per);
+      if (v < 0) return true;
+      const int32_t verdict = device_verdict_status(v);
+      if (verdict != codec::OK) io.status[i] = verdict;
+      else io.img[i] = arena + (int64_t)slot * p.per;
+      return true;
+    }
+    return false;
+  };
+  const JsonRecord* hf = reinterpret_cast<const JsonRecord*>(hpl + p.o_frecs);
+  for (size_t q = 0; q < nf; ++q) {
+    const int nch = json_fused_chunks(hf[q].off, hf[q].len, p.fuse_waves);
+    int v = 0;
+    for (int c = 0; c < nch; ++c) v = std::max(v, d_fbad[hf[q].tile0 + c]);
+    settle((size_t)p.fused[q], d_ftot[q].x, d_ftot[q].y, v, hf[q].slot);
+  }
   size_t k = 0;
   for (size_t j = 0; j < nr; ++j) {
     const size_t i = (size_t)p.rec_of[j];
@@ -303,24 +342,14 @@
       tok += d_gsum[g];
       bad |= d_gbad[g];
     }
-    if (bad != 0) {
-      io.status[i] = codec::BAD_NUMBER;
-    } else if (tok == 0) {
-      io.status[i] = codec::EMPTY;
-    } else if (tok % p.per != 0) {
-      io.status[i] = codec::BAD_SHAPE;
-    } else {
-      io.images[i] = (int32_t)(tok / p.per);
-      if (p.cnt_base >= 0) io.cnt_off[i] = p.cnt_off(hr[j]);
-      if (pr) {
-        const int nt = json_tile_count(pr->off, pr->len);
-        int v = 0;
-        for (int t0 = 0; t0 < nt; ++t0) v = std::max(v, d_pbad[pr->tile0 + t0]);
-        const int32_t verdict = device_verdict_status(v);
-        if (verdict != codec::OK) io.status[i] = verdict;
-        else io.img[i] = arena + (int64_t)pr->slot * p.per;
-      }
+    int v = -1;
+    if (pr) {
+      const int nt = json_tile_count(pr->off, pr->len);
+      v = 0;
+      for (int t0 = 0; t0 < nt; ++t0) v = std::max(v, d_pbad[pr->tile0 + t0]);
     }
+    if (settle(i, tok, bad, v, pr ? pr->slot : 0) && p.cnt_base >= 0)
+      io.cnt_off[i] = p.cnt_off(hr[j]);
   }
   post_ns_ += mono_ns() - t_post;
 }
diff --git a/csrc/runtime/gpu_ingest.h b/csrc/runtime/gpu_ingest.h
--- a/csrc/runtime/gpu_ingest.h
+++ b/csrc/runtime/gpu_ingest.h
@@ -90,6 +90,7 @@
       dev_wait_ns_{0};
   int dev_every_ = 0;
   bool plan_separate_ = false;
+  bool fused_ = false;
   std::atomic<int64_t> plan_in_chunk_{0};
   uint32_t* d_tables_ = nullptr;
   std::vector<std::unique_ptr<Lane>> lanes_;
diff --git a/csrc/runtime/ingest_plan.cpp b/csrc/runtime/ingest_plan.cpp
--- a/csrc/runtime/ingest_plan.cpp
+++ b/csrc/runtime/ingest_plan.cpp
@@ -55,20 +55,31 @@
 void plan_json_ingest(const std::vector<std::pair<int64_t, int64_t>>& batches, int64_t attr_off,
                       bool check_crcs, const std::vector<JsonPlanRecord>& recs, int H, int W,
                       int C, size_t arena_bytes, size_t fetch_size, size_t dev_cap,
-                      int64_t tap_result, bool plan_separate, JsonIngestPlan& out) {
+                      int64_t tap_result, bool plan_separate, JsonIngestPlan& out,
+                      int fuse_waves) {
   {
     JsonIngestPlan fresh;
     fresh.chunks.swap(out.chunks);
     fresh.batch_chunks.swap(out.batch_chunks);
     fresh.rec_of.swap(out.rec_of);
     fresh.pjs.swap(out.pjs);
+    fresh.fused.swap(out.fused);
     fresh.chunks.clear();
     fresh.batch_chunks.clear();
     fresh.rec_of.clear();
     fresh.pjs.clear();
+    fresh.fused.clear();
     out = std::move(fresh);
   }
+  if (fuse_waves != 0 && fuse_waves != 8 && fuse_waves != 16)
+    throw std::invalid_argument("ingest plan: fused chunks are 8 or 16 tiles");
   const int64_t per = out.per = image_elements(H, W, C);
+  out.fuse_waves = fuse_waves;
+  const int64_t S = 2 * per;
+  auto slots_fit = [&](int64_t off, int64_t len) {
+    const int64_t slot = (off + S - 1) / S, cap = len / S;
+    return cap > 0 && (slot + cap) * per * (int64_t)sizeof(float) <= (int64_t)arena_bytes;
+  };
   size_t lo = fetch_size, hi = 0;
   plan_batches(batches, attr_off, check_crcs, fetch_size, out.chunks, out.batch_chunks, lo, hi);
   for (size_t i = 0; i < recs.size(); ++i) {
@@ -80,10 +91,16 @@
       throw std::invalid_argument("ingest plan: record outside the fetch");
     if ((uint64_t)r.arr_off + (uint64_t)r.arr_len > (uint64_t)r.value_len)
       throw std::invalid_argument("ingest plan: array outside its record");
-    out.rec_of.push_back((int)i);
     const int nt = json_tile_count(r.value_off + r.arr_off, (int32_t)r.arr_len);
-    out.ntiles += nt;
-    out.ngroups += (nt + kGroupTiles - 1) / kGroupTiles;
+    if (fuse_waves > 0 && arena_bytes > 0 && nt > 0 && nt <= kFusedMaxTiles &&
+        slots_fit(r.value_off + r.arr_off, r.arr_len)) {
+      out.fused.push_back((int)i);
+      out.fchunks += (nt + fuse_waves - 1) / fuse_waves;
+    } else {
+      out.rec_of.push_back((int)i);
+      out.ntiles += nt;
+      out.ngroups += (nt + kGroupTiles - 1) / kGroupTiles;
+    }
     lo = std::min(lo, (size_t)r.value_off);
     hi = std::max(hi, (size_t)(r.value_off + r.value_len));
   }
@@ -112,12 +129,10 @@
       out.cnt_base = (int64_t)((dev_cap - cb) & ~(size_t)255);
   }
   if (arena_bytes > 0 && out.cnt_base >= 0) {
-    const int64_t S = 2 * per;
     for (size_t j = 0; j < nr; ++j) {
       const JsonPlanRecord& r = recs[(size_t)out.rec_of[j]];
       const int64_t off = r.value_off + r.arr_off;
-      const int64_t slot = (off + S - 1) / S, cap = r.arr_len / S;
-      if (cap <= 0 || (slot + cap) * per * (int64_t)sizeof(float) > (int64_t)arena_bytes) continue;
+      if (!slots_fit(off, r.arr_len)) continue;
       out.pjs.push_back((int)j);
       out.ptiles += json_tile_count(off, (int32_t)r.arr_len);
     }
@@ -128,11 +143,16 @@
   out.o_recs = out.o_groups + align16(ngroups * sizeof(int2));
   out.o_precs = out.o_recs + nr * sizeof(JsonRecord);
   out.o_ptr = out.o_precs + np * sizeof(JsonRecord);
-  out.o_gsum = out.o_ptr + align16(ptiles * sizeof(int));
+  const size_t nf = out.nf(), fchunks = (size_t)out.fchunks;
+  out.o_frecs = out.o_ptr + align16(ptiles * sizeof(int));
+  out.o_fchunks = out.o_frecs + nf * sizeof(JsonRecord);
+  out.o_gsum = out.o_fchunks + align16(fchunks * sizeof(int2));
   out.o_crc = out.o_gsum + align16(ngroups * 4);
   out.o_gbad = out.o_crc + align16(nc * 4);
   out.o_pbad = out.o_gbad + align16(ngroups * 4);
-  out.io_bytes = out.o_pbad + align16(ptiles * 4);
+  out.o_ftot = out.o_pbad + align16(ptiles * 4);
+  out.o_fbad = out.o_ftot + align16(nf * sizeof(int2));
+  out.io_bytes = out.o_fbad + align16(fchunks * 4);
   out.plan_off = align256(std::max(fetch_size, out.used));
   const size_t plan_lim = out.cnt_base >= 0 ? (size_t)out.cnt_base : dev_cap;
   const bool on_tab = out.packed && out.plan_off < out.tab_off + out.ng * 2 * sizeof(uint32_t) &&
@@ -185,6 +205,28 @@
     const int nt = json_tile_count(pr.off, pr.len);
     for (int t = 0; t < nt; ++t) hpt[pt + t] = (int)k;
     pt += nt;
+  }
+  JsonRecord* hf = reinterpret_cast<JsonRecord*>(dst + p.o_frecs);
+  int2* hc = reinterpret_cast<int2*>(dst + p.o_fchunks);
+  int chunk = 0;
+  for (size_t k = 0; k < p.nf(); ++k) {
+    const JsonPlanRecord& r = recs[(size_t)p.fused[k]];
+    JsonRecord& fr = hf[k];
+    fr.off = r.value_off + r.arr_off;
+    fr.len = (int32_t)r.arr_len;
+    fr.slot = (int32_t)((fr.off + S - 1) / S);
+    fr.images = -1;
+    fr.status = 0;
+    fr.tile0 = chunk;
+    fr.has_cnt = 0;
+    fr.cnt_off = -1;
+    fr.grp0 = 0;
+    const int nt = json_tile_count(fr.off, fr.len);
+    for (int t0 = 0; t0 < nt; t0 += p.fuse_waves) {
+      hc[chunk].x = (int)k;
+      hc[chunk].y = t0;
+      ++chunk;
+    }
   }
 }
 
diff --git a/csrc/runtime/ingest_plan.h b/csrc/runtime/ingest_plan.h
--- a/csrc/runtime/ingest_plan.h
+++ b/csrc/runtime/ingest_plan.h
@@ -25,6 +25,9 @@
   std::vector<std::pair<size_t, size_t>> batch_chunks;
   std::vector<int> rec_of;
   std::vector<int> pjs;
+  std::vector<int> fused;
+  int fchunks = 0;
+  int fuse_waves = 0;
   int ntiles = 0, ngroups = 0;
   int ptiles = 0;
   bool packed = false;
@@ -36,6 +39,8 @@
   size_t o_chunks = 0, o_groups = 0, o_recs = 0, o_precs = 0, o_ptr = 0;
   size_t o_gsum = 0;
   size_t o_crc = 0, o_gbad = 0, o_pbad = 0, io_bytes = 0;
+  size_t o_frecs = 0, o_fchunks = 0;
+  size_t o_ftot = 0, o_fbad = 0;
   size_t plan_off = 0;
   bool plan_in_chunk = false;
   int64_t per = 0;
@@ -43,7 +48,8 @@
   size_t nc() const { return chunks.size(); }
   size_t nr() const { return rec_of.size(); }
   size_t np() const { return pjs.size(); }
-  bool empty() const { return chunks.empty() && rec_of.empty(); }
+  size_t nf() const { return fused.size(); }
+  bool empty() const { return chunks.empty() && rec_of.empty() && fused.empty(); }
   int64_t cnt_off(const JsonRecord& r) const {
     return cnt_base + ((int64_t)r.tile0 + r.grp0) * (int64_t)sizeof(int);
   }
@@ -52,7 +58,8 @@
 void plan_json_ingest(const std::vector<std::pair<int64_t, int64_t>>& batches, int64_t attr_off,
                       bool check_crcs, const std::vector<JsonPlanRecord>& recs, int H, int W,
                       int C, size_t arena_bytes, size_t fetch_size, size_t dev_cap,
-                      int64_t tap_result, bool plan_separate, JsonIngestPlan& out);
+                      int64_t tap_result, bool plan_separate, JsonIngestPlan& out,
+                      int fuse_waves = 0);
 
 void fill_json_ingest(const JsonIngestPlan& plan, const std::vector<JsonPlanRecord>& recs,
                       uint8_t* dst);
```

Measured after the change: 2.082 million. 0.969x the previous value.
